# microsoft/gated-graph-neural-network-samples

Measured on AMD Instinct MI355X. Metric: node-state updates/sec on QM9-shaped graphs, h=100, 4 edge types, higher is better.
Workload: dtype f32

## Files before the change

gated-graph-neural-network-samples_amd/_lib.py:

```python
from __future__ import annotations

import ctypes
import os
from ctypes import POINTER, c_char_p, c_float, c_int, c_int32, c_int64, c_size_t, c_uint64, c_void_p

_HERE = os.path.dirname(os.path.abspath(__file__))
LIB_PATH = os.path.join(_HERE, "libggnn_hip%s.so" % ("_" + os.environ["GGNN_LIB_VARIANT"] if os.environ.get("GGNN_LIB_VARIANT") else ""))
ABI_VERSION = 3

SYMBOLS = {
    "ggnn_abi_version": (c_int, []),
    "ggnn_matrix_path_is_split": (c_int, []),
    "ggnn_gru_forward_format": (c_int, []),
    "ggnn_gru_form_set": (c_int, [c_int]),
    "ggnn_absmax_f32": (c_int, [POINTER(c_void_p), POINTER(c_int64), c_int, c_void_p, c_void_p]),
    "ggnn_last_error": (c_char_p, []),
    "ggnn_csr_workspace_bytes": (c_size_t, [c_int64, c_int]),
    "ggnn_build_target_csr": (c_int, [c_void_p, POINTER(c_int64), c_int, c_int, c_int64, c_void_p, c_void_p,
                                      c_void_p, c_void_p, c_void_p, c_size_t, c_void_p]),
    "ggnn_build_source_csr": (c_int, [c_void_p, POINTER(c_int64), c_int, c_int, c_int64, c_void_p, c_void_p,
                                      c_void_p, c_void_p, c_void_p, c_size_t, c_void_p]),
    "ggnn_msg_transform_f32": (c_int, [c_void_p, c_int, c_void_p, c_void_p, c_int, c_int, c_int, c_void_p]),
    "ggnn_msg_transform_compact_supported": (c_int, [c_int]),
    "ggnn_compact_workspace_bytes": (c_size_t, [c_int, c_int]),
    "ggnn_build_compact_sources": (c_int, [c_void_p, c_int, c_int, c_void_p, c_void_p, c_void_p, c_void_p, c_size_t, c_void_p]),
    "ggnn_remap_gather_rows": (c_int, [c_void_p, c_void_p, c_void_p, c_int64, c_void_p]),
    "ggnn_msg_transform_compact_workspace_bytes": (c_size_t, [c_int, c_int]),
    "ggnn_msg_transform_compact_f32": (c_int, [c_void_p, c_void_p, c_void_p, POINTER(c_int64), c_void_p, c_void_p, c_size_t,
                                               c_int, c_int, c_int, c_int, c_void_p]),
    "ggnn_gather_segment_sum_f32": (c_int, [c_void_p, c_void_p, c_void_p, c_void_p, c_void_p, c_int, c_void_p,
                                            c_int, c_int, c_int, c_void_p]),
    "ggnn_build_slot_heads": (c_int, [c_void_p, c_void_p, c_void_p, c_int, c_void_p]),
    "ggnn_gather_segment_sum_heads_f32": (c_int, [c_void_p, c_void_p, c_void_p, c_void_p, c_void_p, c_void_p, c_int, c_void_p,
                                                  c_int, c_int, c_int, c_int, c_void_p]),
    "ggnn_attn_bwd_target_f32": (c_int, [c_void_p] * 11 + [c_int, c_int, c_int, c_int, c_void_p]),
    "ggnn_weighted_segment_sum_f32": (c_int, [c_void_p] * 6 + [c_int, c_int, c_int, c_void_p]),
    "ggnn_range_sum_f32": (c_int, [c_void_p, POINTER(c_int64), c_int, c_void_p, c_void_p]),
    "ggnn_unsorted_segment_sum_f32": (c_int, [c_void_p, c_void_p, c_void_p, c_int64, c_int, c_int, c_void_p]),
    "ggnn_gated_readout_f32": (c_int, [c_void_p, c_void_p, c_void_p, c_void_p, c_void_p, c_void_p, c_void_p, c_void_p, c_int,
                                       c_int, c_int, c_void_p]),
    "ggnn_readout_workspace_bytes": (c_size_t, [c_int, c_int, c_int]),
    "ggnn_readout_loss_fwd_f32": (c_int, [c_void_p] * 15 + [c_void_p, c_size_t, c_int, c_int, c_int, c_void_p]),
    "ggnn_readout_loss_bwd_f32": (c_int, [c_void_p] * 14 + [c_int] + [c_void_p] * 4 + [c_void_p, c_size_t, c_int, c_int, c_int, c_void_p]),
    "ggnn_gru_workspace_bytes": (c_size_t, [c_int, c_int]),
    "ggnn_gru_f32": (c_int, [POINTER(c_void_p), c_int, c_void_p, c_void_p, c_void_p, c_void_p, c_void_p, c_void_p,
                             c_void_p, c_size_t, c_void_p, c_void_p, c_void_p, c_int, c_int, c_int, c_void_p]),
    "ggnn_gather_segment_sum_attn_f32": (c_int, [c_void_p, c_void_p, c_void_p, c_void_p, c_void_p, c_void_p, c_void_p, c_int,
                                                 c_void_p, c_int, c_int, c_int, c_void_p]),
    "ggnn_rnn_f32": (c_int, [POINTER(c_void_p), c_int, c_void_p, c_void_p, c_void_p, c_void_p, c_int, c_int, c_int, c_void_p]),
    "ggnn_cudnn_gru_workspace_bytes": (c_size_t, [c_int, c_int]),
    "ggnn_cudnn_gru_f32": (c_int, [POINTER(c_void_p), c_int, c_void_p, c_void_p, c_void_p, c_void_p, c_void_p, c_void_p,
                                   c_void_p, c_void_p, c_void_p, c_size_t, c_int, c_int, c_void_p]),
    "ggnn_gru_is_fused": (c_int, [c_int]),
    "ggnn_gru_packed_bytes": (c_size_t, [c_int, c_int]),
    "ggnn_gru_pack_weights_f32": (c_int, [c_void_p, c_void_p, c_int, c_int, c_int, c_void_p, c_void_p]),
    "ggnn_gru_packed_f32": (c_int, [POINTER(c_void_p), c_int, c_void_p, c_void_p, c_void_p, c_void_p, c_void_p, c_void_p,
                                    c_void_p, c_void_p, c_int, c_int, c_int, c_int, c_void_p, c_void_p]),
    "ggnn_edge_weights_pack_f32": (c_int, [c_void_p, c_int, c_int, c_int, c_void_p, c_void_p]),
    "ggnn_gru_packed_gather_f32": (c_int, [POINTER(c_void_p), c_int, c_void_p, c_void_p, c_void_p, c_void_p, c_void_p, c_void_p,
                                           c_void_p, c_void_p, c_void_p, c_int, c_int, c_int, c_int, c_int, c_int, c_void_p, c_void_p]),
    "ggnn_gru_packed_gather_train_f32": (c_int, [POINTER(c_void_p), c_int, c_void_p, c_void_p, c_void_p, c_void_p, c_void_p, c_void_p,
                                                 c_void_p, c_void_p, c_void_p, c_int, c_int, c_void_p, c_void_p, c_void_p, c_void_p,
                                                 c_int, c_int, c_int, c_int, c_void_p, c_void_p]),
    "ggnn_gru_gates_f32": (c_int, [POINTER(c_void_p), c_int, c_void_p, c_void_p, c_void_p, c_void_p, c_void_p, c_void_p,
                                   c_int, c_int, c_void_p]),
    "ggnn_gru_candidate_f32": (c_int, [POINTER(c_void_p), c_int, c_void_p, c_void_p, c_void_p, c_void_p, c_void_p,
                                       c_void_p, c_void_p, c_int, c_int, c_int, c_void_p]),
    "ggnn_sparse_propagate_workspace_bytes": (c_size_t, [c_int, c_int, c_int, c_int64]),
    "ggnn_sparse_propagate_f32": (c_int, [c_void_p, c_int, c_int, c_int, c_void_p, c_void_p, c_void_p, POINTER(c_int64),
                                          c_void_p, c_int, c_int, POINTER(c_int32), POINTER(c_int32), POINTER(c_int32),
                                          POINTER(c_void_p), POINTER(c_void_p), POINTER(c_void_p), POINTER(c_void_p),
                                          POINTER(c_void_p), POINTER(c_void_p), POINTER(c_void_p), POINTER(c_void_p), POINTER(c_int32),
                                          POINTER(c_int32), c_int, c_int, POINTER(c_void_p), c_void_p, c_size_t, c_void_p]),
    "ggnn_gru_bwd_stage1_f32": (c_int, [c_void_p, c_void_p, c_void_p, c_void_p, c_void_p, c_int, c_void_p, c_void_p, c_void_p,
                                        c_void_p, c_int, c_int, c_int, c_int, c_void_p]),
    "ggnn_gru_bwd_stage2_f32": (c_int, [c_void_p, c_int, c_void_p, c_void_p, c_void_p, c_void_p, c_int, c_int, c_void_p]),
    "ggnn_dense_aggregate_f32": (c_int, [c_void_p, c_void_p, c_void_p, c_void_p, c_int, c_int, c_int, c_int, c_void_p]),
    "ggnn_gemm_f32": (c_int, [POINTER(c_void_p), c_int, c_int, c_int, c_void_p, c_int, c_void_p, c_int, c_int, c_int,
                              c_void_p]),
    "ggnn_xty_workspace_bytes": (c_size_t, [c_int, c_int, c_int, c_int]),
    "ggnn_xty_f32": (c_int, [POINTER(c_void_p), c_int, c_int, POINTER(c_int32), c_void_p, c_void_p, c_int, c_void_p, c_int, c_int,
                             c_int, POINTER(c_int32), c_int, c_void_p, c_size_t, c_void_p]),
    "ggnn_dense_propagate_supported": (c_int, [c_int, c_int, c_int]),
    "ggnn_dense_propagate_is_split": (c_int, [c_int, c_int, c_int]),
    "ggnn_dense_edge_packed_bytes": (c_size_t, [c_int, c_int]),
    "ggnn_dense_edge_pack_f32": (c_int, [c_void_p, c_int, c_int, c_void_p, c_void_p]),
    "ggnn_dense_gru_packed_bytes": (c_size_t, [c_int]),
    "ggnn_dense_gru_pack_f32": (c_int, [c_void_p, c_void_p, c_int, c_void_p, c_void_p]),
    "ggnn_dense_propagate_f32": (c_int, [c_void_p, c_void_p, c_void_p, c_void_p, c_void_p, c_void_p, c_void_p, c_void_p, c_int, c_int,
                                         c_int, c_int, c_int, c_int, c_void_p]),
    "ggnn_dense_train_supported": (c_int, [c_int, c_int, c_int]),
    "ggnn_dense_train_saved_bytes": (c_size_t, [c_int, c_int, c_int, c_int]),
    "ggnn_dense_propagate_save_f32": (c_int, [c_void_p, c_void_p, c_void_p, c_void_p, c_void_p, c_void_p, c_void_p, c_void_p, c_int, c_int,
                                              c_int, c_int, c_int, c_int, c_void_p, c_size_t, c_void_p]),
    "ggnn_dense_bwd_packed_bytes": (c_size_t, [c_int, c_int]),
    "ggnn_dense_bwd_pack_f32": (c_int, [c_void_p, c_void_p, c_void_p, c_int, c_int, c_void_p, c_void_p]),
    "ggnn_dense_propagate_bwd_f32": (c_int, [c_void_p, c_void_p, c_void_p, c_void_p, c_int, c_int, c_int, c_int, c_int, c_void_p, c_void_p,
                                             c_void_p, c_void_p, c_void_p, c_void_p]),
    "ggnn_dense_edge_grad_workspace_bytes": (c_size_t, [c_int, c_int, c_int]),
    "ggnn_dense_edge_grad_f32": (c_int, [c_void_p, c_void_p, c_void_p, c_void_p, c_int, c_int, c_int, c_int, c_void_p, c_void_p, c_int,
                                         c_void_p, c_size_t, c_void_p]),
    "ggnn_dense_train_workspace_bytes": (c_size_t, [c_int, c_int, c_int, c_int, c_int]),
    "ggnn_dense_train_forward_f32": (c_int, [c_void_p, c_void_p, c_void_p, c_void_p, c_void_p, c_void_p, c_void_p, c_int, c_int, c_int,
                                             c_int, c_int, c_int, c_void_p, c_size_t, POINTER(c_int64), c_void_p]),
    "ggnn_dense_train_backward_f32": (c_int, [c_void_p, c_void_p, c_void_p, c_void_p, c_int, c_int, c_int, c_int, c_int, c_void_p,
                                              c_void_p, c_void_p, c_void_p, c_void_p, c_void_p, c_void_p, c_size_t, c_void_p, c_void_p]),
    "ggnn_assemble_batch_backward": (c_int, [POINTER(c_void_p), POINTER(c_void_p), c_int, c_int, POINTER(c_int64), POINTER(c_int64), c_void_p,
                                             c_void_p, c_int, c_int, c_int, c_int, c_int, POINTER(c_int64), POINTER(c_int64),
                                             POINTER(c_void_p), c_void_p]),
    "ggnn_assemble_batch": (c_int, [POINTER(c_void_p), c_int, c_int, POINTER(c_int64), POINTER(c_int64), c_void_p, c_int, c_int, c_int,
                                    c_int, c_int, POINTER(c_int64), POINTER(c_int64), POINTER(c_void_p), c_void_p]),
    "ggnn_xty_acc_f32": (c_int, [POINTER(c_void_p), c_int, c_int, POINTER(c_int32), c_void_p, c_void_p, c_int, c_void_p, c_void_p,
                                 c_int, c_int, c_int, c_int, POINTER(c_int32), c_int, c_void_p, c_size_t, c_void_p]),
    "ggnn_colsum_workspace_bytes": (c_size_t, [c_int]),
    "ggnn_colsum_f32": (c_int, [c_void_p, c_int, c_int, c_int, c_void_p, c_void_p, c_size_t, c_void_p]),
    "ggnn_gru_bwd_dx_cand_f32": (c_int, [c_void_p] * 7 + [c_int, c_int, c_int, c_void_p]),
    "ggnn_gru_bwd_dx_gates_f32": (c_int, [c_void_p] * 5 + [c_int, c_int, c_void_p, c_int, c_int, c_int, c_void_p]),
    "ggnn_gather_segment_sum_acc_f32": (c_int, [c_void_p, c_void_p, c_void_p, c_void_p, c_int, c_int, c_void_p]),
    "ggnn_bwd_dx_f32": (c_int, [c_void_p, c_int, c_int, c_void_p, c_int, c_void_p, c_int, c_int, c_void_p, c_void_p, c_int, c_int,
                                c_void_p, c_int, c_int, c_int, c_int, c_void_p]),
    "ggnn_act_bwd_f32": (c_int, [c_void_p, c_void_p, c_int, c_void_p, c_int, c_int, c_void_p]),
    "ggnn_cudnn_gru_train_f32": (c_int, [POINTER(c_void_p), c_int] + [c_void_p] * 9 + [c_void_p, c_size_t, c_int, c_int, c_void_p]),
    "ggnn_cudnn_gru_bwd_stage_f32": (c_int, [c_void_p] * 10 + [c_int, c_int, c_void_p]),
    "ggnn_gru_bwd_is_fused": (c_int, [c_int]),
    "ggnn_gru_bwd_packed_bytes": (c_size_t, [c_int, c_int]),
    "ggnn_gru_bwd_fused_f32": (c_int, [c_void_p] * 12 + [POINTER(c_void_p), c_void_p, c_int, c_int, c_int, c_int, c_int, c_int, c_void_p]),
    "ggnn_gru_bwd_fused_gather_f32": (c_int, [c_void_p] * 12 + [POINTER(c_void_p), c_void_p, c_int, c_int, c_int, c_int, c_int, c_int, c_void_p]),
    "ggnn_optim_block_floats": (c_int, []),
    "ggnn_clip_adam_f32": (c_int, [c_void_p] * 9 + [c_int, c_float, c_float, c_float, c_float, c_float, c_void_p]),
    "ggnn_probe_mfma_workspace_bytes": (c_size_t, []),
    "ggnn_probe_mfma_rate": (c_int, [c_int, c_int, c_void_p, c_size_t, POINTER(ctypes.c_double), POINTER(ctypes.c_double), c_void_p]),
    "ggnn_gemm_tn_workspace_bytes": (c_size_t, [c_int, c_int, c_int]),
    "ggnn_gemm_tn_f32": (c_int, [c_void_p, c_int, c_void_p, c_int, c_void_p, c_int, c_int, c_int, c_void_p, c_size_t, c_void_p]),
    "ggnn_pack_batch_tables": (c_int, [c_void_p, c_int, c_int, c_void_p, c_int, c_void_p, c_void_p, c_int, c_void_p, c_int, c_void_p,
                                       c_void_p, c_void_p, c_void_p]),
    "ggnn_sparse_train_prepare_f32": (c_int, [c_int, c_int, c_int, POINTER(c_int32), POINTER(c_void_p), c_float, POINTER(c_uint64),
                                              POINTER(c_void_p), POINTER(c_void_p), POINTER(c_int32), POINTER(c_void_p), POINTER(c_void_p),
                                              POINTER(c_void_p), POINTER(c_void_p), c_void_p]),
    "ggnn_sparse_train_workspace_bytes": (c_size_t, [c_int, c_int, c_int, c_int64, c_int]),
    "ggnn_sparse_train_forward_f32": (c_int, [c_void_p, c_int, c_int, c_int, c_void_p, c_void_p, c_void_p, POINTER(c_int64), c_void_p,
                                              c_int, c_int, POINTER(c_int32), POINTER(c_int32), POINTER(c_int32), POINTER(c_void_p),
                                              POINTER(c_void_p), POINTER(c_void_p), POINTER(c_void_p), POINTER(c_int32), c_int, c_void_p,
                                              c_size_t, POINTER(c_int64), c_void_p]),
    "ggnn_sparse_train_backward_f32": (c_int, [c_void_p, c_int, c_int, c_int, c_void_p, POINTER(c_int64), c_void_p, c_int, c_int,
                                               POINTER(c_int32), POINTER(c_int32), POINTER(c_int32), c_void_p, c_void_p, c_void_p,
                                               c_void_p, c_void_p, c_void_p, c_void_p, POINTER(c_void_p), POINTER(c_void_p), c_int,
                                               POINTER(c_void_p), POINTER(c_void_p), POINTER(c_void_p), POINTER(c_void_p),
                                               POINTER(c_void_p), c_void_p, POINTER(c_void_p), c_void_p, c_size_t, c_void_p, c_void_p]),
    "ggnn_dropout_f32": (c_int, [c_void_p, c_void_p, c_void_p, c_int64, c_uint64, c_float, c_int64, c_int, c_void_p]),
    "ggnn_gcn_fused_supported": (c_int, [c_int]),
    "ggnn_gcn_image_bytes": (c_size_t, [c_int]),
    "ggnn_gcn_pack_weights_f32": (c_int, [c_void_p, c_int, c_int, c_void_p, c_void_p]),
    "ggnn_gcn_layer_f32": (c_int, [c_void_p, c_void_p, c_void_p, c_void_p, c_int64, c_void_p, c_void_p, c_int, c_void_p, c_int64,
                                   c_uint64, c_float, c_void_p, c_void_p, c_int, c_int, c_void_p]),
    "ggnn_gcn_epilogue_f32": (c_int, [c_void_p, c_void_p, c_int, c_void_p, c_int64, c_uint64, c_float, c_void_p, c_int, c_int, c_void_p]),
    "ggnn_gcn_workspace_bytes": (c_size_t, [c_int, c_int, c_int]),
    "ggnn_gcn_propagate_f32": (c_int, [c_void_p, c_int, c_int, c_int, c_void_p, c_void_p, c_void_p, c_int64, POINTER(c_void_p),
                                       POINTER(c_void_p), c_void_p, c_void_p, c_size_t, c_void_p]),
    "ggnn_gcn_assemble_batch": (c_int, [POINTER(c_void_p), c_int, c_int, c_int, c_void_p, c_int, c_void_p, c_int, c_int, c_int, c_int,
                                        c_int, c_int, POINTER(c_void_p), c_void_p]),
    "ggnn_dense_assemble_batch": (c_int, [POINTER(c_void_p), c_int, c_int, c_int, c_int, c_void_p, c_int, c_void_p, c_int, c_int, c_int,
                                          c_int, c_int, c_int, c_int, POINTER(c_int64), POINTER(c_int64), c_int, POINTER(c_void_p),
                                          c_void_p]),
}

_lib = None


class GGNNError(RuntimeError):
    def __init__(self, code: int, msg: str):
        super().__init__("libggnn_hip error %d: %s" % (code, msg))
        self.code = code


def load() -> ctypes.CDLL:
    global _lib
    if _lib is not None:
        return _lib
    if not os.path.exists(LIB_PATH):
        raise ImportError(
            "libggnn_hip.so not found at %s -- run `python __graft_entry__.py build` (hipcc, gfx950). "
            "There is no CPU fallback for the GGNN hot path." % LIB_PATH)
    lib = ctypes.CDLL(LIB_PATH)
    for name, (restype, argtypes) in SYMBOLS.items():
        fn = getattr(lib, name)
        fn.restype = restype
        fn.argtypes = argtypes
    ver = lib.ggnn_abi_version()
    if ver != ABI_VERSION:
        raise ImportError("libggnn_hip.so ABI version %d != expected %d; rebuild" % (ver, ABI_VERSION))
    _lib = lib
    return lib


def check(rc: int) -> None:
    if rc != 0:
        msg = load().ggnn_last_error()
        raise GGNNError(rc, msg.decode("utf-8", "replace") if msg else "")
```

gated-graph-neural-network-samples_amd/csrc/ggnn_bwd_gemm.hip:

```cpp
#include "ggnn_gemm.hpp"
#include "ggnn_split.hpp"

namespace ggnn {

constexpr int kXtyMaxBatch = 64;
constexpr int kXtyWaves = 16;
constexpr int kXtyMaxI = 4;
#ifndef GGNN_XTY_TIMELINE
#define GGNN_XTY_TIMELINE 0
#endif

__device__ const float kXtyOnesChunk[4] = {1.0f, 0.0f, 0.0f, 0.0f};
__device__ const float kXtyZeroChunk[4] = {0.0f, 0.0f, 0.0f, 0.0f};

struct XtyArgs {
    const float* X[4]; int ldx[4]; int nseg; int Dseg;
    const int* x_rows;
    const float* Y; int ldy;
    float* part;
    int K, N, nbatch;
    int Kout;
    int row_off[kXtyMaxBatch + 1];
    int wg_off[kXtyMaxBatch + 1];
    int kb_tiles, n_tiles;
    int pitch_x, pitch_y;
    unsigned long long* tdbg;
};

static inline int xty_pitch(int width) {
    int p = (width + 15) / 16 * 16;
    while (p % 64 != 16 && p % 64 != 48) p += 16;
    return p;
}

__host__ __device__ inline void xty_group(int n, int g, int& off, int& cnt) {
    const int base = n >> 2, rem = n & 3;
    cnt = base + (g < rem ? 1 : 0);
    off = g * base + (g < rem ? g : rem);
}

template <bool GATHER, int ROWS, int MTM, int NTM>
__global__ __launch_bounds__(kXtyWaves * 64) void xty_kernel(XtyArgs a) {
    extern __shared__ __attribute__((aligned(16))) float slab[];
    constexpr int nw = kXtyWaves;
    const int tid = threadIdx.x, lane = tid & 63;
    const int wave = __builtin_amdgcn_readfirstlane(tid >> 6);
    const int li = lane & 15, kq = lane >> 4;
    int batch = 0;
    while (batch + 1 < a.nbatch && (int)blockIdx.y >= a.wg_off[batch + 1]) ++batch;
    const int split = (int)blockIdx.y - a.wg_off[batch], splits = a.wg_off[batch + 1] - a.wg_off[batch];
    const int rb = a.row_off[batch], re = a.row_off[batch + 1];
    int rows_per = (re - rb + splits - 1) / splits;
    rows_per = (rows_per + ROWS - 1) / ROWS * ROWS;
    const int r_beg = rb + split * rows_per;
    const int r_end = min(re, r_beg + rows_per);
    const int kcol0 = blockIdx.x * a.kb_tiles * 16;
    const int px = a.pitch_x, py = a.pitch_y;
    float* sx = slab;
    float* sy = slab + 2 * ROWS * px;
    float* out = a.part + (size_t)blockIdx.y * a.Kout * a.N;

    int kt0, my_mt, nt0, my_nt;
    xty_group(a.kb_tiles, wave >> 2, kt0, my_mt);
    xty_group(a.n_tiles, ((wave >> 2) + (wave & 3)) & 3, nt0, my_nt);

    int stamp_i = 2;
#if GGNN_XTY_TIMELINE
#define GGNN_XT(K) if (a.tdbg && blockIdx.x == 0 && blockIdx.y == 0 && lane == 0 && (wave == 0 || wave == nw - 1) && (K) < 64) \
        a.tdbg[(wave ? 64 : 0) + (K)] = __builtin_amdgcn_s_memtime();
#else
#define GGNN_XT(K)
#endif
    GGNN_XT(0)

    constexpr int MAXI = kXtyMaxI;
    const int cprx = px / 4, cpry = py / 4;
    const int nix = ROWS * cprx / 64, niy = ROWS * cpry / 64;
    unsigned mx[MAXI], my[MAXI];
#pragma unroll
    for (int j = 0; j < MAXI; ++j) {
        const int ix = j * nw + wave;
        mx[j] = 0x80000000u; my[j] = 0x80000000u;
        if (ix < nix) {
            const int c = ix * 64 + lane, row = c / cprx, q = c - row * cprx;
            int col = kcol0 + 4 * q;
            const bool ones = a.Kout > a.K && col == a.K && 4 * q < a.kb_tiles * 16;
            if (!(4 * q < a.kb_tiles * 16 && col < a.K)) col = 0;
            const int seg = col / a.Dseg, within = col - seg * a.Dseg;
            mx[j] = (unsigned)within | ((unsigned)seg << 16) | ((unsigned)row << 18) | (ones ? 0x40000000u : 0u);
        }
        if (ix < niy) {
            const int c = ix * 64 + lane, row = c / cpry, q = c - row * cpry;
            my[j] = (unsigned)(4 * q < a.N ? 4 * q : 0) | ((unsigned)row << 18);
        }
    }
    auto xrow = [&](int r0, unsigned m) -> int {
        int r = r0 + (int)((m >> 18) & 127u); r = r < r_end ? r : r_end - 1;
        return r;
    };
    int rid[GATHER ? MAXI : 1];
    auto fetch_rows = [&](int r0) {
        if constexpr (GATHER) {
#pragma unroll
            for (int j = 0; j < MAXI; ++j) rid[j] = (mx[j] >> 31) ? 0 : a.x_rows[xrow(r0 < r_end ? r0 : r_beg, mx[j])];
        }
    };
    auto sgpr_ptr = [](const float* p) {
        const unsigned long long v = reinterpret_cast<unsigned long long>(p);
        const unsigned lo = __builtin_amdgcn_readfirstlane((unsigned)v), hi = __builtin_amdgcn_readfirstlane((unsigned)(v >> 32));
        return reinterpret_cast<const float*>(((unsigned long long)hi << 32) | lo);
    };
    const float* X0 = sgpr_ptr(a.X[0]); const float* X1 = sgpr_ptr(a.X[1]);
    const float* X2 = sgpr_ptr(a.X[2]); const float* X3 = sgpr_ptr(a.X[3]);
    const int L0 = __builtin_amdgcn_readfirstlane(a.ldx[0]), L1 = __builtin_amdgcn_readfirstlane(a.ldx[1]);
    const int L2 = __builtin_amdgcn_readfirstlane(a.ldx[2]), L3 = __builtin_amdgcn_readfirstlane(a.ldx[3]);
    const float* Yb = sgpr_ptr(a.Y);
    const int ldy = __builtin_amdgcn_readfirstlane(a.ldy);
    auto issue = [&](int buf, int r0) {
#pragma unroll
        for (int j = 0; j < MAXI; ++j) {
            if (!(mx[j] >> 31)) {
                const unsigned m = mx[j];
                const int seg = (int)((m >> 16) & 3u);
                const float* xb = seg == 0 ? X0 : (seg == 1 ? X1 : (seg == 2 ? X2 : X3));
                const int xl = seg == 0 ? L0 : (seg == 1 ? L1 : (seg == 2 ? L2 : L3));
                const int xr = GATHER ? rid[GATHER ? j : 0] : xrow(r0, m);
                const float* src = xb + (size_t)xr * xl + (m & 0xFFFFu);
                if (m & 0x40000000u) src = kXtyOnesChunk;
                if (r0 + (int)((m >> 18) & 127u) >= r_end) src = kXtyZeroChunk;
                float* dst = sx + buf * ROWS * px + (size_t)(j * nw + wave) * 256;
                __builtin_amdgcn_global_load_lds((glb_void*)src, (lds_void*)dst, 16, 0, 0);
            }
        }
#pragma unroll
        for (int j = 0; j < MAXI; ++j) {
            if (!(my[j] >> 31)) {
                const unsigned m = my[j];
                int r = r0 + (int)((m >> 18) & 127u); r = r < r_end ? r : r_end - 1;
                const float* src = Yb + (size_t)r * ldy + (m & 0xFFFFu);
                float* dst = sy + buf * ROWS * py + (size_t)(j * nw + wave) * 256;
                __builtin_amdgcn_global_load_lds((glb_void*)src, (lds_void*)dst, 16, 0, 0);
            }
        }
    };

    auto run = [&](auto mt_c, auto nt_c) {
        constexpr int MT = decltype(mt_c)::value, NT = decltype(nt_c)::value;
        constexpr bool ON = MT > 0 && NT > 0;
        f32x4 acc[ON ? MT : 1][ON ? NT : 1];
#pragma unroll
        for (int mt = 0; mt < (ON ? MT : 1); ++mt)
#pragma unroll
            for (int nt = 0; nt < (ON ? NT : 1); ++nt) acc[mt][nt] = f32x4{0.f, 0.f, 0.f, 0.f};
        const int cls = wave >> 2;
        if (r_beg < r_end) {
            int buf = 0;
            fetch_rows(r_beg);
            issue(0, r_beg);
            fetch_rows(r_beg + ROWS);
            __syncthreads();
            GGNN_XT(1)
            for (int r0 = r_beg; r0 < r_end; r0 += ROWS) {
                const bool has_next = r0 + ROWS < r_end;
                if (has_next && !ON) { issue(buf ^ 1, r0 + ROWS); fetch_rows(r0 + 2 * ROWS); }
                if (stamp_i < 22) { GGNN_XT(20 + stamp_i) }
                if constexpr (ON) {
                    const float* bx = sx + buf * ROWS * px + kt0 * 16 + li;
                    const float* by = sy + buf * ROWS * py + nt0 * 16 + li;
                    float xa[2][MT], yb[2][NT];
#pragma unroll
                    for (int mt = 0; mt < MT; ++mt) xa[0][mt] = bx[kq * px + mt * 16];
#pragma unroll
                    for (int nt = 0; nt < NT; ++nt) yb[0][nt] = by[kq * py + nt * 16];
#pragma unroll
                    for (int s = 0; s < ROWS / 4; ++s) {
                        if (s + 1 < ROWS / 4) {
#pragma unroll
                            for (int mt = 0; mt < MT; ++mt) xa[(s + 1) & 1][mt] = bx[(4 * (s + 1) + kq) * px + mt * 16];
#pragma unroll
                            for (int nt = 0; nt < NT; ++nt) yb[(s + 1) & 1][nt] = by[(4 * (s + 1) + kq) * py + nt * 16];
                        }
                        if (s % (ROWS / 32) == 0 && s / (ROWS / 32) < 4) {
                            if (has_next && cls == s / (ROWS / 32)) { issue(buf ^ 1, r0 + ROWS); fetch_rows(r0 + 2 * ROWS); }
                        }
                        __builtin_amdgcn_sched_barrier(0);
#pragma unroll
                        for (int mt = 0; mt < MT; ++mt)
#pragma unroll
                            for (int nt = 0; nt < NT; ++nt)
                                acc[mt][nt] = __builtin_amdgcn_mfma_f32_16x16x4f32(xa[s & 1][mt], yb[s & 1][nt], acc[mt][nt], 0, 0, 0);
                        __builtin_amdgcn_sched_barrier(0);
                    }
                }
                if (stamp_i < 22) { GGNN_XT(40 + stamp_i) }
                __syncthreads();
                buf ^= 1;
                if (stamp_i < 22) { GGNN_XT(stamp_i) }
                ++stamp_i;
            }
        }
        GGNN_XT(62)
        if constexpr (ON) {
#pragma unroll
            for (int mt = 0; mt < MT; ++mt) {
                const int k0 = kcol0 + (kt0 + mt) * 16;
#pragma unroll
                for (int nt = 0; nt < NT; ++nt) {
                    const int n = 16 * (nt0 + nt) + li;
                    if (n < a.N) {
#pragma unroll
                        for (int e = 0; e < 4; ++e) {
                            const int k = k0 + 4 * kq + e;
                            if (k < a.Kout) out[(size_t)k * a.N + n] = acc[mt][nt][e];
                        }
                    }
                }
            }
        }
        GGNN_XT(63)
    };
    using I0 = std::integral_constant<int, 0>;
    using IM = std::integral_constant<int, MTM>; using IM1 = std::integral_constant<int, MTM - 1>;
    using IN = std::integral_constant<int, NTM>; using IN1 = std::integral_constant<int, NTM - 1>;
    if (my_mt == MTM && my_nt == NTM) run(IM{}, IN{});
    else if (my_mt == MTM - 1 && my_nt == NTM) run(IM1{}, IN{});
    else if (my_mt == MTM && my_nt == NTM - 1) run(IM{}, IN1{});
    else if (my_mt == MTM - 1 && my_nt == NTM - 1) run(IM1{}, IN1{});
    else run(I0{}, I0{});
#undef GGNN_XT
}


#ifndef GGNN_XTY_INTER_MAX
#define GGNN_XTY_INTER_MAX 24
#endif
constexpr int kXtySplitWaves = 8;
constexpr int kXtySplitMaxI = 8;

template <bool GATHER, int ROWS, int MTM, int NTM>
__global__ __launch_bounds__(kXtySplitWaves * 64) void xty_split_kernel(XtyArgs a) {
    extern __shared__ __attribute__((aligned(16))) float slab[];
    constexpr int nw = kXtySplitWaves;
    const int tid = threadIdx.x, lane = tid & 63;
    const int wave = __builtin_amdgcn_readfirstlane(tid >> 6);
    const int li = lane & 15, kq = lane >> 4;
    int batch = 0;
    while (batch + 1 < a.nbatch && (int)blockIdx.y >= a.wg_off[batch + 1]) ++batch;
    const int split = (int)blockIdx.y - a.wg_off[batch], splits = a.wg_off[batch + 1] - a.wg_off[batch];
    const int rb = a.row_off[batch], re = a.row_off[batch + 1];
    int rows_per = (re - rb + splits - 1) / splits;
    rows_per = (rows_per + ROWS - 1) / ROWS * ROWS;
    const int r_beg = rb + split * rows_per;
    const int r_end = min(re, r_beg + rows_per);
    const int kcol0 = blockIdx.x * a.kb_tiles * 16;
    const int px = a.pitch_x, py = a.pitch_y;
    float* sx = slab;
    float* sy = slab + 2 * ROWS * px;
    float* out = a.part + (size_t)blockIdx.y * a.Kout * a.N;

    int kt0, my_mt, nta0, cnta, ntb0, cntb;
    xty_group(a.kb_tiles, wave >> 1, kt0, my_mt);
    const int ga = ((wave >> 1) + 2 * (wave & 1)) & 3;
    xty_group(a.n_tiles, ga, nta0, cnta);
    xty_group(a.n_tiles, (ga + 1) & 3, ntb0, cntb);
    const int my_nt = cnta + cntb;

    constexpr int MAXI = kXtySplitMaxI;
    const int cprx = px / 4, cpry = py / 4;
    const int nix = ROWS * cprx / 64, niy = ROWS * cpry / 64;
    unsigned mx[MAXI], my[MAXI];
#pragma unroll
    for (int j = 0; j < MAXI; ++j) {
        const int ix = j * nw + wave;
        mx[j] = 0x80000000u; my[j] = 0x80000000u;
        if (ix < nix) {
            const int c = ix * 64 + lane, row = c / cprx, q = c - row * cprx;
            int col = kcol0 + 4 * q;
            const bool ones = a.Kout > a.K && col == a.K && 4 * q < a.kb_tiles * 16;
            if (!(4 * q < a.kb_tiles * 16 && col < a.K)) col = 0;
            const int seg = col / a.Dseg, within = col - seg * a.Dseg;
            mx[j] = (unsigned)within | ((unsigned)seg << 16) | ((unsigned)row << 18) | (ones ? 0x40000000u : 0u);
        }
        if (ix < niy) {
            const int c = ix * 64 + lane, row = c / cpry, q = c - row * cpry;
            my[j] = (unsigned)(4 * q < a.N ? 4 * q : 0) | ((unsigned)row << 18);
        }
    }
    auto xrow = [&](int r0, unsigned m) __attribute__((always_inline)) -> int {
        int r = r0 + (int)((m >> 18) & 127u); r = r < r_end ? r : r_end - 1;
        return r;
    };
    int rid[GATHER ? MAXI : 1];
    auto fetch_rows = [&](int r0) __attribute__((always_inline)) {
        if constexpr (GATHER) {
#pragma unroll
            for (int j = 0; j < MAXI; ++j) rid[j] = (mx[j] >> 31) ? 0 : a.x_rows[xrow(r0 < r_end ? r0 : r_beg, mx[j])];
        }
    };
    auto sgpr_ptr = [](const float* p) {
        const unsigned long long v = reinterpret_cast<unsigned long long>(p);
        const unsigned lo = __builtin_amdgcn_readfirstlane((unsigned)v), hi = __builtin_amdgcn_readfirstlane((unsigned)(v >> 32));
        return reinterpret_cast<const float*>(((unsigned long long)hi << 32) | lo);
    };
    const float* X0 = sgpr_ptr(a.X[0]); const float* X1 = sgpr_ptr(a.X[1]);
    const float* X2 = sgpr_ptr(a.X[2]); const float* X3 = sgpr_ptr(a.X[3]);
    const int L0 = __builtin_amdgcn_readfirstlane(a.ldx[0]), L1 = __builtin_amdgcn_readfirstlane(a.ldx[1]);
    const int L2 = __builtin_amdgcn_readfirstlane(a.ldx[2]), L3 = __builtin_amdgcn_readfirstlane(a.ldx[3]);
    const float* Yb = sgpr_ptr(a.Y);
    const int ldy = __builtin_amdgcn_readfirstlane(a.ldy);
    auto dma1 = [&](const float* src, float* dst) __attribute__((always_inline)) {
        const unsigned l = __builtin_amdgcn_readfirstlane((unsigned)(unsigned long)(lds_void*)dst);
        asm volatile("s_mov_b32 m0, %0\n\ts_nop 0\n\tglobal_load_lds_dwordx4 %1, off" :: "s"(l), "v"(src) : "memory");
    };
    auto issue = [&](int buf, int r0) __attribute__((always_inline)) {
#pragma unroll
        for (int j = 0; j < MAXI; ++j) {
            if (!(mx[j] >> 31)) {
                const unsigned m = mx[j];
                const int seg = (int)((m >> 16) & 3u);
                const float* xb = seg == 0 ? X0 : (seg == 1 ? X1 : (seg == 2 ? X2 : X3));
                const int xl = seg == 0 ? L0 : (seg == 1 ? L1 : (seg == 2 ? L2 : L3));
                const int xr = GATHER ? rid[GATHER ? j : 0] : xrow(r0, m);
                const float* src = xb + (size_t)xr * xl + (m & 0xFFFFu);
                if (m & 0x40000000u) src = kXtyOnesChunk;
                if (r0 + (int)((m >> 18) & 127u) >= r_end) src = kXtyZeroChunk;
                dma1(src, sx + buf * ROWS * px + (size_t)(j * nw + wave) * 256);
            }
        }
#pragma unroll
        for (int j = 0; j < MAXI; ++j) {
            if (!(my[j] >> 31)) {
                const unsigned m = my[j];
                int r = r0 + (int)((m >> 18) & 127u); r = r < r_end ? r : r_end - 1;
                dma1(Yb + (size_t)r * ldy + (m & 0xFFFFu), sy + buf * ROWS * py + (size_t)(j * nw + wave) * 256);
            }
        }
    };

    auto run = [&](auto mt_c, auto nt_c) __attribute__((always_inline)) {
        constexpr int MT = decltype(mt_c)::value, NT = decltype(nt_c)::value;
        constexpr bool ON = MT > 0 && NT > 0;
        f32x4 acc[ON ? MT : 1][ON ? NT : 1];
#pragma unroll
        for (int mt = 0; mt < (ON ? MT : 1); ++mt)
#pragma unroll
            for (int nt = 0; nt < (ON ? NT : 1); ++nt) acc[mt][nt] = f32x4{0.f, 0.f, 0.f, 0.f};
        auto ycol = [&](int t) __attribute__((always_inline)) { return (t < cnta ? nta0 + t : ntb0 + (t - cnta)) * 16; };
        if (r_beg < r_end) {
            int buf = 0;
            fetch_rows(r_beg);
            issue(0, r_beg);
            fetch_rows(r_beg + ROWS);
            dma_wait();
            __syncthreads();
            for (int r0 = r_beg; r0 < r_end; r0 += ROWS) {
                const bool has_next = r0 + ROWS < r_end;
                if (has_next) { issue(buf ^ 1, r0 + ROWS); fetch_rows(r0 + 2 * ROWS); }
                if constexpr (ON) {
                    const float* bx = sx + buf * ROWS * px + kt0 * 16 + li;
                    const float* by = sy + buf * ROWS * py + li;
                    auto tile_planes = [&](const float* col, int pitch, int s, u32x4& hi, u32x4& mid, u32x4& lo) __attribute__((always_inline)) {
                        float v[8];
#pragma unroll
                        for (int j = 0; j < 8; ++j) v[j] = col[(size_t)(32 * s + 4 * j + kq) * pitch];
                        unsigned h[4], m[4], l[4];
#pragma unroll
                        for (int q = 0; q < 4; ++q) split_pair(v[2 * q], v[2 * q + 1], h[q], m[q], l[q]);
                        hi = u32x4{h[0], h[1], h[2], h[3]}; mid = u32x4{m[0], m[1], m[2], m[3]}; lo = u32x4{l[0], l[1], l[2], l[3]};
                    };
#pragma unroll
                    for (int s = 0; s < ROWS / 32; ++s) {
                        u32x4 xh[MT], xm[MT], xl[MT];
#pragma unroll
                        for (int mt = 0; mt < MT; ++mt) tile_planes(bx + mt * 16, px, s, xh[mt], xm[mt], xl[mt]);
                        u32x4 yh, ym, yl, zh, zm, zl;
                        tile_planes(by + ycol(0), py, s, yh, ym, yl);
#pragma unroll
                        for (int nt = 0; nt < NT; ++nt) {
                            __builtin_amdgcn_sched_barrier(0);
                            if (nt + 1 < NT) tile_planes(by + ycol(nt + 1), py, s, zh, zm, zl);
#define GGNN_XS(XP, YP) _Pragma("unroll") for (int mt = 0; mt < MT; ++mt) acc[mt][nt] = mfma_bf16(XP[mt], YP, acc[mt][nt]);
                            GGNN_XS(xl, yh) GGNN_XS(xm, ym) GGNN_XS(xm, yh) GGNN_XS(xh, yl) GGNN_XS(xh, ym) GGNN_XS(xh, yh)
#undef GGNN_XS
                            yh = zh; ym = zm; yl = zl;
                        }
                        __builtin_amdgcn_sched_barrier(0);
                    }
                }
                dma_wait();
                __syncthreads();
                buf ^= 1;
            }
        }
        if constexpr (ON) {
#pragma unroll
            for (int mt = 0; mt < MT; ++mt) {
                const int k0 = kcol0 + (kt0 + mt) * 16;
#pragma unroll
                for (int nt = 0; nt < NT; ++nt) {
                    const int n = ycol(nt) + li;
                    if (n < a.N) {
#pragma unroll
                        for (int e = 0; e < 4; ++e) {
                            const int k = k0 + 4 * kq + e;
                            if (k < a.Kout) out[(size_t)k * a.N + n] = acc[mt][nt][e];
                        }
                    }
                }
            }
        }
    };
    using I0 = std::integral_constant<int, 0>;
    using IM = std::integral_constant<int, MTM>; using IM1 = std::integral_constant<int, MTM - 1>;
    using IN = std::integral_constant<int, 2 * NTM>; using IN1 = std::integral_constant<int, 2 * NTM - 1>;
    using IN2 = std::integral_constant<int, 2 * NTM - 2>;
    if (my_mt == MTM && my_nt == 2 * NTM) run(IM{}, IN{});
    else if (my_mt == MTM && my_nt == 2 * NTM - 1) run(IM{}, IN1{});
    else if (my_mt == MTM && my_nt == 2 * NTM - 2) run(IM{}, IN2{});
    else if (my_mt == MTM - 1 && my_nt == 2 * NTM) run(IM1{}, IN{});
    else if (my_mt == MTM - 1 && my_nt == 2 * NTM - 1) run(IM1{}, IN1{});
    else if (my_mt == MTM - 1 && my_nt == 2 * NTM - 2) run(IM1{}, IN2{});
    else run(I0{}, I0{});
}

template <int MTM, int NTM>
__global__ __launch_bounds__(kXtySplitWaves * 64) void xty_planes_kernel(XtyArgs a) {
    extern __shared__ __attribute__((aligned(16))) float slab[];
    constexpr int nw = kXtySplitWaves, NTH = nw * 64, ROWS = 32;
    const int tid = threadIdx.x, lane = tid & 63;
    const int wave = __builtin_amdgcn_readfirstlane(tid >> 6);
    const int li = lane & 15, kq = lane >> 4;
    int batch = 0;
    while (batch + 1 < a.nbatch && (int)blockIdx.y >= a.wg_off[batch + 1]) ++batch;
    const int split = (int)blockIdx.y - a.wg_off[batch], splits = a.wg_off[batch + 1] - a.wg_off[batch];
    const int rb = a.row_off[batch], re = a.row_off[batch + 1];
    int rows_per = (re - rb + splits - 1) / splits;
    rows_per = (rows_per + ROWS - 1) / ROWS * ROWS;
    const int r_beg = rb + split * rows_per;
    const int r_end = min(re, r_beg + rows_per);
    const int kcol0 = blockIdx.x * a.kb_tiles * 16;
    const int XC = a.kb_tiles * 16, YC = a.n_tiles * 16, CT = XC + YC;
    const unsigned plane_b = 4u * (unsigned)CT * 16u;
    const unsigned buf_b = 3u * plane_b;
    float* out = a.part + (size_t)blockIdx.y * a.Kout * a.N;

    int kt0, my_mt, nta0, cnta, ntb0, cntb;
    xty_group(a.kb_tiles, wave >> 1, kt0, my_mt);
    const int ga = ((wave >> 1) + 2 * (wave & 1)) & 3;
    xty_group(a.n_tiles, ga, nta0, cnta);
    xty_group(a.n_tiles, (ga + 1) & 3, ntb0, cntb);
    const int my_nt = cnta + cntb;

    const char* const zero_p = reinterpret_cast<const char*>(kXtyZeroChunk);
    const int QT = CT >> 2;
    const bool uon = tid < 4 * QT;
    const int ug = uon ? tid / QT : 0;
    const int uc = uon ? 4 * (tid - ug * QT) : 0;
    const int ureg = uc < XC ? 0 : XC, utile = (uc - ureg) >> 4;
    const unsigned udbase = ((unsigned)ug * (unsigned)CT + (unsigned)ureg + 16u * (unsigned)utile) * 16u;
    const unsigned urot = (unsigned)(((uc - ureg) & 15) + utile);
    const char* urow = zero_p; unsigned ustride = 0u;
    if (uon) {
        const size_t row0 = (size_t)(r_beg + 8 * ug);
        if (uc < XC) {
            const int col = kcol0 + uc;
            if (col < a.K) {
                const int seg = col / a.Dseg;
                ustride = (unsigned)a.ldx[seg] * 4u;
                urow = reinterpret_cast<const char*>(a.X[seg] + (col - seg * a.Dseg)) + row0 * ustride;
            } else if (col == a.K && a.Kout > a.K) urow = reinterpret_cast<const char*>(kXtyOnesChunk);
        } else if (uc - XC < a.N) {
            ustride = (unsigned)a.ldy * 4u;
            urow = reinterpret_cast<const char*>(a.Y + (uc - XC)) + row0 * ustride;
        }
    }
    const bool wave_on = wave * 64 < 4 * QT;
    f32x4 stage[8];
    auto fetch = [&](int r0, auto full_c) __attribute__((always_inline)) {
        constexpr bool FULL = decltype(full_c)::value;
        if (wave_on) {
            const char* q = urow;
#pragma unroll
            for (int j = 0; j < 8; ++j) {
                const char* src = q;
                if constexpr (!FULL) { if (r0 + 8 * ug + j >= r_end) src = zero_p; }
                stage[j] = *(const __attribute__((address_space(1))) f32x4*)src;
                q += ustride;
            }
            urow += (size_t)32 * ustride;
        }
    };
    auto fetch_step = [&](int r0) __attribute__((always_inline)) {
        if (r0 + ROWS <= r_end) fetch(r0, std::true_type{}); else fetch(r0, std::false_type{});
    };
    auto put_col = [&](int buf, auto k_c) __attribute__((always_inline)) {
        constexpr int k = decltype(k_c)::value;
        if (wave_on) {
            char* base = reinterpret_cast<char*>(slab) + (size_t)buf * buf_b;
            unsigned h[4], m[4], l[4];
#pragma unroll
            for (int q = 0; q < 4; ++q) split_pair(stage[2 * q][k], stage[2 * q + 1][k], h[q], m[q], l[q]);
            if (uon) {
                const unsigned d = udbase + ((urot + (unsigned)k) & 15u) * 16u;
                *reinterpret_cast<u32x4*>(base + d) = u32x4{h[0], h[1], h[2], h[3]};
                *reinterpret_cast<u32x4*>(base + plane_b + d) = u32x4{m[0], m[1], m[2], m[3]};
                *reinterpret_cast<u32x4*>(base + 2u * plane_b + d) = u32x4{l[0], l[1], l[2], l[3]};
            }
        }
    };
    auto put = [&](int buf) __attribute__((always_inline)) {
        put_col(buf, std::integral_constant<int, 0>{}); put_col(buf, std::integral_constant<int, 1>{});
        put_col(buf, std::integral_constant<int, 2>{}); put_col(buf, std::integral_constant<int, 3>{});
    };
    auto advance_col = [&](int buf, int r0, bool has_next, auto k_c) __attribute__((always_inline)) {
        if (has_next) {
            put_col(buf ^ 1, k_c);
            if (decltype(k_c)::value == 3 && r0 + 2 * ROWS < r_end) fetch_step(r0 + 2 * ROWS);
        }
    };

    auto run = [&](auto mt_c, auto nt_c) __attribute__((always_inline)) {
        constexpr int MT = decltype(mt_c)::value, NT = decltype(nt_c)::value;
        constexpr bool ON = MT > 0 && NT > 0;
        f32x4 acc[ON ? MT : 1][ON ? NT : 1];
#pragma unroll
        for (int mt = 0; mt < (ON ? MT : 1); ++mt)
#pragma unroll
            for (int nt = 0; nt < (ON ? NT : 1); ++nt) acc[mt][nt] = f32x4{0.f, 0.f, 0.f, 0.f};
        auto ytile = [&](int t) __attribute__((always_inline)) { return t < cnta ? nta0 + t : ntb0 + (t - cnta); };
        auto mma_step = [&](int buf, int r0, bool has_next, auto inter_c) __attribute__((always_inline)) {
            constexpr bool INTER = decltype(inter_c)::value;
            if constexpr (ON) {
                const char* pb = reinterpret_cast<const char*>(slab) + (size_t)buf * buf_b + (unsigned)kq * (unsigned)CT * 16u;
                auto planes = [&](int reg, int T, u32x4& hi, u32x4& mid, u32x4& lo) __attribute__((always_inline)) {
                    const char* q = pb + (unsigned)(reg + 16 * T + ((li + T) & 15)) * 16u;
                    hi = *reinterpret_cast<const u32x4*>(q); mid = *reinterpret_cast<const u32x4*>(q + plane_b);
                    lo = *reinterpret_cast<const u32x4*>(q + 2u * plane_b);
                };
                u32x4 xh[MT], xm[MT], xl[MT];
#pragma unroll
                for (int mt = 0; mt < MT; ++mt) planes(0, kt0 + mt, xh[mt], xm[mt], xl[mt]);
                u32x4 yh, ym, yl, zh, zm, zl;
                planes(XC, ytile(0), yh, ym, yl);
#pragma unroll
                for (int nt = 0; nt < NT; ++nt) {
                    if (nt + 1 < NT) planes(XC, ytile(nt + 1), zh, zm, zl);
#define GGNN_XS(XP, YP) _Pragma("unroll") for (int mt = 0; mt < MT; ++mt) acc[mt][nt] = mfma_bf16(XP[mt], YP, acc[mt][nt]);
                    GGNN_XS(xl, yh) GGNN_XS(xm, ym) GGNN_XS(xm, yh) GGNN_XS(xh, yl) GGNN_XS(xh, ym) GGNN_XS(xh, yh)
#undef GGNN_XS
                    yh = zh; ym = zm; yl = zl;
                    if constexpr (INTER) {
                        constexpr int PU = NT >= 8 ? 2 : 1;
                        if (nt % PU == 0 && nt / PU < 4) {
                            if (nt / PU == 0) advance_col(buf, r0, has_next, std::integral_constant<int, 0>{});
                            if (nt / PU == 1) advance_col(buf, r0, has_next, std::integral_constant<int, 1>{});
                            if (nt / PU == 2) advance_col(buf, r0, has_next, std::integral_constant<int, 2>{});
                            if (nt / PU == 3) advance_col(buf, r0, has_next, std::integral_constant<int, 3>{});
                        }
                    }
                }
                if constexpr (INTER && NT < 4) {
                    if (NT <= 1) advance_col(buf, r0, has_next, std::integral_constant<int, 1>{});
                    if (NT <= 2) advance_col(buf, r0, has_next, std::integral_constant<int, 2>{});
                    if (NT <= 3) advance_col(buf, r0, has_next, std::integral_constant<int, 3>{});
                }
            }
        };
        if (r_beg < r_end) {
            int buf = 0;
            fetch_step(r_beg);
            put(0);
            if (r_beg + ROWS < r_end) fetch_step(r_beg + ROWS);
            __syncthreads();
            constexpr bool INTER = ON && MT * NT <= GGNN_XTY_INTER_MAX;
            for (int r0 = r_beg; r0 < r_end; r0 += ROWS) {
                const bool has_next = r0 + ROWS < r_end;
                if constexpr (!INTER) { if (has_next) { put(buf ^ 1); if (r0 + 2 * ROWS < r_end) fetch_step(r0 + 2 * ROWS); } }
                mma_step(buf, r0, has_next, std::integral_constant<bool, INTER>{});
                __syncthreads();
                buf ^= 1;
            }
        }
        if constexpr (ON) {
#pragma unroll
            for (int mt = 0; mt < MT; ++mt) {
                const int k0 = kcol0 + (kt0 + mt) * 16;
#pragma unroll
                for (int nt = 0; nt < NT; ++nt) {
                    const int n = ytile(nt) * 16 + li;
                    if (n < a.N) {
#pragma unroll
                        for (int e = 0; e < 4; ++e) {
                            const int k = k0 + 4 * kq + e;
                            if (k < a.Kout) out[(size_t)k * a.N + n] = acc[mt][nt][e];
                        }
                    }
                }
            }
        }
    };
    using I0 = std::integral_constant<int, 0>;
    using IM = std::integral_constant<int, MTM>; using IM1 = std::integral_constant<int, MTM - 1>;
    using IN = std::integral_constant<int, 2 * NTM>; using IN1 = std::integral_constant<int, 2 * NTM - 1>;
    using IN2 = std::integral_constant<int, 2 * NTM - 2>;
    if (my_mt == MTM && my_nt == 2 * NTM) run(IM{}, IN{});
    else if (my_mt == MTM && my_nt == 2 * NTM - 1) run(IM{}, IN1{});
    else if (my_mt == MTM && my_nt == 2 * NTM - 2) run(IM{}, IN2{});
    else if (my_mt == MTM - 1 && my_nt == 2 * NTM) run(IM1{}, IN{});
    else if (my_mt == MTM - 1 && my_nt == 2 * NTM - 1) run(IM1{}, IN1{});
    else if (my_mt == MTM - 1 && my_nt == 2 * NTM - 2) run(IM1{}, IN2{});
    else run(I0{}, I0{});
}

struct XtyReduceArgs { int wg_off[kXtyMaxBatch + 1]; };
__global__ __launch_bounds__(256) void xty_reduce_kernel(const float* __restrict__ part, float* __restrict__ C, float* __restrict__ Cb,
                                                         int KN, int KwN, int nbatch, int accumulate, XtyReduceArgs ra) {
    __shared__ float red[8][32];
    const int c = threadIdx.x & 31, q = threadIdx.x >> 5;
    const long long i = (long long)blockIdx.x * 32 + c;
    const bool on = i < (long long)KN * nbatch;
    float s = 0.f;
    int b = 0, j = 0;
    if (on) {
        b = (int)(i / KN); j = (int)(i - (long long)b * KN);
        const int S = ra.wg_off[b + 1] - ra.wg_off[b];
        const float* src = part + (size_t)ra.wg_off[b] * KN + j;
        int p = q;
        for (; p + 24 < S; p += 32) {
            const float v0 = src[(size_t)p * KN], v1 = src[(size_t)(p + 8) * KN], v2 = src[(size_t)(p + 16) * KN], v3 = src[(size_t)(p + 24) * KN];
            s += v0; s += v1; s += v2; s += v3;
        }
        for (; p < S; p += 8) s += src[(size_t)p * KN];
    }
    red[q][c] = s;
    __syncthreads();
    if (q == 0 && on) {
        const float v = ((red[0][c] + red[1][c]) + (red[2][c] + red[3][c])) + ((red[4][c] + red[5][c]) + (red[6][c] + red[7][c]));
        float* dst = (Cb && j >= KwN) ? Cb + (size_t)b * (KN - KwN) + (j - KwN) : C + (size_t)b * (Cb ? KwN : KN) + j;
        *dst = accumulate ? *dst + v : v;
    }
}

struct XtyPlan { int rows, kb_tiles, n_tiles, kblocks, px, py, wg_rows; size_t lds; int wg_off[kXtyMaxBatch + 1]; };

static XtyPlan xty_plan(const int* row_off, int nbatch, int Kout, int N) {
    XtyPlan p{};
    const int ktiles = (Kout + 15) / 16;
    p.kblocks = (ktiles + 15) / 16;
    p.kb_tiles = (ktiles + p.kblocks - 1) / p.kblocks;
    p.n_tiles = (N + 15) / 16;
    p.px = xty_pitch(p.kb_tiles * 16); p.py = xty_pitch(p.n_tiles * 16);
    const int mtm = (p.kb_tiles + 3) / 4, ntm = (p.n_tiles + 3) / 4;
    p.rows = (size_t)2 * 64 * (p.px + p.py) * sizeof(float) <= (size_t)160 * 1024 && mtm + ntm <= 6 ? 64 : 32;
    static const int rows_env = [] { const char* e = getenv("GGNN_XTY_ROWS"); return e ? atoi(e) : 0; }();
    if (rows_env == 32) p.rows = 32;
    p.lds = (size_t)2 * p.rows * (p.px + p.py) * sizeof(float);
    long long total = 0;
    for (int b = 0; b < nbatch; ++b) total += row_off[b + 1] - row_off[b];
    int target = num_cus() / p.kblocks;
    if (target < 1) target = 1;
    p.wg_off[0] = 0;
    for (int b = 0; b < nbatch; ++b) {
        const long long m = row_off[b + 1] - row_off[b];
        long long w = total > 0 ? (long long)target * m / total : 0;
        const long long cap = (m + 4 * p.rows - 1) / (4 * p.rows);
        if (w > cap) w = cap;
        if (w < 1 && m > 0) w = 1;
        p.wg_off[b + 1] = p.wg_off[b] + (int)w;
    }
    p.wg_rows = p.wg_off[nbatch];
    return p;
}

template <bool GATHER, int ROWS, int MTM, int NTM>
static int launch_xty(const XtyArgs& a, const XtyPlan& p, float* C, float* Cb, int accumulate, hipStream_t st) {
    static std::atomic<unsigned long long> lds_ok{0};
    if (p.wg_rows > 0) {
        if (p.lds > 64 * 1024) GGNN_CHECK_HIP((allow_dynamic_lds(&xty_kernel<GATHER, ROWS, MTM, NTM>, p.lds, lds_ok)));
        hipLaunchKernelGGL((xty_kernel<GATHER, ROWS, MTM, NTM>), dim3(p.kblocks, p.wg_rows), dim3(kXtyWaves * 64), p.lds, st, a);
        GGNN_CHECK_HIP(hipGetLastError());
    }
    XtyReduceArgs ra;
    for (int b = 0; b <= kXtyMaxBatch; ++b) ra.wg_off[b] = a.wg_off[b <= a.nbatch ? b : a.nbatch];
    const long long total = (long long)a.Kout * a.N * a.nbatch;
    hipLaunchKernelGGL(xty_reduce_kernel, dim3((unsigned)((total + 31) / 32)), dim3(256), 0, st, (const float*)a.part, C, Cb, a.Kout * a.N,
                       a.K * a.N, a.nbatch, accumulate, ra);
    GGNN_CHECK_HIP(hipGetLastError());
    return GGNN_OK;
}

template <int MTM, int NTM>
static int launch_xty_planes(const XtyArgs& a, const XtyPlan& p, float* C, float* Cb, int accumulate, hipStream_t st) {
    static std::atomic<unsigned long long> lds_ok{0};
    const size_t lds = (size_t)2 * 192 * (size_t)(16 * (p.kb_tiles + p.n_tiles));
    if (p.wg_rows > 0) {
        if (lds > 64 * 1024) GGNN_CHECK_HIP((allow_dynamic_lds(&xty_planes_kernel<MTM, NTM>, lds, lds_ok)));
        hipLaunchKernelGGL((xty_planes_kernel<MTM, NTM>), dim3(p.kblocks, p.wg_rows), dim3(kXtySplitWaves * 64), lds, st, a);
        GGNN_CHECK_HIP(hipGetLastError());
    }
    XtyReduceArgs ra;
    for (int b = 0; b <= kXtyMaxBatch; ++b) ra.wg_off[b] = a.wg_off[b <= a.nbatch ? b : a.nbatch];
    const long long total = (long long)a.Kout * a.N * a.nbatch;
    hipLaunchKernelGGL(xty_reduce_kernel, dim3((unsigned)((total + 31) / 32)), dim3(256), 0, st, (const float*)a.part, C, Cb, a.Kout * a.N,
                       a.K * a.N, a.nbatch, accumulate, ra);
    GGNN_CHECK_HIP(hipGetLastError());
    return GGNN_OK;
}

template <bool GATHER, int ROWS, int MTM, int NTM>
static int launch_xty_split(const XtyArgs& a, const XtyPlan& p, float* C, float* Cb, int accumulate, hipStream_t st) {
    static std::atomic<unsigned long long> lds_ok{0};
    if (p.wg_rows > 0) {
        if (p.lds > 64 * 1024) GGNN_CHECK_HIP((allow_dynamic_lds(&xty_split_kernel<GATHER, ROWS, MTM, NTM>, p.lds, lds_ok)));
        hipLaunchKernelGGL((xty_split_kernel<GATHER, ROWS, MTM, NTM>), dim3(p.kblocks, p.wg_rows), dim3(kXtySplitWaves * 64), p.lds, st, a);
        GGNN_CHECK_HIP(hipGetLastError());
    }
    XtyReduceArgs ra;
    for (int b = 0; b <= kXtyMaxBatch; ++b) ra.wg_off[b] = a.wg_off[b <= a.nbatch ? b : a.nbatch];
    const long long total = (long long)a.Kout * a.N * a.nbatch;
    hipLaunchKernelGGL(xty_reduce_kernel, dim3((unsigned)((total + 31) / 32)), dim3(256), 0, st, (const float*)a.part, C, Cb, a.Kout * a.N,
                       a.K * a.N, a.nbatch, accumulate, ra);
    GGNN_CHECK_HIP(hipGetLastError());
    return GGNN_OK;
}

constexpr int kColsumBlocks = 256;

__global__ __launch_bounds__(256) void colsum_partial_kernel(const float* __restrict__ Y, int ldy, int M, int N, float* __restrict__ part) {
    extern __shared__ float red[];
    const int N4 = N >> 2;
    const int lanes_per_row = N4;
    const int rows_par = 256 / lanes_per_row > 0 ? 256 / lanes_per_row : 1;
    const int rl = threadIdx.x / lanes_per_row, c4 = threadIdx.x % lanes_per_row;
    f32x4 s = {0.f, 0.f, 0.f, 0.f};
    if (rl < rows_par) {
        for (int r = blockIdx.x * rows_par + rl; r < M; r += gridDim.x * rows_par)
            s += *reinterpret_cast<const f32x4*>(Y + (size_t)r * ldy + 4 * c4);
        *reinterpret_cast<f32x4*>(red + rl * N + 4 * c4) = s;
    }
    __syncthreads();
    for (int i = threadIdx.x; i < N; i += 256) {
        float t = 0.f;
        for (int q = 0; q < rows_par; ++q) t += red[q * N + i];
        part[(size_t)blockIdx.x * N + i] = t;
    }
}

__global__ void colsum_final_kernel(const float* __restrict__ part, int nblocks, int N, float* __restrict__ out) {
    const int i = blockIdx.x * blockDim.x + threadIdx.x;
    if (i >= N) return;
    float s[8] = {0.f, 0.f, 0.f, 0.f, 0.f, 0.f, 0.f, 0.f};
    int b = 0;
    for (; b + 8 <= nblocks; b += 8) {
#pragma unroll
        for (int q = 0; q < 8; ++q) s[q] += part[(size_t)(b + q) * N + i];
    }
    for (int q = 0; b < nblocks; ++b, ++q) s[q] += part[(size_t)b * N + i];
    out[i] = ((s[0] + s[1]) + (s[2] + s[3])) + ((s[4] + s[5]) + (s[6] + s[7]));
}

}

using namespace ggnn;

extern "C" size_t ggnn_xty_workspace_bytes(int M_max, int K, int N, int nbatch) {
    if (M_max <= 0 || K <= 0 || N <= 0 || nbatch <= 0) return 256;
    return (size_t)(num_cus() + nbatch) * (K + 1) * N * sizeof(float) + 256;
}

extern "C" int ggnn_xty_f32(const float* const* x_segs, int nseg, int Dseg, const int32_t* ldx, const int32_t* x_rows,
                            const float* Y, int ldy, float* C, int K, int N, int ones_row, const int32_t* row_off, int nbatch,
                            void* ws, size_t ws_bytes, ggnn_stream_t stream) {
    return ggnn_xty_acc_f32(x_segs, nseg, Dseg, ldx, x_rows, Y, ldy, C, nullptr, 0, K, N, ones_row, row_off, nbatch, ws, ws_bytes, stream);
}

extern "C" int ggnn_xty_acc_f32(const float* const* x_segs, int nseg, int Dseg, const int32_t* ldx, const int32_t* x_rows,
                                const float* Y, int ldy, float* C, float* Cb, int accumulate, int K, int N, int ones_row,
                                const int32_t* row_off, int nbatch, void* ws, size_t ws_bytes, ggnn_stream_t stream) {
    const int Kout = ones_row ? K + 1 : K;
    GGNN_CHECK_ARG(!Cb || ones_row, "a bias destination needs the ones row");
    GGNN_CHECK_ARG(nseg >= 1 && nseg <= 4 && Dseg > 0 && Dseg % 4 == 0 && K == nseg * Dseg, "X is nseg <= 4 segments of Dseg columns (K = %d, nseg = %d, Dseg = %d)", K, nseg, Dseg);
    GGNN_CHECK_ARG(N > 0 && N % 4 == 0 && N <= 256, "N = %d must be a multiple of 4, <= 256", N);
    GGNN_CHECK_ARG(nbatch >= 1 && nbatch <= kXtyMaxBatch && row_off && C && ldx, "bad batch description");
    GGNN_CHECK_ARG(ldy >= N && ldy % 4 == 0, "ldy %d", ldy);
    hipStream_t st = (hipStream_t)stream;
    XtyArgs a{};
    int m_max = 0;
    for (int b = 0; b <= nbatch; ++b) {
        a.row_off[b] = row_off[b];
        if (b) { GGNN_CHECK_ARG(row_off[b] >= row_off[b - 1], "row_off not monotone"); m_max = row_off[b] - row_off[b - 1] > m_max ? row_off[b] - row_off[b - 1] : m_max; }
    }
    if (m_max == 0) {
        if (!accumulate) {
            GGNN_CHECK_HIP(hipMemsetAsync(C, 0, (size_t)nbatch * (Cb ? K : Kout) * N * sizeof(float), st));
            if (Cb) GGNN_CHECK_HIP(hipMemsetAsync(Cb, 0, (size_t)nbatch * N * sizeof(float), st));
        }
        return GGNN_OK;
    }
    GGNN_CHECK_ARG(x_segs && Y && ws && aligned16(Y) && aligned16(ws), "null or misaligned pointer");
    for (int s = 0; s < nseg; ++s) {
        GGNN_CHECK_ARG(x_segs[s] && aligned16(x_segs[s]) && ldx[s] >= Dseg && ldx[s] % 4 == 0, "X segment %d null, misaligned or bad stride", s);
        a.X[s] = x_segs[s]; a.ldx[s] = ldx[s];
    }
    if (ws_bytes < ggnn_xty_workspace_bytes(m_max, K, N, nbatch)) return fail(GGNN_E_WORKSPACE, "xty workspace too small");
    const XtyPlan p = xty_plan(row_off, nbatch, Kout, N);
    a.Kout = Kout;
    a.nseg = nseg; a.Dseg = Dseg; a.x_rows = x_rows; a.Y = Y; a.ldy = ldy; a.part = static_cast<float*>(ws);
    a.K = K; a.N = N; a.nbatch = nbatch; a.kb_tiles = p.kb_tiles; a.n_tiles = p.n_tiles;
    a.pitch_x = p.px; a.pitch_y = p.py;
    for (int b = 0; b <= kXtyMaxBatch; ++b) a.wg_off[b] = p.wg_off[b <= nbatch ? b : nbatch];
    { const char* e = getenv("GGNN_XTY_TPTR"); a.tdbg = e ? (unsigned long long*)strtoull(e, nullptr, 10) : nullptr; }
    if ((p.rows * p.px / 256 + kXtyWaves - 1) / kXtyWaves > kXtyMaxI || (p.rows * p.py / 256 + kXtyWaves - 1) / kXtyWaves > kXtyMaxI)
        return fail(GGNN_E_UNSUPPORTED, "xty: slab too wide (K=%d N=%d)", K, N);
    const int mtm = (p.kb_tiles + 3) / 4, ntm = (p.n_tiles + 3) / 4;
    const bool g = x_rows != nullptr;
    static const bool xty_split = [] { const char* e = getenv("GGNN_XTY_SPLIT"); return !e || atoi(e) != 0; }();
    if (split_matrix_path() && xty_split && p.kb_tiles >= 4 && p.n_tiles >= 4 && (p.rows * p.px / 256 + kXtySplitWaves - 1) / kXtySplitWaves <= kXtySplitMaxI &&
        (p.rows * p.py / 256 + kXtySplitWaves - 1) / kXtySplitWaves <= kXtySplitMaxI) {
        static const bool xty_planes = [] { const char* e = getenv("GGNN_XTY_PLANES"); return !e || atoi(e) != 0; }();
        if (xty_planes && !g && (size_t)2 * 192 * 16 * (p.kb_tiles + p.n_tiles) <= (size_t)160 * 1024 &&
            16 * (p.kb_tiles + p.n_tiles) <= kXtySplitWaves * 64) {
#define GGNN_XTYP_CASE(M, Nn) if (mtm == M && ntm == Nn) return launch_xty_planes<M, Nn>(a, p, C, Cb, accumulate, st);
            GGNN_XTYP_CASE(4, 4) GGNN_XTYP_CASE(3, 4) GGNN_XTYP_CASE(4, 2) GGNN_XTYP_CASE(3, 2)
#undef GGNN_XTYP_CASE
        }
#define GGNN_XTYS_CASE(G, R, M, Nn) if (g == G && p.rows == R && mtm == M && ntm == Nn) return launch_xty_split<G, R, M, Nn>(a, p, C, Cb, accumulate, st);
        GGNN_XTYS_CASE(false, 32, 4, 4) GGNN_XTYS_CASE(false, 32, 3, 4) GGNN_XTYS_CASE(false, 64, 4, 2) GGNN_XTYS_CASE(false, 64, 3, 2)
#undef GGNN_XTYS_CASE
    }
#define GGNN_XTY_CASE(G, R, M, Nn) if (g == G && p.rows == R && mtm == M && ntm == Nn) return launch_xty<G, R, M, Nn>(a, p, C, Cb, accumulate, st);
#define GGNN_XTY_ROW32(M) GGNN_XTY_CASE(false, 32, M, 1) GGNN_XTY_CASE(false, 32, M, 2) GGNN_XTY_CASE(false, 32, M, 3) GGNN_XTY_CASE(false, 32, M, 4)
    GGNN_XTY_ROW32(1) GGNN_XTY_ROW32(2) GGNN_XTY_ROW32(3) GGNN_XTY_ROW32(4)
    GGNN_XTY_CASE(false, 64, 1, 1) GGNN_XTY_CASE(false, 64, 1, 2) GGNN_XTY_CASE(false, 64, 1, 3) GGNN_XTY_CASE(false, 64, 1, 4)
    GGNN_XTY_CASE(false, 64, 2, 1) GGNN_XTY_CASE(false, 64, 2, 2) GGNN_XTY_CASE(false, 64, 2, 3) GGNN_XTY_CASE(false, 64, 2, 4)
    GGNN_XTY_CASE(false, 64, 3, 1) GGNN_XTY_CASE(false, 64, 3, 2) GGNN_XTY_CASE(false, 64, 3, 3)
    GGNN_XTY_CASE(false, 64, 4, 1) GGNN_XTY_CASE(false, 64, 4, 2)
    GGNN_XTY_CASE(true, 64, 1, 1) GGNN_XTY_CASE(true, 64, 1, 2) GGNN_XTY_CASE(true, 64, 2, 1) GGNN_XTY_CASE(true, 64, 2, 2)
#undef GGNN_XTY_ROW32
#undef GGNN_XTY_CASE
    return fail(GGNN_E_UNSUPPORTED, "xty: no kernel for %d x %d tile groups (K=%d N=%d)", mtm, ntm, K, N);
}

extern "C" size_t ggnn_colsum_workspace_bytes(int N) { return (size_t)kColsumBlocks * (N > 0 ? N : 1) * sizeof(float) + 256; }

extern "C" int ggnn_colsum_f32(const float* Y, int ldy, int M, int N, float* out, void* ws, size_t ws_bytes, ggnn_stream_t stream) {
    GGNN_CHECK_ARG(M >= 0 && N > 0 && N % 4 == 0 && N <= 1024 && ldy >= N && ldy % 4 == 0, "bad sizes M=%d N=%d ldy=%d", M, N, ldy);
    GGNN_CHECK_ARG(out && ws, "null pointer");
    if (ws_bytes < ggnn_colsum_workspace_bytes(N)) return fail(GGNN_E_WORKSPACE, "colsum workspace too small");
    hipStream_t st = (hipStream_t)stream;
    if (M == 0) { GGNN_CHECK_HIP(hipMemsetAsync(out, 0, N * sizeof(float), st)); return GGNN_OK; }
    GGNN_CHECK_ARG(Y && aligned16(Y), "null or misaligned pointer");
    const int rows_par = 256 / (N / 4) > 0 ? 256 / (N / 4) : 1;
    GGNN_CHECK_ARG(N / 4 <= 256, "N too large");
    int nb = (M + rows_par - 1) / rows_par;
    if (nb > kColsumBlocks) nb = kColsumBlocks;
    float* part = static_cast<float*>(ws);
    hipLaunchKernelGGL(colsum_partial_kernel, dim3(nb), dim3(256), (size_t)rows_par * N * sizeof(float), st, Y, ldy, M, N, part);
    GGNN_CHECK_HIP(hipGetLastError());
    hipLaunchKernelGGL(colsum_final_kernel, dim3((N + 255) / 256), dim3(256), 0, st, (const float*)part, nb, N, out);
    GGNN_CHECK_HIP(hipGetLastError());
    return GGNN_OK;
}
```

gated-graph-neural-network-samples_amd/csrc/ggnn_train.hip:

```cpp
#include "ggnn_split.hpp"
#include "ggnn_philox.hpp"
#include <mutex>

namespace ggnn {
namespace {

constexpr int kMaxLayers = 62;
constexpr int kMaxNx = 3;

inline size_t al256(size_t x) { return (x + 255) / 256 * 256; }

struct TrainLayout {
    size_t Hc, state, r, u, c, inc, counters;
    size_t dpc, rh, dh, dpg, dx, dHc, Z, xty;
    size_t vd, rd, total;
    int steps;
};

TrainLayout train_layout(int V, int D, int T, int64_t R, int steps) {
    TrainLayout L{};
    L.steps = steps;
    L.vd = (size_t)V * D * sizeof(float);
    L.rd = al256((size_t)(R > 0 ? R : 1) * D * sizeof(float));
    size_t p = 0;
    auto take = [&](size_t bytes) { const size_t at = p; p += al256(bytes); return at; };
    L.Hc = take(L.rd);
    L.state = take(L.vd * (steps + 1));
    L.r = take(L.vd * steps); L.u = take(L.vd * steps); L.c = take(L.vd * steps);
    L.inc = take(L.vd * steps);
    L.counters = take((size_t)steps * sizeof(int32_t));
    L.dpc = take(L.vd * steps); L.rh = take(L.vd * steps); L.dh = take(L.vd * steps); L.dpg = take(2 * L.vd * steps);
    L.dx = take(L.vd * steps * kMaxNx);
    L.dHc = take(L.rd * steps); L.Z = take(L.rd);
    L.xty = take(ggnn_xty_workspace_bytes((V > R ? V : (int)R) * (steps > 1 ? steps : 1), 4 * D, 2 * D, T));
    L.total = p + 256;
    (void)T;
    return L;
}

struct EventPool {
    hipEvent_t ev[64];
    int next = 0;
    bool ready = false;
};
std::mutex g_pool_mutex;
EventPool g_pools[16];

int next_event(hipEvent_t* out) {
    int dev = 0;
    GGNN_CHECK_HIP(hipGetDevice(&dev));
    std::lock_guard<std::mutex> lock(g_pool_mutex);
    EventPool& p = g_pools[dev & 15];
    if (!p.ready) {
        for (int i = 0; i < 64; ++i) GGNN_CHECK_HIP(hipEventCreateWithFlags(&p.ev[i], hipEventDisableTiming));
        p.ready = true;
    }
    *out = p.ev[p.next];
    p.next = (p.next + 1) & 63;
    return GGNN_OK;
}

int order_after(hipStream_t waiter, hipStream_t producer) {
    if (waiter == producer) return GGNN_OK;
    hipEvent_t e;
    if (int rc = next_event(&e)) return rc;
    GGNN_CHECK_HIP(hipEventRecord(e, producer));
    GGNN_CHECK_HIP(hipStreamWaitEvent(waiter, e, 0));
    return GGNN_OK;
}

__global__ void add_inplace_kernel(float* __restrict__ dst, const float* __restrict__ src, long long n4) {
    const long long i = (long long)blockIdx.x * blockDim.x + threadIdx.x;
    if (i >= n4) return;
    f32x4 a = reinterpret_cast<f32x4*>(dst)[i];
    const f32x4 b = reinterpret_cast<const f32x4*>(src)[i];
    a += b;
    reinterpret_cast<f32x4*>(dst)[i] = a;
}

int add_inplace(float* dst, const float* src, long long n, hipStream_t st) {
    const long long n4 = n / 4;
    if (n4 == 0) return GGNN_OK;
    hipLaunchKernelGGL(add_inplace_kernel, dim3((unsigned)((n4 + 255) / 256)), dim3(256), 0, st, dst, src, n4);
    GGNN_CHECK_HIP(hipGetLastError());
    return GGNN_OK;
}

constexpr int kPrepMaxLayers = 16;
struct PrepArgs {
    const float* edge_w[kPrepMaxLayers]; const float* Wg[kPrepMaxLayers]; const float* Wc[kPrepMaxLayers];
    float* edge_img[kPrepMaxLayers]; float* edge_img_t[kPrepMaxLayers]; float* gru_img[kPrepMaxLayers]; float* gru_bwd_img[kPrepMaxLayers];
    unsigned long long seed[kPrepMaxLayers];
    int nx[kPrepMaxLayers];
    int gru_fmt[kPrepMaxLayers];
    int T; float keep;
};

template <int D, bool SF>
__global__ __launch_bounds__(256) void train_prepare_kernel(PrepArgs a) {
    using C = StageCfg<D>;
    const int l = blockIdx.z, i = blockIdx.y;
    const int first = blockIdx.x * blockDim.x + threadIdx.x, stride = gridDim.x * blockDim.x;
    const int T = a.T, ng = 3 * (a.nx[l] + 1);
    if (i < 2 * T) {
        const bool tr = i >= T;
        const int t = tr ? i - T : i;
        const float* W = a.edge_w[l] + (size_t)t * D * D;
        const float keep = a.keep;
        const unsigned long long seed = a.seed[l];
        auto value = [&](int k, int n) -> float {
            if (n >= D) return 0.f;
            const int r = tr ? n : k, c = tr ? k : n;
            float v = W[(size_t)r * D + c];
            if (keep < 1.0f) v = dropout_apply(v, keep, seed, (unsigned long long)(t * D + r), c);
            return v;
        };
        float* img = (tr ? a.edge_img_t[l] : a.edge_img[l]) + (size_t)t * ImgCfg<D, SF>::IMG;
        if constexpr (SF) {
            pack_split_image<D>(value, img, first, stride);
        } else {
            for (int j = first; j < C::IMG; j += stride) {
                float v = 0.f;
                if (j < C::MAIN) {
                    const int e = j & 3, n = (j >> 2) % C::BN, k = 4 * ((j >> 2) / C::BN) + e;
                    v = value(k, n);
                } else if (j < C::MAIN + C::REM) {
                    const int jj = j - C::MAIN;
                    v = value(16 * C::NC + jj / C::BN, jj % C::BN);
                }
                img[j] = v;
            }
        }
    } else if (i < 2 * T + ng) {
        const int ci = i - 2 * T;
        if constexpr (SF) {
            if (a.gru_fmt[l] == kSplitF16x2)
                gru_fwd_image_pack_split<D, kSplitF16x2>(a.Wg[l], a.Wc[l], a.nx[l], ci, a.gru_img[l] + (size_t)ci * ImgCfg<D, true, kSplitF16x2>::IMG, first, stride);
            else
                gru_fwd_image_pack_split<D, kSplitBf16x3>(a.Wg[l], a.Wc[l], a.nx[l], ci, a.gru_img[l] + (size_t)ci * ImgCfg<D, true>::IMG, first, stride);
        } else gru_fwd_image_pack<D>(a.Wg[l], a.Wc[l], a.nx[l], ci, a.gru_img[l] + (size_t)ci * ImgCfg<D, false>::IMG, first, stride);
    } else if (i < 2 * T + 2 * ng) {
        const int bi = i - 2 * T - ng;
        float* img = a.gru_bwd_img[l] + (size_t)bi * ImgCfg<D, SF>::IMG;
        if constexpr (SF) gru_bwd_image_pack_split<D>(a.Wg[l], a.Wc[l], a.nx[l], bi, img, first, stride);
        else gru_bwd_image_pack<D>(a.Wg[l], a.Wc[l], a.nx[l], bi, img, first, stride);
    }
}

bool merge_products() {
    static const bool v = [] { const char* e = getenv("GGNN_TRAIN_MERGE_PRODUCTS"); return !e || atoi(e) != 0; }();
    return v;
}

struct LayerPlan { int first_step, steps, nres; int res[kMaxNx]; };

int plan_layers(int num_layers, const int32_t* layer_timesteps, const int32_t* res_ptr, const int32_t* res_idx, LayerPlan* plan,
                int* total_steps) {
    GGNN_CHECK_ARG(num_layers > 0 && num_layers <= kMaxLayers && layer_timesteps && res_ptr, "bad layer description");
    int steps = 0;
    for (int l = 0; l < num_layers; ++l) {
        LayerPlan& P = plan[l];
        P.first_step = steps; P.steps = layer_timesteps[l];
        GGNN_CHECK_ARG(P.steps >= 1, "layer %d has %d timesteps: the native training step needs at least one per layer", l, P.steps);
        P.nres = res_ptr[l + 1] - res_ptr[l];
        GGNN_CHECK_ARG(P.nres >= 0 && P.nres + 1 <= kMaxNx, "layer %d has %d residual inputs (the fused kernels take %d)", l, P.nres, kMaxNx - 1);
        for (int i = 0; i < P.nres; ++i) {
            P.res[i] = res_idx[res_ptr[l] + i];
            GGNN_CHECK_ARG(P.res[i] >= 0 && P.res[i] <= l, "layer %d: residual index %d refers to a later layer", l, P.res[i]);
        }
        steps += P.steps;
    }
    *total_steps = steps;
    return GGNN_OK;
}

}

int stream_order_after(hipStream_t waiter, hipStream_t producer) { return order_after(waiter, producer); }

}

using namespace ggnn;

extern "C" int ggnn_sparse_train_prepare_f32(int num_layers, int T, int D, const int32_t* nx, const float* const* edge_w, float keep_prob,
                                             const uint64_t* seeds, const float* const* Wg, const float* const* Wc,
                                             const int32_t* gru_fmt, float* const* edge_packed, float* const* edge_packed_t,
                                             float* const* gru_packed, float* const* gru_bwd_packed, ggnn_stream_t stream) {
    GGNN_CHECK_ARG(num_layers > 0 && num_layers <= kPrepMaxLayers, "num_layers %d outside 1..%d", num_layers, kPrepMaxLayers);
    GGNN_CHECK_ARG(T > 0 && T <= 64 && nx && edge_w && Wg && Wc && edge_packed && edge_packed_t && gru_packed && gru_bwd_packed, "bad arguments");
    GGNN_CHECK_ARG(keep_prob > 0.0f && keep_prob <= 1.0f && (keep_prob >= 1.0f || seeds), "keep_prob %g outside (0, 1] or seeds missing", (double)keep_prob);
    if (ggnn_gru_is_fused(D) != 1 || !ggnn_gru_bwd_is_fused(D) || !ggnn_msg_transform_compact_supported(D))
        return fail(GGNN_E_UNSUPPORTED, "no whole-block stage images for hidden size %d", D);
    PrepArgs a{};
    a.T = T; a.keep = keep_prob;
    int max_images = 0;
    for (int l = 0; l < num_layers; ++l) {
        GGNN_CHECK_ARG(nx[l] >= 1 && nx[l] <= kMaxNx, "layer %d: nx %d outside 1..%d", l, nx[l], kMaxNx);
        GGNN_CHECK_ARG(edge_w[l] && Wg[l] && Wc[l] && edge_packed[l] && edge_packed_t[l] && gru_packed[l] && gru_bwd_packed[l], "layer %d: null pointer", l);
        a.edge_w[l] = edge_w[l]; a.Wg[l] = Wg[l]; a.Wc[l] = Wc[l];
        a.edge_img[l] = edge_packed[l]; a.edge_img_t[l] = edge_packed_t[l]; a.gru_img[l] = gru_packed[l]; a.gru_bwd_img[l] = gru_bwd_packed[l];
        a.seed[l] = seeds ? seeds[l] : 0ULL; a.nx[l] = nx[l];
        a.gru_fmt[l] = gru_launch_fmt(gru_fmt ? gru_fmt[l] : kSplitBf16x3);
        const int images = 2 * T + 6 * (nx[l] + 1);
        if (images > max_images) max_images = images;
    }
    const dim3 grid(8, max_images, num_layers);
    hipStream_t st = (hipStream_t)stream;
    const bool sf = split_matrix_path();
#define GGNN_PREP(DD) if (sf) hipLaunchKernelGGL((train_prepare_kernel<DD, true>), grid, dim3(256), 0, st, a); \
                      else hipLaunchKernelGGL((train_prepare_kernel<DD, false>), grid, dim3(256), 0, st, a);
    switch (D) {
        case 100: GGNN_PREP(100) break;
        case 64: GGNN_PREP(64) break;
        default: GGNN_PREP(32) break;
    }
#undef GGNN_PREP
    GGNN_CHECK_HIP(hipGetLastError());
    return GGNN_OK;
}

extern "C" size_t ggnn_sparse_train_workspace_bytes(int V, int D, int T, int64_t compact_rows, int total_steps) {
    if (V < 0 || D <= 0 || T <= 0 || total_steps <= 0) return 0;
    return train_layout(V, D, T, compact_rows, total_steps).total;
}

extern "C" int ggnn_sparse_train_forward_f32(
        const float* h0, int V, int D, int T, const int32_t* row_ptr, const int32_t* gather_row_c, const int32_t* pair_node,
        const int64_t* type_row_off, const float* nin, int use_avg, int num_layers, const int32_t* layer_timesteps,
        const int32_t* res_ptr, const int32_t* res_idx, const float* const* edge_packed, const float* const* bg,
        const float* const* bc, const float* const* gru_packed, const int32_t* gru_fmt, int act, void* ws, size_t ws_bytes,
        int64_t* final_state_offset, ggnn_stream_t stream) {
    GGNN_CHECK_ARG(V > 0 && D > 0 && D % 4 == 0 && T > 0, "bad sizes V=%d D=%d T=%d", V, D, T);
    GGNN_CHECK_ARG(h0 && row_ptr && gather_row_c && pair_node && type_row_off && ws && final_state_offset, "null pointer");
    GGNN_CHECK_ARG(edge_packed && bg && bc && gru_packed, "weights missing");
    GGNN_CHECK_ARG((reinterpret_cast<size_t>(ws) & 255) == 0, "workspace must be 256-byte aligned");
    if (ggnn_gru_is_fused(D) != 1 || !ggnn_msg_transform_compact_supported(D))
        return fail(GGNN_E_UNSUPPORTED, "native training step: hidden size %d has no gather-fused GRU / compacted transform", D);
    LayerPlan plan[kMaxLayers];
    int steps = 0;
    if (int rc = plan_layers(num_layers, layer_timesteps, res_ptr, res_idx, plan, &steps)) return rc;
    const int64_t R = type_row_off[T];
    GGNN_CHECK_ARG(R > 0, "no messages in the batch");
    const TrainLayout L = train_layout(V, D, T, R, steps);
    if (ws_bytes < L.total) return fail(GGNN_E_WORKSPACE, "training workspace too small: %zu < %zu", ws_bytes, L.total);
    char* base = static_cast<char*>(ws);
    float* Hc = reinterpret_cast<float*>(base + L.Hc);
    int32_t* counters = reinterpret_cast<int32_t*>(base + L.counters);
    hipStream_t st = (hipStream_t)stream;
    GGNN_CHECK_HIP(hipMemsetAsync(counters, 0, (size_t)steps * sizeof(int32_t), st));
    auto buf = [&](size_t off, int step) { return reinterpret_cast<float*>(base + off + (size_t)step * L.vd); };
    const float* states[kMaxLayers + 1];
    states[0] = h0;
    GGNN_CHECK_HIP(hipMemcpyAsync(buf(L.state, 0), h0, L.vd, hipMemcpyDeviceToDevice, st));
    const size_t edge_img_bytes = ggnn_msg_transform_compact_workspace_bytes(D, T);
    for (int l = 0; l < num_layers; ++l) {
        const LayerPlan& P = plan[l];
        const float* xs[kMaxNx];
        for (int i = 0; i < P.nres; ++i) xs[i] = states[P.res[i]];
        const int nx = P.nres + 1;
        const float* cur = states[l];
        GGNN_CHECK_ARG(edge_packed[l] && bg[l] && bc[l] && gru_packed[l], "layer %d: weights missing", l);
        for (int s = 0; s < P.steps; ++s) {
            const int k = P.first_step + s;
            if (int rc = ggnn_msg_transform_compact_f32(cur, nullptr, pair_node, type_row_off, Hc, const_cast<float*>(edge_packed[l]),
                                                        edge_img_bytes, V, D, T, GGNN_GRU_FMT_BF16X3, stream)) return rc;
            float* out = buf(L.state, k + 1);
            if (int rc = ggnn_gru_packed_gather_train_f32(xs, nx, cur, gru_packed[l], bg[l], bc[l], out, Hc, row_ptr, gather_row_c,
                                                          use_avg ? nin : nullptr, T, use_avg ? 1 : 0, buf(L.r, k), buf(L.u, k),
                                                          buf(L.c, k), buf(L.inc, k), V, D, act,
                                                          gru_fmt ? gru_fmt[l] : GGNN_GRU_FMT_BF16X3, counters + k, stream)) return rc;
            cur = out;
        }
        states[l + 1] = cur;
    }
    *final_state_offset = (int64_t)(reinterpret_cast<const char*>(states[num_layers]) - base);
    return GGNN_OK;
}

extern "C" int ggnn_sparse_train_backward_f32(
        const float* h0, int V, int D, int T, const int32_t* pair_node, const int64_t* type_row_off, const float* nin, int use_avg,
        int num_layers, const int32_t* layer_timesteps, const int32_t* res_ptr, const int32_t* res_idx,
        const int32_t* rows_rp, const int32_t* rows_gather, const int32_t* rows_heads,
        const int32_t* node_rp, const int32_t* node_order, const int32_t* node_heads, const int32_t* identity_rows,
        const float* const* edge_packed_t, const float* const* gru_bwd_packed, int act,
        float* const* g_edge, float* const* g_Wg, float* const* g_bg, float* const* g_Wc, float* const* g_bc,
        float* d_final, float* const* d_state_ws, void* ws, size_t ws_bytes, ggnn_stream_t stream, ggnn_stream_t side_stream) {
    GGNN_CHECK_ARG(V > 0 && D > 0 && D % 4 == 0 && T > 0 && T <= 64, "bad sizes V=%d D=%d T=%d", V, D, T);
    GGNN_CHECK_ARG(h0 && pair_node && type_row_off && rows_rp && rows_gather && node_rp && node_order && identity_rows && d_final && ws,
                   "null pointer");
    GGNN_CHECK_ARG(edge_packed_t && gru_bwd_packed && g_edge && g_Wg && g_bg && g_Wc && g_bc && d_state_ws, "weights / gradient buffers missing");
    GGNN_CHECK_ARG(!use_avg || nin, "nin is required for mean aggregation");
    GGNN_CHECK_ARG((reinterpret_cast<size_t>(ws) & 255) == 0, "workspace must be 256-byte aligned");
    if (!ggnn_gru_bwd_is_fused(D)) return fail(GGNN_E_UNSUPPORTED, "native training step: no fused GRU backward for hidden size %d", D);
    LayerPlan plan[kMaxLayers];
    int steps = 0;
    if (int rc = plan_layers(num_layers, layer_timesteps, res_ptr, res_idx, plan, &steps)) return rc;
    const int64_t R64 = type_row_off[T];
    GGNN_CHECK_ARG(R64 > 0 && R64 < (1LL << 31), "bad compact row count");
    const int R = (int)R64;
    const TrainLayout L = train_layout(V, D, T, R, steps);
    if (ws_bytes < L.total) return fail(GGNN_E_WORKSPACE, "training workspace too small: %zu < %zu", ws_bytes, L.total);
    char* base = static_cast<char*>(ws);
    hipStream_t st = (hipStream_t)stream, side = side_stream ? (hipStream_t)side_stream : (hipStream_t)stream;
    auto buf = [&](size_t off, int step) { return reinterpret_cast<float*>(base + off + (size_t)step * L.vd); };
    float* Z = reinterpret_cast<float*>(base + L.Z);
    void* xty_ws = base + L.xty;
    const size_t xty_ws_bytes = L.total - 256 - L.xty;
    const size_t edge_img_bytes = ggnn_msg_transform_compact_workspace_bytes(D, T);
    const long long nvd = (long long)V * D;
    int32_t row_off_v[2] = {0, V};
    int32_t row_off_t[65];
    for (int t = 0; t <= T; ++t) row_off_t[t] = (int32_t)type_row_off[t];

    const float* states[kMaxLayers + 1];
    states[0] = buf(L.state, 0);
    for (int l = 0; l < num_layers; ++l) states[l + 1] = buf(L.state, plan[l].first_step + plan[l].steps);
    (void)h0;
    float* dstate[kMaxLayers + 1];
    bool has[kMaxLayers + 1];
    for (int l = 0; l < num_layers; ++l) { dstate[l] = d_state_ws[l]; has[l] = false; GGNN_CHECK_ARG(dstate[l], "d_state_ws[%d] is null", l); }
    dstate[num_layers] = d_final; has[num_layers] = true;

    if (int rc = order_after(side, st)) return rc;

    static const bool fuse_env = [] { const char* e = getenv("GGNN_TRAIN_FUSE_NODE_SUM"); return !e || atoi(e) != 0; }();
    const bool fuse_node_sum = fuse_env && node_heads != nullptr && T <= 4;
    bool z_pending = false;

    for (int l = num_layers - 1; l >= 0; --l) {
        const LayerPlan& P = plan[l];
        const int nx = P.nres + 1;
        GGNN_CHECK_ARG(has[l + 1], "no gradient reaches the output of layer %d", l);
        GGNN_CHECK_ARG(edge_packed_t[l] && gru_bwd_packed[l] && g_edge[l] && g_Wg[l] && g_bg[l] && g_Wc[l] && g_bc[l], "layer %d: pointers missing", l);
        const float* g = dstate[l + 1];
        for (int s = P.steps - 1; s >= 0; --s) {
            const int k = P.first_step + s;
            const float* h_in = buf(L.state, k);
            float* dh_dst = buf(L.dh, k);
            bool dh_direct = false;
            if (s == 0 && !has[l]) { dh_dst = dstate[l]; dh_direct = true; }
            float* dxp[kMaxNx];
            bool dx_direct[kMaxNx];
            for (int i = 0; i < P.nres; ++i) {
                const int src = P.res[i];
                dx_direct[i] = !has[src] && !(s == 0 && src == l && dh_direct);
                for (int j = 0; j < i; ++j) if (P.res[j] == src) dx_direct[i] = false;
                dxp[i] = dx_direct[i] ? dstate[src] : reinterpret_cast<float*>(base + L.dx + ((size_t)k * kMaxNx + i) * L.vd);
            }
            float* dinc = reinterpret_cast<float*>(base + L.dx + ((size_t)k * kMaxNx + (nx - 1)) * L.vd);
            dxp[nx - 1] = dinc;
            float* dpc = buf(L.dpc, k); float* rh = buf(L.rh, k);
            float* dpg = reinterpret_cast<float*>(base + L.dpg + (size_t)k * 2 * L.vd);
            if (z_pending) {
                if (int rc = ggnn_gru_bwd_fused_gather_f32(g, Z, node_heads, h_in, buf(L.r, k), buf(L.u, k), buf(L.c, k),
                                                           const_cast<float*>(gru_bwd_packed[l]), dpc, dpg, rh, dh_dst, dxp, nin, T,
                                                           use_avg ? 1 : 0, nx, V, D, act, stream)) return rc;
                z_pending = false;
            } else {
                if (int rc = ggnn_gru_bwd_fused_f32(g, h_in, buf(L.r, k), buf(L.u, k), buf(L.c, k), nullptr, nullptr,
                                                    const_cast<float*>(gru_bwd_packed[l]), dpc, dpg, rh, dh_dst, dxp, nin, T, use_avg ? 1 : 0,
                                                    nx, V, D, act, stream)) return rc;
            }
            for (int i = 0; i < P.nres; ++i) if (dx_direct[i]) has[P.res[i]] = true;
            if (dh_direct) has[l] = true;

            const bool merged = P.nres == 0 && P.steps > 1 && merge_products();
            if (merged) {
                if (s == 0) {
                    if (int rc = order_after(side, st)) return rc;
                    const int k0 = P.first_step;
                    int32_t row_off_m[2] = {0, V * P.steps};
                    const float* X[2] = {buf(L.inc, k0), buf(L.rh, k0)}; int32_t ldx[2] = {D, D};
                    if (int rc = ggnn_xty_acc_f32(X, 2, D, ldx, nullptr, buf(L.dpc, k0), D, g_Wc[l], g_bc[l], 1, 2 * D, D, 1, row_off_m, 1,
                                                  xty_ws, xty_ws_bytes, side)) return rc;
                    X[1] = buf(L.state, k0);
                    if (int rc = ggnn_xty_acc_f32(X, 2, D, ldx, nullptr, reinterpret_cast<float*>(base + L.dpg + (size_t)k0 * 2 * L.vd), 2 * D,
                                                  g_Wg[l], g_bg[l], 1, 2 * D, 2 * D, 1, row_off_m, 1, xty_ws, xty_ws_bytes, side)) return rc;
                }
            } else {
                if (int rc = order_after(side, st)) return rc;
                const float* X[4]; int32_t ldx[4];
                for (int i = 0; i < P.nres; ++i) { X[i] = states[P.res[i]]; ldx[i] = D; }
                X[nx - 1] = buf(L.inc, k); ldx[nx - 1] = D;
                X[nx] = rh; ldx[nx] = D;
                if (int rc = ggnn_xty_acc_f32(X, nx + 1, D, ldx, nullptr, dpc, D, g_Wc[l], g_bc[l], 1, (nx + 1) * D, D, 1, row_off_v, 1,
                                              xty_ws, xty_ws_bytes, side)) return rc;
                X[nx] = h_in;
                if (int rc = ggnn_xty_acc_f32(X, nx + 1, D, ldx, nullptr, dpg, 2 * D, g_Wg[l], g_bg[l], 1, (nx + 1) * D, 2 * D, 1, row_off_v, 1,
                                              xty_ws, xty_ws_bytes, side)) return rc;
            }

            float* dHc = reinterpret_cast<float*>(base + L.dHc + (size_t)k * L.rd);
            if (rows_heads) {
                if (int rc = ggnn_gather_segment_sum_heads_f32(dinc, rows_rp, rows_gather, rows_heads, nullptr, nullptr, 0, dHc, R, D, 1, 0, stream)) return rc;
            } else {
                if (int rc = ggnn_gather_segment_sum_f32(dinc, rows_rp, rows_gather, nullptr, nullptr, 0, dHc, R, D, 1, stream)) return rc;
            }
            const bool first_step = l == 0 && s == 0;
            if (!first_step) {
                if (int rc = ggnn_msg_transform_compact_f32(dHc, nullptr, identity_rows, type_row_off, Z, const_cast<float*>(edge_packed_t[l]),
                                                            edge_img_bytes, R, D, T, GGNN_GRU_FMT_BF16X3, stream)) return rc;
                if (fuse_node_sum) {
                    z_pending = true;
                } else if (node_heads) {
                    if (int rc = ggnn_gather_segment_sum_heads_f32(Z, node_rp, node_order, node_heads, nullptr, nullptr, 0, dh_dst, V, D, 1, 1, stream)) return rc;
                } else {
                    if (int rc = ggnn_gather_segment_sum_acc_f32(Z, node_rp, node_order, dh_dst, V, D, stream)) return rc;
                }
            }
            if (int rc = order_after(side, st)) return rc;
            {
                const float* X[1] = {h_in}; int32_t ldx[1] = {D};
                if (int rc = ggnn_xty_acc_f32(X, 1, D, ldx, pair_node, dHc, D, g_edge[l], nullptr, 1, D, D, 0, row_off_t, T, xty_ws, xty_ws_bytes,
                                              side)) return rc;
            }
            for (int i = 0; i < P.nres; ++i) {
                if (!dx_direct[i] && P.res[i] != 0) { if (int rc = add_inplace(dstate[P.res[i]], dxp[i], nvd, st)) return rc; }
            }
            if (s == 0 && !dh_direct && l != 0) { if (int rc = add_inplace(dstate[l], dh_dst, nvd, st)) return rc; }
            g = dh_dst;
        }
    }
    GGNN_CHECK_ARG(!z_pending, "internal: a deferred node sum of the transform backward was never added (fuse_node_sum invariant)");
    return order_after(st, side);
}
```

gated-graph-neural-network-samples_amd/ops.py:

```python
from __future__ import annotations

import ctypes
import os
from dataclasses import dataclass
from typing import Any, Dict, List, Optional, Sequence

import torch

from . import _lib
from ._lib import check

ACT_IDS = {"tanh": 0, "relu": 1}
GRU_FUSED_MAX_INPUTS = 3
GRU_MAX_INPUTS = 7
GRU_FMT_F16X2, GRU_FMT_EXACT = 2, 3


def kernel_width(D: int) -> int:
    D = int(D)
    if D <= 0:
        raise ValueError("hidden_size must be positive")
    if D % 32 == 0 or D % 100 == 0:
        return D
    for w in (32, 64, 100, 128, 192, 256):
# ... 46 lines not shown
    if t.dtype != dtype:
        raise TypeError("%s must be %s, got %s" % (name, dtype, t.dtype))
    if not t.is_contiguous():
        raise ValueError("%s must be contiguous" % name)
    return t


def _ptr(t: Optional[torch.Tensor]):
    return None if t is None else t.data_ptr()


@dataclass
class MessageIndex:
    adj: torch.Tensor
    type_off: List[int]
    row_ptr: torch.Tensor
    gather_row: torch.Tensor
    msg_perm: torch.Tensor
    num_nodes: int
    num_edge_types: int

    @property
    def num_messages(self) -> int:
        return int(self.type_off[-1])


def _build_index(adjacency_lists: Sequence[torch.Tensor], num_nodes: int, validate: bool, by_source: bool) -> MessageIndex:
    lib = _lib.load()
    T = len(adjacency_lists)
    if T == 0:
        raise ValueError("need at least one edge type")
    lists = [_req(a.reshape(-1, 2), torch.int32, "adjacency_lists[%d]" % i) for i, a in enumerate(adjacency_lists)]
    dev = lists[0].device
    type_off = [0]
    for a in lists:
        type_off.append(type_off[-1] + a.shape[0])
    M = type_off[-1]
    adj = torch.cat(lists, dim=0).contiguous() if M else torch.zeros((0, 2), dtype=torch.int32, device=dev)
    nseg = num_nodes * T if by_source else num_nodes
    row_ptr = torch.empty(nseg + 1, dtype=torch.int32, device=dev)
    gather_row = torch.empty(M, dtype=torch.int32, device=dev)
    msg_perm = torch.empty(M, dtype=torch.int32, device=dev)
    err = torch.zeros(1, dtype=torch.int32, device=dev)
    ws_bytes = lib.ggnn_csr_workspace_bytes(M, num_nodes)
    ws = torch.empty(ws_bytes, dtype=torch.uint8, device=dev)
    off = (ctypes.c_int64 * (T + 1))(*type_off)
    fn = lib.ggnn_build_source_csr if by_source else lib.ggnn_build_target_csr
    check(fn(_ptr(adj), off, T, num_nodes, M, _ptr(row_ptr), _ptr(gather_row), _ptr(msg_perm), _ptr(err), _ptr(ws),
             ws_bytes, _stream()))
    if validate and M and int(err.item()) != 0:
        raise IndexError("adjacency list holds a node id outside [0, %d)" % num_nodes)
    return MessageIndex(adj, type_off, row_ptr, gather_row, msg_perm, nseg, T)


def build_message_index(adjacency_lists: Sequence[torch.Tensor], num_nodes: int,
                        validate: bool = True) -> MessageIndex:
    return _build_index(adjacency_lists, num_nodes, validate, by_source=False)


def build_source_index(adjacency_lists: Sequence[torch.Tensor], num_nodes: int) -> MessageIndex:
    return _build_index(adjacency_lists, num_nodes, False, by_source=True)


USE_SLOT_HEADS = os.environ.get("GGNN_SLOT_HEADS", "1") != "0"


def slot_heads(owner, row_ptr: torch.Tensor, gather_row: torch.Tensor, num_segments: int) -> Optional[torch.Tensor]:
    if not USE_SLOT_HEADS or num_segments == 0:
        return None
    cached = getattr(owner, "_slot_heads", None)
    if cached is not None and cached[0] is gather_row:
        return cached[1]
    lib = _lib.load()
    heads = torch.empty((num_segments, 4), dtype=torch.int32, device=row_ptr.device)
    check(lib.ggnn_build_slot_heads(_ptr(row_ptr), _ptr(gather_row), _ptr(heads), num_segments, _stream()))
    owner._slot_heads = (gather_row, heads)
    return heads


def _segment_sum(name, Hrows, row_ptr, gather_row, heads, nin, bias, use_avg, out, V, D, T, accumulate=False):
    lib = _lib.load()
    if heads is not None:
        _launch(name, lambda: lib.ggnn_gather_segment_sum_heads_f32(
            _ptr(Hrows), _ptr(row_ptr), _ptr(gather_row), _ptr(heads), _ptr(nin), _ptr(bias), 1 if use_avg else 0, _ptr(out), V, D, T,
            1 if accumulate else 0, _stream()))
    elif accumulate:
        _launch(name, lambda: lib.ggnn_gather_segment_sum_acc_f32(_ptr(Hrows), _ptr(row_ptr), _ptr(gather_row), _ptr(out), V, D, _stream()))
    else:
        _launch(name, lambda: lib.ggnn_gather_segment_sum_f32(_ptr(Hrows), _ptr(row_ptr), _ptr(gather_row), _ptr(nin), _ptr(bias),
                                                              1 if use_avg else 0, _ptr(out), V, D, T, _stream()))
    return out


def msg_transform(h: torch.Tensor, edge_weights: torch.Tensor, out: Optional[torch.Tensor] = None) -> torch.Tensor:
    lib = _lib.load()
    _req(h, torch.float32, "h"); _req(edge_weights, torch.float32, "edge_weights")
    V, D = h.shape
    T = edge_weights.shape[0]
    if edge_weights.shape != (T, D, D):
        raise ValueError("edge_weights must be [T,D,D]")
    if out is None:
        out = torch.empty((V, T * D), dtype=torch.float32, device=h.device)
    else:
        _req(out, torch.float32, "out")
        if out.shape != (V, T * D):
            raise ValueError("out must be [V, T*D]")
    _launch("msg_transform", lambda: lib.ggnn_msg_transform_f32(_ptr(h), D, _ptr(edge_weights), _ptr(out), V, D, T, _stream()))
    return out


def gather_segment_sum(H: torch.Tensor, index: MessageIndex, num_incoming_edges_per_type: Optional[torch.Tensor],
                       edge_biases: Optional[torch.Tensor], use_avg: bool,
                       out: Optional[torch.Tensor] = None) -> torch.Tensor:
    lib = _lib.load()
    _req(H, torch.float32, "H")
    V, T = index.num_nodes, index.num_edge_types
    if H.shape[0] != V or H.shape[1] % T:
        raise ValueError("H must be [V, T*D]")
    D = H.shape[1] // T
    nin = num_incoming_edges_per_type
    if nin is not None:
        _req(nin, torch.float32, "num_incoming_edges_per_type")
        if nin.shape != (V, T):
            raise ValueError("num_incoming_edges_per_type must be [V,T]")
    if edge_biases is not None:
        _req(edge_biases, torch.float32, "edge_biases")
        if edge_biases.shape != (T, D):
            raise ValueError("edge_biases must be [T,D]")
    if out is None:
        out = torch.empty((V, D), dtype=torch.float32, device=H.device)
    else:
        _req(out, torch.float32, "out")
    return _segment_sum("gather_segment_sum", H, index.row_ptr, index.gather_row, slot_heads(index, index.row_ptr, index.gather_row, V),
                        nin, edge_biases, use_avg, out, V, D, T)


def gru_workspace(V: int, D: int, device) -> torch.Tensor:
    lib = _lib.load()
    return torch.empty(lib.ggnn_gru_workspace_bytes(V, D) // 4, dtype=torch.float32, device=device)


def gru(x_segs: Sequence[torch.Tensor], h: torch.Tensor, Wg: torch.Tensor, bg: torch.Tensor, Wc: torch.Tensor,
        bc: torch.Tensor, activation: str = "tanh", out: Optional[torch.Tensor] = None,
        ws: Optional[torch.Tensor] = None, save: Optional[dict] = None, two_launch: bool = False,
        fmt: Optional[int] = None) -> torch.Tensor:
    lib = _lib.load()
    if fmt is not None and int(fmt) != GRU_FMT_EXACT and not two_launch and lib.ggnn_gru_is_fused(h.shape[1]) \
            and len(x_segs) <= GRU_FUSED_MAX_INPUTS:
        _req(Wg, torch.float32, "Wg"); _req(Wc, torch.float32, "Wc")
        packed = _gru_images().gru(Wg, Wc, len(x_segs), h.shape[1], int(fmt))
        return gru_packed(x_segs, h, packed, bg, bc, activation, out=out, fmt=int(fmt), save=save)
    _req(h, torch.float32, "h")
    V, D = h.shape
    nx = len(x_segs)
    for i, x in enumerate(x_segs):
        _req(x, torch.float32, "x_segs[%d]" % i)
        if x.shape != (V, D):
            raise ValueError("x_segs[%d] must be [V,D]" % i)
    for n, w, shp in (("Wg", Wg, ((nx + 1) * D, 2 * D)), ("bg", bg, (2 * D,)), ("Wc", Wc, ((nx + 1) * D, D)), ("bc", bc, (D,))):
        _req(w, torch.float32, n)
        if tuple(w.shape) != shp:
            raise ValueError("%s must have shape %s, got %s" % (n, shp, tuple(w.shape)))
    act = ACT_IDS.get(activation.lower())
    if act is None:
        raise Exception("Unknown activation function type '%s'." % activation)
    if out is None:
        out = torch.empty_like(h)
    if ws is None:
        ws = gru_workspace(V, D, h.device)
    sr = su = sc = None
    if save is not None:
        sr = save["r"] = torch.empty_like(h)
        su = save["u"] = torch.empty_like(h)
        sc = save["c"] = torch.empty_like(h)
    segs = (ctypes.c_void_p * nx)(*[x.data_ptr() for x in x_segs])
    if not two_launch and (_timing is None or lib.ggnn_gru_is_fused(D)):
        _launch("gru_fused[nx=%d]" % nx, lambda: lib.ggnn_gru_f32(
            segs, nx, _ptr(h), _ptr(Wg), _ptr(bg), _ptr(Wc), _ptr(bc), _ptr(out), _ptr(ws), ws.numel() * 4,
            _ptr(sr), _ptr(su), _ptr(sc), V, D, act, _stream()))
    else:
        if ws.numel() < 2 * V * D:
            raise ValueError("GRU workspace too small")
        rh = ws[:V * D]
        u = su if su is not None else ws[V * D:2 * V * D]
        _launch("gru_gates[nx=%d]" % nx, lambda: lib.ggnn_gru_gates_f32(segs, nx, _ptr(h), _ptr(Wg), _ptr(bg), _ptr(rh),
                                                                         _ptr(u), _ptr(sr), V, D, _stream()))
        _launch("gru_candidate[nx=%d]" % nx, lambda: lib.ggnn_gru_candidate_f32(
            segs, nx, _ptr(rh), _ptr(h), _ptr(u), _ptr(Wc), _ptr(bc), _ptr(out), _ptr(sc), V, D, act, _stream()))
    return out


def gemm(a_segs: Sequence[torch.Tensor], B: torch.Tensor, out: Optional[torch.Tensor] = None) -> torch.Tensor:
    lib = _lib.load()
    M, D = a_segs[0].shape
    lda = a_segs[0].stride(0) if M > 1 else D
    for i, a in enumerate(a_segs):
        if not a.is_cuda or a.dtype != torch.float32:
            raise TypeError("a_segs[%d] must be a float32 CUDA/HIP tensor" % i)
        if a.shape != (M, D) or a.stride(1) != 1 or (M > 1 and a.stride(0) != lda):
            raise ValueError("all segments must be [M,D] row-major with one common row stride")
    _req(B, torch.float32, "B")
    K, N = B.shape
    if K != len(a_segs) * D:
        raise ValueError("B must be [nseg*D, N]")
    if out is None:
        out = torch.empty((M, N), dtype=torch.float32, device=B.device)
    segs = (ctypes.c_void_p * len(a_segs))(*[a.data_ptr() for a in a_segs])
    _launch("gemm[K=%d,N=%d]" % (K, N), lambda: lib.ggnn_gemm_f32(segs, len(a_segs), D, lda, _ptr(B), N, _ptr(out), N, M, N, _stream()))
    return out


def gemm_tn(x: torch.Tensor, dy: torch.Tensor) -> torch.Tensor:
    lib = _lib.load()
    for name, t in (("x", x), ("dy", dy)):
        if not t.is_cuda or t.dtype != torch.float32 or t.dim() != 2 or (t.shape[0] > 0 and t.stride(1) != 1):
            raise TypeError("%s must be a 2-D float32 CUDA/HIP tensor with unit column stride" % name)
    M, K = x.shape
    N = dy.shape[1]
    if dy.shape[0] != M:
        raise ValueError("x and dy must have the same number of rows")
    if M == 0:
        return torch.zeros((K, N), dtype=torch.float32, device=x.device)
    if M > 1 and (dy.stride(0) % 4 != 0 or dy.data_ptr() % 16 != 0):
        n_pad = (N + 3) // 4 * 4
        buf = torch.zeros((M, n_pad), dtype=torch.float32, device=dy.device)
        buf[:, :N] = dy
        return gemm_tn(x, buf)[:, :N].contiguous() if n_pad != N else gemm_tn(x, buf)
    if N > 512 or N % 4 != 0:
        n4 = N // 4 * 4
        parts = [gemm_tn(x, dy[:, c:min(c + 512, n4)]) for c in range(0, n4, 512)]
        if n4 < N:
            tail = torch.zeros((M, 4), dtype=torch.float32, device=dy.device)
            tail[:, :N - n4] = dy[:, n4:]
            parts.append(gemm_tn(x, tail)[:, :N - n4])
        return torch.cat(parts, dim=1)
    lda = x.stride(0) if M > 1 else K
    ldb = dy.stride(0) if M > 1 else N
    out = torch.empty((K, N), dtype=torch.float32, device=x.device)
    ws_bytes = lib.ggnn_gemm_tn_workspace_bytes(M, K, N)
    ws = torch.empty(ws_bytes, dtype=torch.uint8, device=x.device)
    _launch("gemm_tn[K=%d,N=%d]" % (K, N), lambda: lib.ggnn_gemm_tn_f32(_ptr(x), lda, _ptr(dy), ldb, _ptr(out), M, K, N,
                                                                       _ptr(ws), ws_bytes, _stream()))
    return out


def xty(x_segs: Sequence[torch.Tensor], dy: torch.Tensor, x_rows: Optional[torch.Tensor] = None,
        row_off: Optional[Sequence[int]] = None, ones_row: bool = False, add_to: Optional[torch.Tensor] = None,
        add_bias_to: Optional[torch.Tensor] = None) -> Optional[torch.Tensor]:
    lib = _lib.load()
    nseg = len(x_segs)
    Dseg = x_segs[0].shape[1]
    if nseg > 4:
        if row_off is not None or x_rows is not None:
            raise ValueError("batched / row-gathered products take at most 4 segments")
        N = dy.shape[1]
        groups = [list(x_segs[i:i + 4]) for i in range(0, nseg, 4)]
        if add_to is not None:
            dst = add_to.view(nseg * Dseg, N)
            k0 = 0
            for gi, grp in enumerate(groups):
                last = gi == len(groups) - 1
                xty(grp, dy, ones_row=ones_row and last, add_to=dst[k0:k0 + len(grp) * Dseg], add_bias_to=add_bias_to if last else None)
                k0 += len(grp) * Dseg
            return None
        parts = [xty(grp, dy, ones_row=ones_row and gi == len(groups) - 1) for gi, grp in enumerate(groups)]
        return torch.cat(parts, dim=0)
    for i, x in enumerate(x_segs):
        if not x.is_cuda or x.dtype != torch.float32 or x.dim() != 2 or x.shape[1] != Dseg or (x.shape[0] > 1 and x.stride(1) != 1):
            raise TypeError("x_segs[%d] must be a [M, %d] float32 CUDA/HIP tensor with unit column stride" % (i, Dseg))
    if not dy.is_cuda or dy.dtype != torch.float32 or dy.dim() != 2 or (dy.shape[0] > 1 and dy.stride(1) != 1):
        raise TypeError("dy must be a 2-D float32 CUDA/HIP tensor with unit column stride")
    M, N = dy.shape
    K = nseg * Dseg
    batched = row_off is not None
    offs = [0, M] if row_off is None else [int(o) for o in row_off]
    B = len(offs) - 1
    Kout = K + 1 if ones_row else K
    if add_to is not None:
        if ones_row != (add_bias_to is not None):
            raise ValueError("add_to with ones_row needs add_bias_to (and vice versa)")
        for t, n in ((add_to, B * K * N), (add_bias_to, B * N)):
            if t is not None and (not t.is_cuda or t.dtype != torch.float32 or not t.is_contiguous() or t.numel() != n):
                raise TypeError("accumulation buffers must be contiguous float32 CUDA/HIP tensors of %d elements" % n)
        out = None
    else:
        out = torch.empty((B, Kout, N), dtype=torch.float32, device=dy.device)
    m_max = max([offs[b + 1] - offs[b] for b in range(B)] + [0])
    ws_bytes = lib.ggnn_xty_workspace_bytes(m_max, K, N, B)
    ws = torch.empty(ws_bytes, dtype=torch.uint8, device=dy.device)
    segs = (ctypes.c_void_p * nseg)(*[x.data_ptr() for x in x_segs])
    ldx = (ctypes.c_int32 * nseg)(*[(x.stride(0) if x.shape[0] > 1 else Dseg) for x in x_segs])
    ro = (ctypes.c_int32 * (B + 1))(*offs)
    ldy = dy.stride(0) if M > 1 else N
    if x_rows is not None:
        _req(x_rows, torch.int32, "x_rows")
    if out is None:
        _launch("xty[K=%d,N=%d%s]" % (K, N, ",x%d" % B if batched else ""), lambda: lib.ggnn_xty_acc_f32(
            segs, nseg, Dseg, ldx, _ptr(x_rows), _ptr(dy), ldy, _ptr(add_to), _ptr(add_bias_to), 1, K, N, 1 if ones_row else 0, ro, B,
            _ptr(ws), ws_bytes, _stream()))
        return None
    _launch("xty[K=%d,N=%d%s]" % (K, N, ",x%d" % B if batched else ""), lambda: lib.ggnn_xty_f32(
        segs, nseg, Dseg, ldx, _ptr(x_rows), _ptr(dy), ldy, _ptr(out), K, N, 1 if ones_row else 0, ro, B, _ptr(ws), ws_bytes, _stream()))
    return out if batched else out[0]


def colsum(dy: torch.Tensor) -> torch.Tensor:
    lib = _lib.load()
    M, N = dy.shape
    if N > 1024:
        return torch.cat([colsum(dy[:, c:min(c + 1024, N)]) for c in range(0, N, 1024)])
    out = torch.empty(N, dtype=torch.float32, device=dy.device)
    ws_bytes = lib.ggnn_colsum_workspace_bytes(N)
    ws = torch.empty(ws_bytes, dtype=torch.uint8, device=dy.device)
    _launch("colsum[N=%d]" % N, lambda: lib.ggnn_colsum_f32(_ptr(dy), dy.stride(0) if M > 1 else N, M, N, _ptr(out), _ptr(ws), ws_bytes, _stream()))
    return out


def segment_sum_rows_acc(rows: torch.Tensor, index, out: torch.Tensor) -> torch.Tensor:
    lib = _lib.load()
    _req(rows, torch.float32, "rows"); _req(out, torch.float32, "out")
    return _segment_sum("gather_segment_sum_acc", rows, index.row_ptr, index.gather_row,
                        slot_heads(index, index.row_ptr, index.gather_row, index.num_nodes), None, None, False, out, index.num_nodes,
                        rows.shape[1], 1, accumulate=True)


def gru_bwd_is_fused(D: int) -> bool:
    return bool(_lib.load().ggnn_gru_bwd_is_fused(D))


def gru_bwd_fused(g, h, r, u, c, packed, nin, use_avg: bool, nx: int, activation: str, gather=None):
    lib = _lib.load()
    V, D = h.shape
    T = nin.shape[1] if nin is not None else 1
    dev = h.device
    dpc = torch.empty_like(h); rh = torch.empty_like(h); dh = torch.empty_like(h)
    dpg = torch.empty((V, 2 * D), dtype=torch.float32, device=dev)
    dx = [torch.empty_like(h) for _ in range(nx)]
    dxp = (ctypes.c_void_p * nx)(*[t.data_ptr() for t in dx])
    if gather is not None:
        rows, heads = gather
        _req(rows, torch.float32, "rows"); _req(heads, torch.int32, "heads")
        _launch("gru_bwd_fused_gather[nx=%d]" % nx, lambda: lib.ggnn_gru_bwd_fused_gather_f32(
            _ptr(g), _ptr(rows), _ptr(heads), _ptr(h), _ptr(r), _ptr(u), _ptr(c), _ptr(packed), _ptr(dpc), _ptr(dpg), _ptr(rh), _ptr(dh),
            dxp, _ptr(nin), T, 1 if use_avg else 0, nx, V, D, ACT_IDS[activation.lower()], _stream()))
        return dpc, dpg, rh, dh, dx
    _launch("gru_bwd_fused[nx=%d]" % nx, lambda: lib.ggnn_gru_bwd_fused_f32(
        _ptr(g), _ptr(h), _ptr(r), _ptr(u), _ptr(c), None, None, _ptr(packed), _ptr(dpc), _ptr(dpg), _ptr(rh), _ptr(dh), dxp,
        _ptr(nin), T, 1 if use_avg else 0, nx, V, D, ACT_IDS[activation.lower()], _stream()))
    return dpc, dpg, rh, dh, dx


def weighted_segment_sum(rows: torch.Tensor, index: "SegmentIndex", weight_id: torch.Tensor, weights: torch.Tensor,
                         out: Optional[torch.Tensor] = None, accumulate: bool = False) -> torch.Tensor:
    lib = _lib.load()
    _req(rows, torch.float32, "rows"); _req(weights, torch.float32, "weights"); _req(weight_id, torch.int32, "weight_id")
    D = rows.shape[1]
    nseg = index.num_nodes
    if out is None:
        out = torch.empty((nseg, D), dtype=torch.float32, device=rows.device)
    _launch("weighted_segment_sum", lambda: lib.ggnn_weighted_segment_sum_f32(
        _ptr(rows), _ptr(index.row_ptr), _ptr(index.gather_row), _ptr(weight_id), _ptr(weights), _ptr(out), 1 if accumulate else 0,
        nseg, D, _stream()))
    return out


def attn_backward_target(H: torch.Tensor, h: torch.Tensor, d_att: torch.Tensor, index: MessageIndex, type_factors: torch.Tensor,
                         dh: torch.Tensor):
    lib = _lib.load()
    V, D = h.shape
    T, M = index.num_edge_types, index.num_messages
    dev = h.device
    ca = torch.empty(max(M, 1), dtype=torch.float32, device=dev); cs = torch.empty_like(ca); df = torch.empty_like(ca)
    _launch("attn_bwd_target", lambda: lib.ggnn_attn_bwd_target_f32(
        _ptr(H), _ptr(h), _ptr(d_att), _ptr(index.row_ptr), _ptr(index.gather_row), _ptr(index.msg_perm), _ptr(type_factors), _ptr(ca),
        _ptr(cs), _ptr(df), _ptr(dh), 1, V, D, T, _stream()))
    return ca, cs, df


def range_sum(values: torch.Tensor, offsets: Sequence[int]) -> torch.Tensor:
    lib = _lib.load()
    B = len(offsets) - 1
    out = torch.empty(B, dtype=torch.float32, device=values.device)
    off = (ctypes.c_int64 * (B + 1))(*[int(o) for o in offsets])
    check(lib.ggnn_range_sum_f32(_ptr(values), off, B, _ptr(out), _stream()))
    return out


def bwd_dx(dY: torch.Tensor, nseg_y: int, WT: torch.Tensor, xcols: int, split_inc: bool, dx: Optional[torch.Tensor],
           dinc: Optional[torch.Tensor], nin: Optional[torch.Tensor], use_avg: bool, dh: Optional[torch.Tensor], acc_dx: bool,
           acc_dh: bool, D: int) -> None:
    lib = _lib.load()
    V = dY.shape[0]
    K = WT.shape[1]
    T = nin.shape[1] if nin is not None else 1
    _launch("bwd_dx[K=%d]" % K, lambda: lib.ggnn_bwd_dx_f32(
        _ptr(dY), dY.stride(0) if V > 1 else dY.shape[1], nseg_y, _ptr(WT), K, _ptr(dx), xcols, 1 if split_inc else 0, _ptr(dinc),
        _ptr(nin), T, 1 if use_avg else 0, _ptr(dh), 1 if acc_dx else 0, 1 if acc_dh else 0, V, D, _stream()))


def act_bwd(g: torch.Tensor, out: torch.Tensor, activation: str) -> torch.Tensor:
    lib = _lib.load()
    V, D = out.shape
    dP = torch.empty_like(out)
    _launch("act_bwd", lambda: lib.ggnn_act_bwd_f32(_ptr(g), _ptr(out), ACT_IDS[activation.lower()], _ptr(dP), V, D, _stream()))
    return dP


def cudnn_gru_train(x_segs: Sequence[torch.Tensor], h: torch.Tensor, Wg, bg, Wcx, bcx, Wch, bch):
    lib = _lib.load()
    V, D = h.shape
    nx = len(x_segs)
    out = torch.empty_like(h); c = torch.empty_like(h)
    ws_bytes = lib.ggnn_cudnn_gru_workspace_bytes(V, D)
    ws = torch.empty(max(ws_bytes // 4, 1), dtype=torch.float32, device=h.device)
    segs = (ctypes.c_void_p * nx)(*[_req(x, torch.float32, "x").data_ptr() for x in x_segs])
    _launch("cudnn_gru[nx=%d]" % nx, lambda: lib.ggnn_cudnn_gru_train_f32(segs, nx, _ptr(h), _ptr(Wg), _ptr(bg), _ptr(Wcx), _ptr(bcx),
                                                                          _ptr(Wch), _ptr(bch), _ptr(out), _ptr(c), _ptr(ws), ws_bytes,
                                                                          V, D, _stream()))
    n = V * D
    return out, ws[2 * n:3 * n].view(V, D), ws[n:2 * n].view(V, D), c, ws[3 * n:4 * n].view(V, D)


def cudnn_gru_bwd_stage(g, h, r, u, c, hc):
    lib = _lib.load()
    V, D = h.shape
    dpc = torch.empty_like(h); dh = torch.empty_like(h); dhc = torch.empty_like(h)
    dpg = torch.empty((V, 2 * D), dtype=torch.float32, device=h.device)
    _launch("cudnn_gru_bwd_stage", lambda: lib.ggnn_cudnn_gru_bwd_stage_f32(_ptr(g), _ptr(h), _ptr(r), _ptr(u), _ptr(c), _ptr(hc),
                                                                             _ptr(dpc), _ptr(dpg), _ptr(dh), _ptr(dhc), V, D, _stream()))
    return dpc, dpg, dh, dhc


def dropout(x: torch.Tensor, keep_prob: float, seed: int, row_key: Optional[torch.Tensor] = None, row_key_base: int = 0,
            out: Optional[torch.Tensor] = None) -> torch.Tensor:
    lib = _lib.load()
    _req(x, torch.float32, "x")
    if x.dim() < 1:
        raise ValueError("x must have at least one dimension")
    cols = x.shape[-1]
    rows = x.numel() // cols if cols else 0
    if row_key is not None:
        _req(row_key, torch.int64, "row_key")
        if row_key.numel() != rows:
            raise ValueError("row_key must have one entry per row")
    if out is None:
        out = torch.empty_like(x)
    _launch("dropout", lambda: lib.ggnn_dropout_f32(_ptr(x), _ptr(out), _ptr(row_key), int(row_key_base),
                                                    int(seed) & 0xFFFFFFFFFFFFFFFF, float(keep_prob), rows, cols, _stream()))
    return out


def unsorted_segment_sum(data: torch.Tensor, segment_ids: torch.Tensor, num_segments: int) -> torch.Tensor:
    lib = _lib.load()
    _req(data, torch.float32, "data"); _req(segment_ids, torch.int32, "segment_ids")
    M = data.shape[0]
    D = 1 if data.dim() == 1 else data.shape[1]
    out = torch.empty((num_segments,) if data.dim() == 1 else (num_segments, D), dtype=torch.float32, device=data.device)
    check(lib.ggnn_unsorted_segment_sum_f32(_ptr(data), _ptr(segment_ids), _ptr(out), M, D, num_segments, _stream()))
    return out


def segment_sum_rows_by_index(rows: torch.Tensor, index: MessageIndex, out: Optional[torch.Tensor] = None) -> torch.Tensor:
    lib = _lib.load()
    _req(rows, torch.float32, "rows")
    D = rows.shape[1]
    nseg = index.num_nodes
    if out is None:
        out = torch.empty((nseg, D), dtype=torch.float32, device=rows.device)
    return _segment_sum("gather_segment_sum_bwd", rows, index.row_ptr, index.gather_row,
                        slot_heads(index, index.row_ptr, index.gather_row, nseg), None, None, False, out, nseg, D, 1)


def dense_aggregate(adjacency: torch.Tensor, Hm: torch.Tensor, edge_biases: Optional[torch.Tensor],
                    out: Optional[torch.Tensor] = None) -> torch.Tensor:
    lib = _lib.load()
    _req(adjacency, torch.float32, "adjacency"); _req(Hm, torch.float32, "Hm")
    b, E, v, v2 = adjacency.shape
    if v != v2 or Hm.shape[0] != b * v or Hm.shape[1] % E:
        raise ValueError("shape mismatch between adjacency [b,e,v,v] and Hm [b*v, e*D]")
    D = Hm.shape[1] // E
    if edge_biases is not None:
        _req(edge_biases, torch.float32, "edge_biases")
        if edge_biases.shape != (E, D):
            raise ValueError("edge_biases must be [e,D]")
    if out is None:
        out = torch.empty((b * v, D), dtype=torch.float32, device=Hm.device)
    _launch("dense_aggregate", lambda: lib.ggnn_dense_aggregate_f32(_ptr(adjacency), _ptr(Hm), _ptr(edge_biases), _ptr(out),
                                                                   b, v, E, D, _stream()))
    return out


def dense_propagate_supported(v: int, E: int, D: int) -> bool:
    return bool(_lib.load().ggnn_dense_propagate_supported(int(v), int(E), int(D)))


def dense_propagate(h0: torch.Tensor, adjacency: torch.Tensor, edge_packed: torch.Tensor, gru_packed: torch.Tensor,
                    edge_biases: Optional[torch.Tensor], bg: torch.Tensor, bc: torch.Tensor, steps: int,
                    fmt: int = GRU_FMT_EXACT) -> torch.Tensor:
    lib = _lib.load()
    _req(h0, torch.float32, "h0"); _req(adjacency, torch.float32, "adjacency")
    b, v, D = h0.shape
    E = adjacency.shape[1]
    if adjacency.shape != (b, E, v, v):
        raise ValueError("adjacency must be [b,e,v,v]")
    for t, n, name in ((bg, 2 * D, "bg"), (bc, D, "bc")):
        _req(t, torch.float32, name)
        if t.numel() != n:
            raise ValueError("%s must have %d elements" % (name, n))
    if edge_biases is not None:
        _req(edge_biases, torch.float32, "edge_biases")
        if edge_biases.numel() != E * D:
            raise ValueError("edge_biases must be [e,D]")
    out = torch.empty_like(h0)
    _launch("dense_propagate[steps=%d]" % steps, lambda: lib.ggnn_dense_propagate_f32(
        _ptr(h0), _ptr(adjacency), _ptr(edge_packed), _ptr(gru_packed), _ptr(edge_biases), _ptr(bg), _ptr(bc), _ptr(out), b, v, E, D,
        int(steps), int(fmt), _stream()))
    return out


def dense_train_supported(v: int, E: int, D: int) -> bool:
    return bool(_lib.load().ggnn_dense_train_supported(int(v), int(E), int(D)))


def dense_propagate_save(h0: torch.Tensor, adjacency: torch.Tensor, edge_packed: torch.Tensor, gru_packed: torch.Tensor,
                         edge_biases: Optional[torch.Tensor], bg: torch.Tensor, bc: torch.Tensor, steps: int,
                         fmt: int = GRU_FMT_EXACT):
    lib = _lib.load()
    _req(h0, torch.float32, "h0"); _req(adjacency, torch.float32, "adjacency")
    if h0.dim() != 3 or adjacency.dim() != 4:
        raise ValueError("h0 must be [b,v,D] and adjacency [b,e,v,v]")
    b, v, D = h0.shape
    E = adjacency.shape[1]
    if adjacency.shape != (b, E, v, v):
        raise ValueError("adjacency must be [b,e,v,v]")
    for t, n, name in ((bg, 2 * D, "bg"), (bc, D, "bc")):
        _req(t, torch.float32, name)
        if t.numel() != n:
            raise ValueError("%s must have %d elements" % (name, n))
    if edge_biases is not None:
        _req(edge_biases, torch.float32, "edge_biases")
        if edge_biases.numel() != E * D:
            raise ValueError("edge_biases must be [e,D]")
    steps = int(steps)
    if steps < 1:
        raise ValueError("steps must be >= 1")
    out = torch.empty_like(h0)
    saved = torch.empty((6, steps, b * v, D), dtype=torch.float32, device=h0.device)
    _launch("dense_propagate_save[steps=%d]" % steps, lambda: lib.ggnn_dense_propagate_save_f32(
        _ptr(h0), _ptr(adjacency), _ptr(edge_packed), _ptr(gru_packed), _ptr(edge_biases), _ptr(bg), _ptr(bc), _ptr(out), b, v, E, D,
        steps, int(fmt), _ptr(saved), saved.numel() * 4, _stream()))
    return out, saved


def dense_bwd_pack(W: torch.Tensor, Wg: torch.Tensor, Wc: torch.Tensor) -> torch.Tensor:
    lib = _lib.load()
    _req(W, torch.float32, "edge_weights"); _req(Wg, torch.float32, "Wg"); _req(Wc, torch.float32, "Wc")
    if W.dim() != 3 or W.shape[1] != W.shape[2]:
        raise ValueError("edge_weights must be [e,D,D]")
    E, D = W.shape[0], W.shape[1]
    if tuple(Wg.shape) != (2 * D, 2 * D) or tuple(Wc.shape) != (2 * D, D):
        raise ValueError("Wg must be [2D,2D] and Wc [2D,D]")
    nbytes = lib.ggnn_dense_bwd_packed_bytes(D, E)
    if not nbytes:
        raise ValueError("no graph-resident dense backward for hidden size %d" % D)
    packed = torch.empty(nbytes // 4, dtype=torch.float32, device=W.device)
    check(lib.ggnn_dense_bwd_pack_f32(_ptr(W), _ptr(Wg), _ptr(Wc), E, D, _ptr(packed), _stream()))
    return packed


def dense_propagate_bwd(d_out: torch.Tensor, adjacency: torch.Tensor, bwd_packed: torch.Tensor, saved: torch.Tensor,
                        need_d_h0: bool = True):
    lib = _lib.load()
    _req(d_out, torch.float32, "d_out"); _req(adjacency, torch.float32, "adjacency"); _req(saved, torch.float32, "saved")
    if d_out.dim() != 3 or adjacency.dim() != 4:
        raise ValueError("d_out must be [b,v,D] and adjacency [b,e,v,v]")
    b, v, D = d_out.shape
    E = adjacency.shape[1]
    if adjacency.shape != (b, E, v, v):
        raise ValueError("adjacency must be [b,e,v,v]")
    if saved.dim() != 4 or saved.shape[0] != 6 or saved.shape[2:] != (b * v, D):
        raise ValueError("saved must be dense_propagate_save's [6, steps, b*v, D]")
    steps = saved.shape[1]
    dev = d_out.device
    d_h0 = torch.empty_like(d_out) if need_d_h0 else None
    dpc = torch.empty((steps, b * v, D), dtype=torch.float32, device=dev)
    dpg = torch.empty((steps, b * v, 2 * D), dtype=torch.float32, device=dev)
    dx = torch.empty((steps, b * v, D), dtype=torch.float32, device=dev)
    dM = torch.empty((steps, b * v, E * D), dtype=torch.float32, device=dev)
    _launch("dense_propagate_bwd[steps=%d]" % steps, lambda: lib.ggnn_dense_propagate_bwd_f32(
        _ptr(d_out), _ptr(adjacency), _ptr(bwd_packed), _ptr(saved), b, v, E, D, steps, _ptr(d_h0), _ptr(dpc), _ptr(dpg), _ptr(dx),
        _ptr(dM), _stream()))
    return d_h0, dpc, dpg, dx, dM


def dense_edge_grad_supported(E: int, D: int) -> bool:
    return int(D) in (32, 64, 100) and int(E) in (2, 4, 6, 8)


def dense_edge_grad(h: torch.Tensor, dM: torch.Tensor, nin: Optional[torch.Tensor] = None, dx: Optional[torch.Tensor] = None,
                    dW: Optional[torch.Tensor] = None, db: Optional[torch.Tensor] = None, accumulate: bool = False,
                    ws: Optional[torch.Tensor] = None):
    lib = _lib.load()
    tensors = [("h", h), ("dM", dM)] + ([("nin", nin), ("dx", dx)] if nin is not None else []) + \
              [(n, t) for n, t in (("dW", dW), ("db", db if nin is not None else None)) if t is not None]
    for name, t in tensors:
        if not isinstance(t, torch.Tensor) or not t.is_cuda or t.dtype != torch.float32 or not t.is_contiguous():
# ... 876 lines not shown
```

include/ggnn_hip.h:

```cpp
#ifndef GGNN_HIP_H
#define GGNN_HIP_H

#include <stddef.h>
#include <stdint.h>

#ifdef __cplusplus
extern "C" {
#endif

#define GGNN_ABI_VERSION 3

#define GGNN_OK 0
#define GGNN_E_INVALID (-1)
#define GGNN_E_UNSUPPORTED (-2)
#define GGNN_E_WORKSPACE (-3)
#define GGNN_E_HIP (-4)
#define GGNN_E_INDEX (-5)

#define GGNN_ACT_TANH 0
#define GGNN_ACT_RELU 1

typedef void* ggnn_stream_t;

int ggnn_abi_version(void);
const char* ggnn_last_error(void);
int ggnn_matrix_path_is_split(void);
#define GGNN_GRU_FMT_F16X2 2
#define GGNN_GRU_FMT_BF16X3 3
#define GGNN_F16X2_MAX_WEIGHT 255.875f
#define GGNN_F16X2_MAX_ACTIVATION 65504.0f
int ggnn_gru_forward_format(void);
int ggnn_gru_form_set(int form);
int ggnn_absmax_f32(const float* const* ptrs, const int64_t* numel, int n, float* out, ggnn_stream_t stream);

size_t ggnn_csr_workspace_bytes(int64_t M, int V);
int ggnn_build_target_csr(const int32_t* adj, const int64_t* type_off, int T, int V, int64_t M,
                          int32_t* row_ptr, int32_t* gather_row, int32_t* msg_perm, int32_t* err_flag,
                          void* ws, size_t ws_bytes, ggnn_stream_t stream);

int ggnn_build_source_csr(const int32_t* adj, const int64_t* type_off, int T, int V, int64_t M,
                          int32_t* row_ptr, int32_t* gather_row, int32_t* msg_perm, int32_t* err_flag,
                          void* ws, size_t ws_bytes, ggnn_stream_t stream);

int ggnn_msg_transform_f32(const float* h, int ldh, const float* W, float* H, int V, int D, int T,
                           ggnn_stream_t stream);

int ggnn_msg_transform_compact_supported(int D);
size_t ggnn_compact_workspace_bytes(int V, int T);
int ggnn_build_compact_sources(const int32_t* src_row_ptr, int V, int T, int32_t* pair_node, int32_t* pair_id,
                               int32_t* type_row_off, void* ws, size_t ws_bytes, ggnn_stream_t stream);
int ggnn_remap_gather_rows(const int32_t* gather_row, const int32_t* pair_id, int32_t* gather_row_compact, int64_t M,
                           ggnn_stream_t stream);
size_t ggnn_msg_transform_compact_workspace_bytes(int D, int T);
int ggnn_msg_transform_compact_f32(const float* h, const float* W, const int32_t* pair_node, const int64_t* type_row_off,
                                   float* Hc, void* ws, size_t ws_bytes, int V, int D, int T, int fmt, ggnn_stream_t stream);

int ggnn_gather_segment_sum_f32(const float* Hrows, const int32_t* row_ptr, const int32_t* gather_row,
                                const float* nin, const float* bias, int use_avg, float* out,
                                int V, int D, int T, ggnn_stream_t stream);

int ggnn_gather_segment_sum_attn_f32(const float* Hrows, const float* h, const int32_t* row_ptr, const int32_t* gather_row,
                                     const float* type_factors, const float* nin, const float* bias, int use_avg,
                                     float* out, int V, int D, int T, ggnn_stream_t stream);

int ggnn_build_slot_heads(const int32_t* row_ptr, const int32_t* gather_row, int32_t* heads, int V, ggnn_stream_t stream);
int ggnn_gather_segment_sum_heads_f32(const float* Hrows, const int32_t* row_ptr, const int32_t* gather_row, const int32_t* heads,
                                      const float* nin, const float* bias, int use_avg, float* out, int V, int D, int T,
                                      int accumulate, ggnn_stream_t stream);

int ggnn_attn_bwd_target_f32(const float* Hrows, const float* h, const float* d_att, const int32_t* row_ptr,
                             const int32_t* gather_row, const int32_t* msg_perm, const float* type_factors, float* coef_a,
                             float* coef_s, float* dfac, float* dh, int accumulate, int V, int D, int T, ggnn_stream_t stream);
int ggnn_weighted_segment_sum_f32(const float* rows, const int32_t* row_ptr, const int32_t* gather_row, const int32_t* weight_id,
                                  const float* weights, float* out, int accumulate, int num_segments, int D, ggnn_stream_t stream);
int ggnn_range_sum_f32(const float* values, const int64_t* range_off, int num_ranges, float* out, ggnn_stream_t stream);

int ggnn_unsorted_segment_sum_f32(const float* data, const int32_t* ids, float* out, int64_t M, int D,
                                  int num_segments, ggnn_stream_t stream);

int ggnn_gated_readout_f32(const float* hT, const float* h0, const int32_t* graph_nodes_list, const float* gate_W,
                           const float* gate_b, const float* transform_W, const float* transform_b, float* out, int V,
                           int D, int num_graphs, ggnn_stream_t stream);

size_t ggnn_readout_workspace_bytes(int V, int D, int num_graphs);
int ggnn_readout_loss_fwd_f32(const float* hT, const float* h0, const int32_t* graph_nodes_list, const int32_t* graph_ptr,
                              const float* node_mask, const float* gate_W, const float* gate_b, const float* transform_W,
                              const float* transform_b, const float* target, const float* mask, float* out,
                              float* node_gate, float* node_val, float* stats, void* ws, size_t ws_bytes, int V, int D,
                              int num_graphs, ggnn_stream_t stream);
int ggnn_readout_loss_bwd_f32(const float* hT, const float* h0, const int32_t* graph_nodes_list, const float* node_mask,
                              const float* gate_W, const float* transform_W, const float* node_gate, const float* node_val,
                              const float* out, const float* target, const float* mask, const float* d_out,
                              const float* d_stats, float* d_hT, int accumulate, float* d_gate_W, float* d_gate_b,
                              float* d_transform_W, float* d_transform_b, void* ws, size_t ws_bytes, int V, int D,
                              int num_graphs, ggnn_stream_t stream);

size_t ggnn_gru_workspace_bytes(int V, int D);
int ggnn_gru_f32(const float* const* x_segs, int nx, const float* h, const float* Wg, const float* bg,
                 const float* Wc, const float* bc, float* h_out, void* ws, size_t ws_bytes,
                 float* save_r, float* save_u, float* save_c, int V, int D, int act,
                 ggnn_stream_t stream);

int ggnn_rnn_f32(const float* const* x_segs, int nx, const float* h, const float* W, const float* b, float* h_out,
                 int V, int D, int act, ggnn_stream_t stream);
size_t ggnn_cudnn_gru_workspace_bytes(int V, int D);
int ggnn_cudnn_gru_f32(const float* const* x_segs, int nx, const float* h, const float* Wg, const float* bg,
                       const float* Wcx, const float* bcx, const float* Wch, const float* bch, float* h_out,
                       void* ws, size_t ws_bytes, int V, int D, ggnn_stream_t stream);

int ggnn_gru_is_fused(int D);

size_t ggnn_gru_packed_bytes(int D, int nx);
int ggnn_gru_pack_weights_f32(const float* Wg, const float* Wc, int nx, int D, int gru_fmt, float* packed, ggnn_stream_t stream);
int ggnn_gru_packed_f32(const float* const* x_segs, int nx, const float* h, const float* packed, const float* bg,
                        const float* bc, float* h_out, float* save_r, float* save_u, float* save_c, int V, int D, int act,
                        int gru_fmt, int32_t* tile_counter, ggnn_stream_t stream);
int ggnn_edge_weights_pack_f32(const float* W, int T, int D, int fmt, float* packed, ggnn_stream_t stream);

int ggnn_gru_packed_gather_f32(const float* const* x_segs, int nx, const float* h, const float* packed, const float* bg,
                               const float* bc, float* h_out, const float* Hrows, const int32_t* row_ptr,
                               const int32_t* gather_row, const float* nin, int T, int use_avg, int V, int D, int act,
                               int gru_fmt, int32_t* tile_counter, ggnn_stream_t stream);
int ggnn_gru_packed_gather_train_f32(const float* const* x_segs, int nx, const float* h, const float* packed, const float* bg,
                                     const float* bc, float* h_out, const float* Hrows, const int32_t* row_ptr,
                                     const int32_t* gather_row, const float* nin, int T, int use_avg, float* save_r, float* save_u,
                                     float* save_c, float* save_incoming, int V, int D, int act, int gru_fmt,
                                     int32_t* tile_counter, ggnn_stream_t stream);

int ggnn_gru_gates_f32(const float* const* x_segs, int nx, const float* h, const float* Wg, const float* bg,
                       float* rh, float* u, float* save_r, int V, int D, ggnn_stream_t stream);
int ggnn_gru_candidate_f32(const float* const* x_segs, int nx, const float* rh, const float* h, const float* u,
                           const float* Wc, const float* bc, float* h_out, float* save_c, int V, int D, int act,
                           ggnn_stream_t stream);

size_t ggnn_sparse_propagate_workspace_bytes(int V, int D, int T, int64_t compact_rows);
int ggnn_sparse_propagate_f32(const float* h0, int V, int D, int T,
                              const int32_t* row_ptr, const int32_t* gather_row, const int32_t* pair_node,
                              const int64_t* type_row_off, const float* nin, int use_avg,
                              int num_layers, const int32_t* layer_timesteps, const int32_t* res_ptr, const int32_t* res_idx,
                              const float* const* edge_w, const float* const* edge_packed, const float* const* edge_bias,
                              const float* const* Wg, const float* const* bg, const float* const* Wc, const float* const* bc,
                              const float* const* gru_packed, const int32_t* gru_fmt, const int32_t* edge_fmt, int act,
                              int fuse_gather, float* const* layer_out, void* ws, size_t ws_bytes, ggnn_stream_t stream);

int ggnn_gru_bwd_stage1_f32(const float* g, const float* h, const float* r, const float* u, const float* c, int act,
                            float* dpc, float* dpg, float* dh, float* a_c, int lda, int col0, int V, int D,
                            ggnn_stream_t stream);
int ggnn_gru_bwd_stage2_f32(const float* drh, int ld_drh, const float* h, const float* r, float* dh, float* dpg,
                            int V, int D, ggnn_stream_t stream);

int ggnn_dense_propagate_supported(int v, int E, int D);
int ggnn_dense_propagate_is_split(int v, int E, int D);
size_t ggnn_dense_edge_packed_bytes(int D, int T);
int ggnn_dense_edge_pack_f32(const float* W, int T, int D, float* packed, ggnn_stream_t stream);
size_t ggnn_dense_gru_packed_bytes(int D);
int ggnn_dense_gru_pack_f32(const float* Wg, const float* Wc, int D, float* packed, ggnn_stream_t stream);
int ggnn_dense_propagate_f32(const float* h0, const float* A, const float* edge_packed, const float* gru_packed, const float* edge_bias,
                             const float* bg, const float* bc, float* out, int b, int v, int E, int D, int steps, int fmt,
                             ggnn_stream_t stream);
int ggnn_dense_train_supported(int v, int E, int D);
size_t ggnn_dense_train_saved_bytes(int b, int v, int D, int steps);
int ggnn_dense_propagate_save_f32(const float* h0, const float* A, const float* edge_packed, const float* gru_packed,
                                  const float* edge_bias, const float* bg, const float* bc, float* out, int b, int v, int E, int D,
                                  int steps, int fmt, float* saved, size_t saved_bytes, ggnn_stream_t stream);
size_t ggnn_dense_bwd_packed_bytes(int D, int E);
int ggnn_dense_bwd_pack_f32(const float* W, const float* Wg, const float* Wc, int E, int D, float* packed, ggnn_stream_t stream);
int ggnn_dense_propagate_bwd_f32(const float* d_out, const float* A, const float* bwd_packed, const float* saved, int b, int v, int E,
                                 int D, int steps, float* d_h0, float* dpc, float* dpg, float* dx, float* dM, ggnn_stream_t stream);
size_t ggnn_dense_edge_grad_workspace_bytes(int N, int E, int D);
int ggnn_dense_edge_grad_f32(const float* h, const float* dM, const float* nin, const float* dx, int N, int rows_per_step, int E, int D,
                             float* dW, float* db, int accumulate, void* ws, size_t ws_bytes, ggnn_stream_t stream);
size_t ggnn_dense_train_workspace_bytes(int b, int v, int E, int D, int steps);
int ggnn_dense_train_forward_f32(const float* h0, const float* A, const float* edge_packed, const float* gru_packed,
                                 const float* edge_bias, const float* bg, const float* bc, int b, int v, int E, int D, int steps, int fmt,
                                 void* ws, size_t ws_bytes, int64_t* final_off, ggnn_stream_t stream);
int ggnn_dense_train_backward_f32(const float* d_final, const float* A, const float* nin, const float* bwd_packed, int b, int v, int E,
                                  int D, int steps, float* g_W, float* g_b, float* g_Wg, float* g_bg, float* g_Wc, float* g_bc,
                                  void* ws, size_t ws_bytes, ggnn_stream_t stream, ggnn_stream_t side_stream);
int ggnn_dense_aggregate_f32(const float* A, const float* Hm, const float* bias, float* acts, int b, int v,
                             int e, int D, ggnn_stream_t stream);

int ggnn_gemm_f32(const float* const* a_segs, int nseg, int D, int lda, const float* B, int ldb, float* C, int ldc,
                  int M, int N, ggnn_stream_t stream);

size_t ggnn_gemm_tn_workspace_bytes(int M, int K, int N);
int ggnn_gemm_tn_f32(const float* A, int lda, const float* B, int ldb, float* C, int M, int K, int N, void* ws,
                     size_t ws_bytes, ggnn_stream_t stream);

size_t ggnn_xty_workspace_bytes(int M_max, int K, int N, int nbatch);
int ggnn_xty_f32(const float* const* x_segs, int nseg, int Dseg, const int32_t* ldx, const int32_t* x_rows, const float* Y,
                 int ldy, float* C, int K, int N, int ones_row, const int32_t* row_off, int nbatch, void* ws, size_t ws_bytes,
                 ggnn_stream_t stream);
int ggnn_xty_acc_f32(const float* const* x_segs, int nseg, int Dseg, const int32_t* ldx, const int32_t* x_rows, const float* Y,
                     int ldy, float* C, float* Cb, int accumulate, int K, int N, int ones_row, const int32_t* row_off, int nbatch,
                     void* ws, size_t ws_bytes, ggnn_stream_t stream);
size_t ggnn_colsum_workspace_bytes(int N);
int ggnn_colsum_f32(const float* Y, int ldy, int M, int N, float* out, void* ws, size_t ws_bytes, ggnn_stream_t stream);
int ggnn_gru_bwd_dx_cand_f32(const float* dpc, const float* WcT, const float* h, const float* r, float* dx, float* dh,
                             float* dpg, int nx, int V, int D, ggnn_stream_t stream);
int ggnn_gru_bwd_dx_gates_f32(const float* dpg, const float* WgT, float* dx, float* dinc, const float* nin, int T,
                              int use_avg, float* dh, int nx, int V, int D, ggnn_stream_t stream);
int ggnn_gather_segment_sum_acc_f32(const float* Hrows, const int32_t* row_ptr, const int32_t* gather_row, float* out,
                                    int V, int D, ggnn_stream_t stream);

int ggnn_bwd_dx_f32(const float* dY, int ldy, int nseg_y, const float* WT, int K, float* dx, int xcols, int split_inc, float* dinc,
                    const float* nin, int T, int use_avg, float* dh, int acc_dx, int acc_dh, int V, int D, ggnn_stream_t stream);
int ggnn_act_bwd_f32(const float* g, const float* out, int act, float* dP, int V, int D, ggnn_stream_t stream);
int ggnn_cudnn_gru_train_f32(const float* const* x_segs, int nx, const float* h, const float* Wg, const float* bg,
                             const float* Wcx, const float* bcx, const float* Wch, const float* bch, float* h_out,
                             float* save_c, void* ws, size_t ws_bytes, int V, int D, ggnn_stream_t stream);
int ggnn_cudnn_gru_bwd_stage_f32(const float* g, const float* h, const float* r, const float* u, const float* c, const float* hc,
                                 float* dpc, float* dpg, float* dh, float* dhc, int V, int D, ggnn_stream_t stream);

int ggnn_gru_bwd_is_fused(int D);
size_t ggnn_gru_bwd_packed_bytes(int D, int nx);
int ggnn_gru_bwd_fused_f32(const float* g, const float* h, const float* r, const float* u, const float* c, const float* Wg,
                           const float* Wc, float* packed, float* dpc, float* dpg, float* rh, float* dh, float* const* dx,
                           const float* nin, int T, int use_avg, int nx, int V, int D, int act, ggnn_stream_t stream);
int ggnn_gru_bwd_fused_gather_f32(const float* g, const float* gz, const int32_t* gz_heads, const float* h, const float* r,
                                  const float* u, const float* c, float* packed, float* dpc, float* dpg, float* rh, float* dh,
                                  float* const* dx, const float* nin, int T, int use_avg, int nx, int V, int D, int act,
                                  ggnn_stream_t stream);

int ggnn_optim_block_floats(void);
int ggnn_clip_adam_f32(float* const* param_ptrs, const int32_t* var_numel, const float* grads, float* m, float* v, float* partial,
                       const int32_t* block_var, const int32_t* var_first, const int32_t* var_active, int nblocks, float clip_norm,
                       float lr_t, float beta1, float beta2, float epsilon, ggnn_stream_t stream);

int ggnn_assemble_batch_backward(const void* const* ds_tables, const void* const* bwd_tables, int A, int T, const int64_t* ds_type_off,
                                 const int64_t* ds_type_row_off, const int32_t* batch_tab, const int32_t* graph_nodes_list, int G, int V,
                                 int M, int R, int D, const int64_t* type_off, const int64_t* type_row_off, void* const* out,
                                 ggnn_stream_t stream);
int ggnn_assemble_batch(const void* const* ds_tables, int A, int T, const int64_t* ds_type_off, const int64_t* ds_type_row_off,
                        const int32_t* batch_tab, int G, int V, int M, int R, int D, const int64_t* type_off,
                        const int64_t* type_row_off, void* const* out, ggnn_stream_t stream);
int ggnn_pack_batch_tables(const int32_t* counts_t, int Gd, int rows, const int64_t* gids, int G, const float* targets,
                           const float* label_mask, int num_targets, const int64_t* task_ids, int K, int32_t* batch_tab,
                           float* target_values, float* target_mask, ggnn_stream_t stream);
int ggnn_gcn_assemble_batch(const void* const* ds_tables, int Gd, int A, int num_targets, const int64_t* task_ids, int K,
                            const int32_t* epoch_tab, int Ge, int s, int G, int V, int nnz, int D, void* const* out,
                            ggnn_stream_t stream);
int ggnn_dense_assemble_batch(const void* const* ds_tables, int Gd, int A, int T, int num_targets, const int64_t* task_ids, int K,
                              const int32_t* epoch_tab, int Ge, int s, int G, int v, int D, int M, int R, const int64_t* type_off,
                              const int64_t* type_row_off, int sparse, void* const* out, ggnn_stream_t stream);

int ggnn_sparse_train_prepare_f32(int num_layers, int T, int D, const int32_t* nx, const float* const* edge_w, float keep_prob,
                                  const uint64_t* seeds, const float* const* Wg, const float* const* Wc, const int32_t* gru_fmt,
                                  float* const* edge_packed, float* const* edge_packed_t, float* const* gru_packed,
                                  float* const* gru_bwd_packed, ggnn_stream_t stream);
size_t ggnn_sparse_train_workspace_bytes(int V, int D, int T, int64_t compact_rows, int total_steps);
int ggnn_sparse_train_forward_f32(const float* h0, int V, int D, int T, const int32_t* row_ptr, const int32_t* gather_row_c,
                                  const int32_t* pair_node, const int64_t* type_row_off, const float* nin, int use_avg, int num_layers,
                                  const int32_t* layer_timesteps, const int32_t* res_ptr, const int32_t* res_idx,
                                  const float* const* edge_packed, const float* const* bg, const float* const* bc,
                                  const float* const* gru_packed, const int32_t* gru_fmt, int act, void* ws, size_t ws_bytes,
                                  int64_t* final_state_offset, ggnn_stream_t stream);
int ggnn_sparse_train_backward_f32(const float* h0, int V, int D, int T, const int32_t* pair_node, const int64_t* type_row_off,
                                   const float* nin, int use_avg, int num_layers, const int32_t* layer_timesteps,
                                   const int32_t* res_ptr, const int32_t* res_idx, const int32_t* rows_rp, const int32_t* rows_gather,
                                   const int32_t* rows_heads, const int32_t* node_rp, const int32_t* node_order,
                                   const int32_t* node_heads, const int32_t* identity_rows, const float* const* edge_packed_t,
                                   const float* const* gru_bwd_packed, int act, float* const* g_edge, float* const* g_Wg,
                                   float* const* g_bg, float* const* g_Wc, float* const* g_bc, float* d_final, float* const* d_state_ws,
                                   void* ws, size_t ws_bytes, ggnn_stream_t stream, ggnn_stream_t side_stream);

int ggnn_dropout_f32(const float* x, float* out, const int64_t* row_key, int64_t row_key_base, uint64_t seed, float keep_prob,
                     int64_t rows, int cols, ggnn_stream_t stream);

int ggnn_gcn_fused_supported(int D);
size_t ggnn_gcn_image_bytes(int D);
int ggnn_gcn_pack_weights_f32(const float* W, int D, int transpose, float* img, ggnn_stream_t stream);
int ggnn_gcn_layer_f32(const float* x, const int32_t* row_ptr, const int32_t* col, const float* val, int64_t nnz, const float* img,
                       const float* bias, int relu, const int64_t* row_key, int64_t row_key_base, uint64_t seed, float keep_prob,
                       float* out, float* s_out, int V, int D, ggnn_stream_t stream);
int ggnn_gcn_epilogue_f32(const float* P, const float* bias, int relu, const int64_t* row_key, int64_t row_key_base, uint64_t seed,
                          float keep_prob, float* out, int V, int D, ggnn_stream_t stream);
size_t ggnn_gcn_workspace_bytes(int V, int D, int num_layers);
int ggnn_gcn_propagate_f32(const float* h0, int V, int D, int num_layers, const int32_t* row_ptr, const int32_t* col, const float* val,
                           int64_t nnz, const float* const* W, const float* const* bias, float* out, void* ws, size_t ws_bytes,
                           ggnn_stream_t stream);

size_t ggnn_probe_mfma_workspace_bytes(void);
int ggnn_probe_mfma_rate(int mode, int launches, void* ws, size_t ws_bytes, double* tflops, double* shader_mhz, ggnn_stream_t stream);

#ifdef __cplusplus
}
#endif
#endif
```

Baseline: 1.263 billion.

## Defer split-K weight-gradient reductions and batch them into one chained kernel

Weight-gradient X^T·Y products in the training backward now write their split partials into dedicated per-product slots, each with a header of workgroup offsets, instead of reducing immediately. One deferred kernel later reduces all pending products, chaining products that accumulate into the same destination. This removes many small reduce launches and lets the GEMM kernels run back to back without waiting on reductions. In exchange it needs one slot of workspace per pending product and adds host-side chaining and overlap-detection logic.

```diff
diff --git a/gated-graph-neural-network-samples_amd/_lib.py b/gated-graph-neural-network-samples_amd/_lib.py
--- a/gated-graph-neural-network-samples_amd/_lib.py
+++ b/gated-graph-neural-network-samples_amd/_lib.py
@@ -7,6 +7,13 @@
 _HERE = os.path.dirname(os.path.abspath(__file__))
 LIB_PATH = os.path.join(_HERE, "libggnn_hip%s.so" % ("_" + os.environ["GGNN_LIB_VARIANT"] if os.environ.get("GGNN_LIB_VARIANT") else ""))
 ABI_VERSION = 3
+
+
+
+class XtyDeferred(ctypes.Structure):
+    _fields_ = [("slot", c_void_p), ("C", c_void_p), ("Cb", c_void_p), ("K", c_int32), ("N", c_int32), ("ones_row", c_int32),
+                ("nbatch", c_int32), ("accumulate", c_int32), ("wg_rows", c_int32)]
+
 
 SYMBOLS = {
     "ggnn_abi_version": (c_int, []),
@@ -112,6 +119,11 @@
                                     c_int, c_int, POINTER(c_int64), POINTER(c_int64), POINTER(c_void_p), c_void_p]),
     "ggnn_xty_acc_f32": (c_int, [POINTER(c_void_p), c_int, c_int, POINTER(c_int32), c_void_p, c_void_p, c_int, c_void_p, c_void_p,
                                  c_int, c_int, c_int, c_int, POINTER(c_int32), c_int, c_void_p, c_size_t, c_void_p]),
+    "ggnn_xty_slot_bytes": (c_size_t, [POINTER(c_int32), c_int, c_int, c_int, c_int]),
+    "ggnn_xty_slot_bytes_max": (c_size_t, [c_int64, c_int, c_int, c_int]),
+    "ggnn_xty_defer_f32": (c_int, [POINTER(c_void_p), c_int, c_int, POINTER(c_int32), c_void_p, c_void_p, c_int, c_void_p, c_void_p,
+                                   c_int, c_int, c_int, c_int, POINTER(c_int32), c_int, c_void_p, c_size_t, POINTER(XtyDeferred), c_void_p]),
+    "ggnn_xty_reduce_deferred_f32": (c_int, [POINTER(XtyDeferred), c_int, c_void_p]),
     "ggnn_colsum_workspace_bytes": (c_size_t, [c_int]),
     "ggnn_colsum_f32": (c_int, [c_void_p, c_int, c_int, c_int, c_void_p, c_void_p, c_size_t, c_void_p]),
     "ggnn_gru_bwd_dx_cand_f32": (c_int, [c_void_p] * 7 + [c_int, c_int, c_int, c_void_p]),
diff --git a/gated-graph-neural-network-samples_amd/csrc/ggnn_bwd_gemm.hip b/gated-graph-neural-network-samples_amd/csrc/ggnn_bwd_gemm.hip
--- a/gated-graph-neural-network-samples_amd/csrc/ggnn_bwd_gemm.hip
+++ b/gated-graph-neural-network-samples_amd/csrc/ggnn_bwd_gemm.hip
@@ -25,7 +25,13 @@
     int kb_tiles, n_tiles;
     int pitch_x, pitch_y;
     unsigned long long* tdbg;
+    int* hdr;
 };
+
+__device__ inline void xty_write_header(const XtyArgs& a) {
+    if (a.hdr && blockIdx.x == 0 && blockIdx.y == 0 && threadIdx.x == 0)
+        for (int b = 0; b <= a.nbatch; ++b) a.hdr[b] = a.wg_off[b];
+}
 
 static inline int xty_pitch(int width) {
     int p = (width + 15) / 16 * 16;
@@ -227,6 +233,7 @@
     else if (my_mt == MTM && my_nt == NTM - 1) run(IM{}, IN1{});
     else if (my_mt == MTM - 1 && my_nt == NTM - 1) run(IM1{}, IN1{});
     else run(I0{}, I0{});
+    xty_write_header(a);
 #undef GGNN_XT
 }
 
@@ -421,6 +428,7 @@
     else if (my_mt == MTM - 1 && my_nt == 2 * NTM - 1) run(IM1{}, IN1{});
     else if (my_mt == MTM - 1 && my_nt == 2 * NTM - 2) run(IM1{}, IN2{});
     else run(I0{}, I0{});
+    xty_write_header(a);
 }
 
 template <int MTM, int NTM>
@@ -610,6 +618,7 @@
     else if (my_mt == MTM - 1 && my_nt == 2 * NTM - 1) run(IM1{}, IN1{});
     else if (my_mt == MTM - 1 && my_nt == 2 * NTM - 2) run(IM1{}, IN2{});
     else run(I0{}, I0{});
+    xty_write_header(a);
 }
 
 struct XtyReduceArgs { int wg_off[kXtyMaxBatch + 1]; };
@@ -638,6 +647,59 @@
         const float v = ((red[0][c] + red[1][c]) + (red[2][c] + red[3][c])) + ((red[4][c] + red[5][c]) + (red[6][c] + red[7][c]));
         float* dst = (Cb && j >= KwN) ? Cb + (size_t)b * (KN - KwN) + (j - KwN) : C + (size_t)b * (Cb ? KwN : KN) + j;
         *dst = accumulate ? *dst + v : v;
+    }
+}
+
+constexpr int kXtySlotHeader = 512;
+constexpr int kXtyDeferMax = 64;
+struct XtyDeferredArgs {
+    const float* part[kXtyDeferMax]; float* C[kXtyDeferMax]; float* Cb[kXtyDeferMax];
+    int KN[kXtyDeferMax], KwN[kXtyDeferMax], nbatch[kXtyDeferMax], accumulate[kXtyDeferMax], wg_rows[kXtyDeferMax];
+    int next[kXtyDeferMax];
+    int head[kXtyDeferMax], block_begin[kXtyDeferMax + 1];
+    int nchains;
+};
+
+__global__ __launch_bounds__(256) void xty_reduce_deferred_kernel(XtyDeferredArgs d) {
+    __shared__ f32x4 red[8][32];
+    const int c = threadIdx.x & 31, q = threadIdx.x >> 5;
+    int g = 0;
+    while (g + 1 < d.nchains && (int)blockIdx.x >= d.block_begin[g + 1]) ++g;
+    int s = d.head[g];
+    const int KN = d.KN[s], KwN = d.KwN[s], nbatch = d.nbatch[s];
+    const long long i = ((long long)((int)blockIdx.x - d.block_begin[g]) * 32 + c) * 4;
+    const bool on = i < (long long)KN * nbatch;
+    const int b = on ? (int)(i / KN) : 0, j = on ? (int)(i - (long long)b * KN) : 0;
+    for (; s >= 0; s = d.next[s]) {
+        f32x4 sum = {0.f, 0.f, 0.f, 0.f};
+        if (on && d.wg_rows[s] > 0) {
+            const float* part = d.part[s];
+            const int* wg_off = reinterpret_cast<const int*>(reinterpret_cast<const char*>(part) - kXtySlotHeader);
+            const int w0 = wg_off[b], S = wg_off[b + 1] - w0;
+            const float* src = part + (size_t)w0 * KN + j;
+            auto ld = [&](int p) { return *reinterpret_cast<const f32x4*>(src + (size_t)p * KN); };
+            int p = q;
+            for (; p + 56 < S; p += 64) {
+                const f32x4 v0 = ld(p), v1 = ld(p + 8), v2 = ld(p + 16), v3 = ld(p + 24), v4 = ld(p + 32), v5 = ld(p + 40), v6 = ld(p + 48), v7 = ld(p + 56);
+                sum += v0; sum += v1; sum += v2; sum += v3; sum += v4; sum += v5; sum += v6; sum += v7;
+            }
+            for (; p + 24 < S; p += 32) {
+                const f32x4 v0 = ld(p), v1 = ld(p + 8), v2 = ld(p + 16), v3 = ld(p + 24);
+                sum += v0; sum += v1; sum += v2; sum += v3;
+            }
+            for (; p < S; p += 8) sum += ld(p);
+        }
+        red[q][c] = sum;
+        __syncthreads();
+        if (q == 0 && on) {
+            const f32x4 v = ((red[0][c] + red[1][c]) + (red[2][c] + red[3][c])) + ((red[4][c] + red[5][c]) + (red[6][c] + red[7][c]));
+            float* Cb = d.Cb[s];
+            float* dst = (Cb && j >= KwN) ? Cb + (size_t)b * (KN - KwN) + (j - KwN) : d.C[s] + (size_t)b * (Cb ? KwN : KN) + j;
+            const bool acc = d.accumulate[s] != 0;
+#pragma unroll
+            for (int e = 0; e < 4; ++e) dst[e] = acc ? dst[e] + v[e] : v[e];
+        }
+        __syncthreads();
     }
 }
 
@@ -672,6 +734,21 @@
     return p;
 }
 
+static size_t xty_slot_bytes(const XtyPlan& p, int Kout, int N) {
+    return ((size_t)kXtySlotHeader + (size_t)p.wg_rows * Kout * N * sizeof(float) + 255) / 256 * 256;
+}
+
+static int launch_xty_reduce(const XtyArgs& a, float* C, float* Cb, int accumulate, hipStream_t st) {
+    if (a.hdr) return GGNN_OK;
+    XtyReduceArgs ra;
+    for (int b = 0; b <= kXtyMaxBatch; ++b) ra.wg_off[b] = a.wg_off[b <= a.nbatch ? b : a.nbatch];
+    const long long total = (long long)a.Kout * a.N * a.nbatch;
+    hipLaunchKernelGGL(xty_reduce_kernel, dim3((unsigned)((total + 31) / 32)), dim3(256), 0, st, (const float*)a.part, C, Cb, a.Kout * a.N,
+                       a.K * a.N, a.nbatch, accumulate, ra);
+    GGNN_CHECK_HIP(hipGetLastError());
+    return GGNN_OK;
+}
+
 template <bool GATHER, int ROWS, int MTM, int NTM>
 static int launch_xty(const XtyArgs& a, const XtyPlan& p, float* C, float* Cb, int accumulate, hipStream_t st) {
     static std::atomic<unsigned long long> lds_ok{0};
@@ -680,13 +757,7 @@
         hipLaunchKernelGGL((xty_kernel<GATHER, ROWS, MTM, NTM>), dim3(p.kblocks, p.wg_rows), dim3(kXtyWaves * 64), p.lds, st, a);
         GGNN_CHECK_HIP(hipGetLastError());
     }
-    XtyReduceArgs ra;
-    for (int b = 0; b <= kXtyMaxBatch; ++b) ra.wg_off[b] = a.wg_off[b <= a.nbatch ? b : a.nbatch];
-    const long long total = (long long)a.Kout * a.N * a.nbatch;
-    hipLaunchKernelGGL(xty_reduce_kernel, dim3((unsigned)((total + 31) / 32)), dim3(256), 0, st, (const float*)a.part, C, Cb, a.Kout * a.N,
-                       a.K * a.N, a.nbatch, accumulate, ra);
-    GGNN_CHECK_HIP(hipGetLastError());
-    return GGNN_OK;
+    return launch_xty_reduce(a, C, Cb, accumulate, st);
 }
 
 template <int MTM, int NTM>
@@ -698,13 +769,7 @@
         hipLaunchKernelGGL((xty_planes_kernel<MTM, NTM>), dim3(p.kblocks, p.wg_rows), dim3(kXtySplitWaves * 64), lds, st, a);
         GGNN_CHECK_HIP(hipGetLastError());
     }
-    XtyReduceArgs ra;
-    for (int b = 0; b <= kXtyMaxBatch; ++b) ra.wg_off[b] = a.wg_off[b <= a.nbatch ? b : a.nbatch];
-    const long long total = (long long)a.Kout * a.N * a.nbatch;
-    hipLaunchKernelGGL(xty_reduce_kernel, dim3((unsigned)((total + 31) / 32)), dim3(256), 0, st, (const float*)a.part, C, Cb, a.Kout * a.N,
-                       a.K * a.N, a.nbatch, accumulate, ra);
-    GGNN_CHECK_HIP(hipGetLastError());
-    return GGNN_OK;
+    return launch_xty_reduce(a, C, Cb, accumulate, st);
 }
 
 template <bool GATHER, int ROWS, int MTM, int NTM>
@@ -715,13 +780,7 @@
         hipLaunchKernelGGL((xty_split_kernel<GATHER, ROWS, MTM, NTM>), dim3(p.kblocks, p.wg_rows), dim3(kXtySplitWaves * 64), p.lds, st, a);
         GGNN_CHECK_HIP(hipGetLastError());
     }
-    XtyReduceArgs ra;
-    for (int b = 0; b <= kXtyMaxBatch; ++b) ra.wg_off[b] = a.wg_off[b <= a.nbatch ? b : a.nbatch];
-    const long long total = (long long)a.Kout * a.N * a.nbatch;
-    hipLaunchKernelGGL(xty_reduce_kernel, dim3((unsigned)((total + 31) / 32)), dim3(256), 0, st, (const float*)a.part, C, Cb, a.Kout * a.N,
-                       a.K * a.N, a.nbatch, accumulate, ra);
-    GGNN_CHECK_HIP(hipGetLastError());
-    return GGNN_OK;
+    return launch_xty_reduce(a, C, Cb, accumulate, st);
 }
 
 constexpr int kColsumBlocks = 256;
@@ -774,9 +833,9 @@
     return ggnn_xty_acc_f32(x_segs, nseg, Dseg, ldx, x_rows, Y, ldy, C, nullptr, 0, K, N, ones_row, row_off, nbatch, ws, ws_bytes, stream);
 }
 
-extern "C" int ggnn_xty_acc_f32(const float* const* x_segs, int nseg, int Dseg, const int32_t* ldx, const int32_t* x_rows,
-                                const float* Y, int ldy, float* C, float* Cb, int accumulate, int K, int N, int ones_row,
-                                const int32_t* row_off, int nbatch, void* ws, size_t ws_bytes, ggnn_stream_t stream) {
+static int xty_product(const float* const* x_segs, int nseg, int Dseg, const int32_t* ldx, const int32_t* x_rows,
+                       const float* Y, int ldy, float* C, float* Cb, int accumulate, int K, int N, int ones_row,
+                       const int32_t* row_off, int nbatch, void* ws, size_t ws_bytes, ggnn_xty_deferred_t* deferred, ggnn_stream_t stream) {
     const int Kout = ones_row ? K + 1 : K;
     GGNN_CHECK_ARG(!Cb || ones_row, "a bias destination needs the ones row");
     GGNN_CHECK_ARG(nseg >= 1 && nseg <= 4 && Dseg > 0 && Dseg % 4 == 0 && K == nseg * Dseg, "X is nseg <= 4 segments of Dseg columns (K = %d, nseg = %d, Dseg = %d)", K, nseg, Dseg);
@@ -790,6 +849,11 @@
         a.row_off[b] = row_off[b];
         if (b) { GGNN_CHECK_ARG(row_off[b] >= row_off[b - 1], "row_off not monotone"); m_max = row_off[b] - row_off[b - 1] > m_max ? row_off[b] - row_off[b - 1] : m_max; }
     }
+    if (deferred) {
+        deferred->slot = ws; deferred->C = C; deferred->Cb = Cb; deferred->K = K; deferred->N = N; deferred->ones_row = ones_row ? 1 : 0;
+        deferred->nbatch = nbatch; deferred->accumulate = accumulate ? 1 : 0; deferred->wg_rows = 0;
+        if (m_max == 0) { if (accumulate) deferred->nbatch = 0; return GGNN_OK; }
+    }
     if (m_max == 0) {
         if (!accumulate) {
             GGNN_CHECK_HIP(hipMemsetAsync(C, 0, (size_t)nbatch * (Cb ? K : Kout) * N * sizeof(float), st));
@@ -802,10 +866,18 @@
         GGNN_CHECK_ARG(x_segs[s] && aligned16(x_segs[s]) && ldx[s] >= Dseg && ldx[s] % 4 == 0, "X segment %d null, misaligned or bad stride", s);
         a.X[s] = x_segs[s]; a.ldx[s] = ldx[s];
     }
-    if (ws_bytes < ggnn_xty_workspace_bytes(m_max, K, N, nbatch)) return fail(GGNN_E_WORKSPACE, "xty workspace too small");
     const XtyPlan p = xty_plan(row_off, nbatch, Kout, N);
+    if (deferred) {
+        if (ws_bytes < xty_slot_bytes(p, Kout, N)) return fail(GGNN_E_WORKSPACE, "xty slot too small");
+        a.hdr = static_cast<int*>(ws);
+        a.part = reinterpret_cast<float*>(static_cast<char*>(ws) + kXtySlotHeader);
+        deferred->wg_rows = p.wg_rows;
+    } else {
+        if (ws_bytes < ggnn_xty_workspace_bytes(m_max, K, N, nbatch)) return fail(GGNN_E_WORKSPACE, "xty workspace too small");
+        a.part = static_cast<float*>(ws);
+    }
     a.Kout = Kout;
-    a.nseg = nseg; a.Dseg = Dseg; a.x_rows = x_rows; a.Y = Y; a.ldy = ldy; a.part = static_cast<float*>(ws);
+    a.nseg = nseg; a.Dseg = Dseg; a.x_rows = x_rows; a.Y = Y; a.ldy = ldy;
     a.K = K; a.N = N; a.nbatch = nbatch; a.kb_tiles = p.kb_tiles; a.n_tiles = p.n_tiles;
     a.pitch_x = p.px; a.pitch_y = p.py;
     for (int b = 0; b <= kXtyMaxBatch; ++b) a.wg_off[b] = p.wg_off[b <= nbatch ? b : nbatch];
@@ -841,6 +913,79 @@
     return fail(GGNN_E_UNSUPPORTED, "xty: no kernel for %d x %d tile groups (K=%d N=%d)", mtm, ntm, K, N);
 }
 
+extern "C" int ggnn_xty_acc_f32(const float* const* x_segs, int nseg, int Dseg, const int32_t* ldx, const int32_t* x_rows,
+                                const float* Y, int ldy, float* C, float* Cb, int accumulate, int K, int N, int ones_row,
+                                const int32_t* row_off, int nbatch, void* ws, size_t ws_bytes, ggnn_stream_t stream) {
+    return xty_product(x_segs, nseg, Dseg, ldx, x_rows, Y, ldy, C, Cb, accumulate, K, N, ones_row, row_off, nbatch, ws, ws_bytes, nullptr, stream);
+}
+
+extern "C" size_t ggnn_xty_slot_bytes(const int32_t* row_off, int nbatch, int K, int N, int ones_row) {
+    if (!row_off || nbatch <= 0 || nbatch > kXtyMaxBatch || K <= 0 || N <= 0) return 0;
+    const int Kout = ones_row ? K + 1 : K;
+    return xty_slot_bytes(xty_plan(row_off, nbatch, Kout, N), Kout, N);
+}
+
+extern "C" size_t ggnn_xty_slot_bytes_max(int64_t M_total, int K, int N, int nbatch) {
+    if (M_total < 0 || K <= 0 || N <= 0 || nbatch <= 0) return 0;
+    const long long by_rows = (M_total + 127) / 128 + nbatch;
+    const long long wg_rows = (by_rows < num_cus() ? by_rows : num_cus()) + nbatch;
+    return ((size_t)kXtySlotHeader + (size_t)wg_rows * (K + 1) * N * sizeof(float) + 255) / 256 * 256;
+}
+
+extern "C" int ggnn_xty_defer_f32(const float* const* x_segs, int nseg, int Dseg, const int32_t* ldx, const int32_t* x_rows,
+                                  const float* Y, int ldy, float* C, float* Cb, int accumulate, int K, int N, int ones_row,
+                                  const int32_t* row_off, int nbatch, void* slot, size_t slot_bytes, ggnn_xty_deferred_t* deferred,
+                                  ggnn_stream_t stream) {
+    GGNN_CHECK_ARG(deferred && slot && aligned16(slot), "null or misaligned slot / descriptor");
+    return xty_product(x_segs, nseg, Dseg, ldx, x_rows, Y, ldy, C, Cb, accumulate, K, N, ones_row, row_off, nbatch, slot, slot_bytes, deferred, stream);
+}
+
+extern "C" int ggnn_xty_reduce_deferred_f32(const ggnn_xty_deferred_t* list, int count, ggnn_stream_t stream) {
+    GGNN_CHECK_ARG(count >= 0 && (list || count == 0), "bad list");
+    hipStream_t st = (hipStream_t)stream;
+    XtyDeferredArgs d{};
+    int n = 0, tail[kXtyDeferMax];
+    struct Range { const char* lo[2]; const char* hi[2]; };
+    Range rng[kXtyDeferMax];
+    auto launch = [&]() -> int {
+        if (n == 0) return GGNN_OK;
+        hipLaunchKernelGGL(xty_reduce_deferred_kernel, dim3((unsigned)d.block_begin[d.nchains]), dim3(256), 0, st, d);
+        GGNN_CHECK_HIP(hipGetLastError());
+        d = XtyDeferredArgs{}; n = 0;
+        return GGNN_OK;
+    };
+    for (int i = 0; i < count; ++i) {
+        const ggnn_xty_deferred_t& e = list[i];
+        if (e.nbatch == 0) continue;
+        GGNN_CHECK_ARG(e.slot && aligned16(e.slot) && e.C && e.K > 0 && e.N > 0 && e.N % 4 == 0 && e.nbatch > 0 && e.nbatch <= kXtyMaxBatch && e.wg_rows >= 0 && (!e.Cb || e.ones_row),
+                       "bad deferred product %d", i);
+        const int KN = (e.ones_row ? e.K + 1 : e.K) * e.N, KwN = e.K * e.N;
+        Range r;
+        r.lo[0] = reinterpret_cast<const char*>(e.C); r.hi[0] = r.lo[0] + (size_t)e.nbatch * (e.Cb ? KwN : KN) * sizeof(float);
+        r.lo[1] = reinterpret_cast<const char*>(e.Cb); r.hi[1] = r.lo[1] + (e.Cb ? (size_t)e.nbatch * (KN - KwN) * sizeof(float) : 0);
+        int chain = -1; bool clash = false;
+        for (int g = 0; g < d.nchains && !clash; ++g) {
+            const int h = d.head[g];
+            if (d.C[h] == e.C && d.Cb[h] == e.Cb && d.KN[h] == KN && d.KwN[h] == KwN && d.nbatch[h] == e.nbatch) { chain = g; break; }
+            for (int x = 0; x < 2; ++x) for (int y = 0; y < 2; ++y)
+                if (r.lo[x] < rng[h].hi[y] && rng[h].lo[y] < r.hi[x]) clash = true;
+        }
+        if (clash || n == kXtyDeferMax) { if (int rc = launch()) return rc; chain = -1; }
+        const int s = n++;
+        d.part[s] = reinterpret_cast<const float*>(static_cast<const char*>(e.slot) + kXtySlotHeader);
+        d.C[s] = e.C; d.Cb[s] = e.Cb; d.KN[s] = KN; d.KwN[s] = KwN; d.nbatch[s] = e.nbatch; d.accumulate[s] = e.accumulate;
+        d.wg_rows[s] = e.wg_rows; d.next[s] = -1; rng[s] = r;
+        if (chain >= 0) { d.next[tail[chain]] = s; tail[chain] = s; }
+        else {
+            const int g = d.nchains++;
+            const long long blocks = ((long long)KN * e.nbatch / 4 + 31) / 32;
+            GGNN_CHECK_ARG(d.block_begin[g] + blocks < (1LL << 31), "deferred reduce: too many blocks");
+            d.head[g] = s; tail[g] = s; d.block_begin[g + 1] = d.block_begin[g] + (int)blocks;
+        }
+    }
+    return launch();
+}
+
 extern "C" size_t ggnn_colsum_workspace_bytes(int N) { return (size_t)kColsumBlocks * (N > 0 ? N : 1) * sizeof(float) + 256; }
 
 extern "C" int ggnn_colsum_f32(const float* Y, int ldy, int M, int N, float* out, void* ws, size_t ws_bytes, ggnn_stream_t stream) {
diff --git a/gated-graph-neural-network-samples_amd/csrc/ggnn_train.hip b/gated-graph-neural-network-samples_amd/csrc/ggnn_train.hip
--- a/gated-graph-neural-network-samples_amd/csrc/ggnn_train.hip
+++ b/gated-graph-neural-network-samples_amd/csrc/ggnn_train.hip
@@ -7,12 +7,15 @@
 
 constexpr int kMaxLayers = 62;
 constexpr int kMaxNx = 3;
+constexpr size_t kXtyArenaBudget = (size_t)1 << 30;
+constexpr int kXtyPendingMax = 64;
 
 inline size_t al256(size_t x) { return (x + 255) / 256 * 256; }
 
 struct TrainLayout {
     size_t Hc, state, r, u, c, inc, counters;
     size_t dpc, rh, dh, dpg, dx, dHc, Z, xty;
+    size_t xty_bytes;
     size_t vd, rd, total;
     int steps;
 };
@@ -32,9 +35,16 @@
     L.dpc = take(L.vd * steps); L.rh = take(L.vd * steps); L.dh = take(L.vd * steps); L.dpg = take(2 * L.vd * steps);
     L.dx = take(L.vd * steps * kMaxNx);
     L.dHc = take(L.rd * steps); L.Z = take(L.rd);
-    L.xty = take(ggnn_xty_workspace_bytes((V > R ? V : (int)R) * (steps > 1 ? steps : 1), 4 * D, 2 * D, T));
+    const size_t wc = ggnn_xty_slot_bytes_max(V, (kMaxNx + 1) * D, D, 1), wg = ggnn_xty_slot_bytes_max(V, (kMaxNx + 1) * D, 2 * D, 1);
+    const size_t we = ggnn_xty_slot_bytes_max(R > 0 ? R : 1, D, D, T);
+    const size_t merged = ggnn_xty_slot_bytes_max((int64_t)V * steps, (kMaxNx + 1) * D, 2 * D, 1);
+    size_t arena = (size_t)steps * (wc + wg + we);
+    if (arena > kXtyArenaBudget) arena = kXtyArenaBudget;
+    if (arena < merged) arena = merged;
+    if (arena < we) arena = we;
+    L.xty_bytes = al256(arena);
+    L.xty = take(L.xty_bytes);
     L.total = p + 256;
-    (void)T;
     return L;
 }
 
@@ -304,8 +314,27 @@
     hipStream_t st = (hipStream_t)stream, side = side_stream ? (hipStream_t)side_stream : (hipStream_t)stream;
     auto buf = [&](size_t off, int step) { return reinterpret_cast<float*>(base + off + (size_t)step * L.vd); };
     float* Z = reinterpret_cast<float*>(base + L.Z);
-    void* xty_ws = base + L.xty;
-    const size_t xty_ws_bytes = L.total - 256 - L.xty;
+    char* const arena = base + L.xty;
+    size_t arena_used = 0;
+    ggnn_xty_deferred_t pending[kXtyPendingMax];
+    int npending = 0;
+    auto flush_products = [&]() -> int {
+        if (npending == 0) return GGNN_OK;
+        const int rc = ggnn_xty_reduce_deferred_f32(pending, npending, side);
+        npending = 0; arena_used = 0;
+        return rc;
+    };
+    auto defer_product = [&](const float* const* X, int nseg, const int32_t* ldx, const int32_t* x_rows, const float* Y, int ldy, float* C,
+                             float* Cb, int K, int N, int ones_row, const int32_t* row_off, int nbatch) -> int {
+        const size_t need = ggnn_xty_slot_bytes(row_off, nbatch, K, N, ones_row);
+        if (need == 0 || need > L.xty_bytes) return fail(GGNN_E_WORKSPACE, "training workspace: a weight-gradient slot of %zu bytes does not fit the arena (%zu)", need, L.xty_bytes);
+        if (npending == kXtyPendingMax || arena_used + need > L.xty_bytes) { if (int rc = flush_products()) return rc; }
+        if (int rc = ggnn_xty_defer_f32(X, nseg, D, ldx, x_rows, Y, ldy, C, Cb, 1, K, N, ones_row, row_off, nbatch, arena + arena_used, need,
+                                        &pending[npending], side)) return rc;
+        ++npending; arena_used += need;
+        return GGNN_OK;
+    };
+    static const bool reduce_per_layer = [] { const char* e = getenv("GGNN_TRAIN_REDUCE_PER_LAYER"); return e && atoi(e) != 0; }();
     const size_t edge_img_bytes = ggnn_msg_transform_compact_workspace_bytes(D, T);
     const long long nvd = (long long)V * D;
     int32_t row_off_v[2] = {0, V};
@@ -371,11 +400,10 @@
                     const int k0 = P.first_step;
                     int32_t row_off_m[2] = {0, V * P.steps};
                     const float* X[2] = {buf(L.inc, k0), buf(L.rh, k0)}; int32_t ldx[2] = {D, D};
-                    if (int rc = ggnn_xty_acc_f32(X, 2, D, ldx, nullptr, buf(L.dpc, k0), D, g_Wc[l], g_bc[l], 1, 2 * D, D, 1, row_off_m, 1,
-                                                  xty_ws, xty_ws_bytes, side)) return rc;
+                    if (int rc = defer_product(X, 2, ldx, nullptr, buf(L.dpc, k0), D, g_Wc[l], g_bc[l], 2 * D, D, 1, row_off_m, 1)) return rc;
                     X[1] = buf(L.state, k0);
-                    if (int rc = ggnn_xty_acc_f32(X, 2, D, ldx, nullptr, reinterpret_cast<float*>(base + L.dpg + (size_t)k0 * 2 * L.vd), 2 * D,
-                                                  g_Wg[l], g_bg[l], 1, 2 * D, 2 * D, 1, row_off_m, 1, xty_ws, xty_ws_bytes, side)) return rc;
+                    if (int rc = defer_product(X, 2, ldx, nullptr, reinterpret_cast<float*>(base + L.dpg + (size_t)k0 * 2 * L.vd), 2 * D,
+                                               g_Wg[l], g_bg[l], 2 * D, 2 * D, 1, row_off_m, 1)) return rc;
                 }
             } else {
                 if (int rc = order_after(side, st)) return rc;
@@ -383,11 +411,9 @@
                 for (int i = 0; i < P.nres; ++i) { X[i] = states[P.res[i]]; ldx[i] = D; }
                 X[nx - 1] = buf(L.inc, k); ldx[nx - 1] = D;
                 X[nx] = rh; ldx[nx] = D;
-                if (int rc = ggnn_xty_acc_f32(X, nx + 1, D, ldx, nullptr, dpc, D, g_Wc[l], g_bc[l], 1, (nx + 1) * D, D, 1, row_off_v, 1,
-                                              xty_ws, xty_ws_bytes, side)) return rc;
+                if (int rc = defer_product(X, nx + 1, ldx, nullptr, dpc, D, g_Wc[l], g_bc[l], (nx + 1) * D, D, 1, row_off_v, 1)) return rc;
                 X[nx] = h_in;
-                if (int rc = ggnn_xty_acc_f32(X, nx + 1, D, ldx, nullptr, dpg, 2 * D, g_Wg[l], g_bg[l], 1, (nx + 1) * D, 2 * D, 1, row_off_v, 1,
-                                              xty_ws, xty_ws_bytes, side)) return rc;
+                if (int rc = defer_product(X, nx + 1, ldx, nullptr, dpg, 2 * D, g_Wg[l], g_bg[l], (nx + 1) * D, 2 * D, 1, row_off_v, 1)) return rc;
             }
 
             float* dHc = reinterpret_cast<float*>(base + L.dHc + (size_t)k * L.rd);
@@ -411,8 +437,7 @@
             if (int rc = order_after(side, st)) return rc;
             {
                 const float* X[1] = {h_in}; int32_t ldx[1] = {D};
-                if (int rc = ggnn_xty_acc_f32(X, 1, D, ldx, pair_node, dHc, D, g_edge[l], nullptr, 1, D, D, 0, row_off_t, T, xty_ws, xty_ws_bytes,
-                                              side)) return rc;
+                if (int rc = defer_product(X, 1, ldx, pair_node, dHc, D, g_edge[l], nullptr, D, D, 0, row_off_t, T)) return rc;
             }
             for (int i = 0; i < P.nres; ++i) {
                 if (!dx_direct[i] && P.res[i] != 0) { if (int rc = add_inplace(dstate[P.res[i]], dxp[i], nvd, st)) return rc; }
@@ -420,7 +445,9 @@
             if (s == 0 && !dh_direct && l != 0) { if (int rc = add_inplace(dstate[l], dh_dst, nvd, st)) return rc; }
             g = dh_dst;
         }
+        if (reduce_per_layer) { if (int rc = flush_products()) return rc; }
     }
     GGNN_CHECK_ARG(!z_pending, "internal: a deferred node sum of the transform backward was never added (fuse_node_sum invariant)");
+    if (int rc = flush_products()) return rc;
     return order_after(st, side);
 }
diff --git a/gated-graph-neural-network-samples_amd/ops.py b/gated-graph-neural-network-samples_amd/ops.py
--- a/gated-graph-neural-network-samples_amd/ops.py
+++ b/gated-graph-neural-network-samples_amd/ops.py
@@ -372,6 +372,58 @@
     _launch("xty[K=%d,N=%d%s]" % (K, N, ",x%d" % B if batched else ""), lambda: lib.ggnn_xty_f32(
         segs, nseg, Dseg, ldx, _ptr(x_rows), _ptr(dy), ldy, _ptr(out), K, N, 1 if ones_row else 0, ro, B, _ptr(ws), ws_bytes, _stream()))
     return out if batched else out[0]
+
+
+class XtyDeferredList:
+
+    def __init__(self, device):
+        self.device = device
+        self._desc = []
+        self._keep = []
+
+    def defer(self, x_segs: Sequence[torch.Tensor], dy: torch.Tensor, add_to: torch.Tensor, add_bias_to: Optional[torch.Tensor] = None,
+              x_rows: Optional[torch.Tensor] = None, row_off: Optional[Sequence[int]] = None, ones_row: bool = False,
+              accumulate: bool = True) -> None:
+        lib = _lib.load()
+        nseg = len(x_segs)
+        if not 1 <= nseg <= 4:
+            raise ValueError("a deferred product takes 1..4 segments")
+        Dseg = x_segs[0].shape[1]
+        for i, x in enumerate(x_segs):
+            if not x.is_cuda or x.dtype != torch.float32 or x.dim() != 2 or x.shape[1] != Dseg or (x.shape[0] > 1 and x.stride(1) != 1):
+                raise TypeError("x_segs[%d] must be a [M, %d] float32 CUDA/HIP tensor with unit column stride" % (i, Dseg))
+        if not dy.is_cuda or dy.dtype != torch.float32 or dy.dim() != 2 or (dy.shape[0] > 1 and dy.stride(1) != 1):
+            raise TypeError("dy must be a 2-D float32 CUDA/HIP tensor with unit column stride")
+        M, N = dy.shape
+        K = nseg * Dseg
+        offs = [0, M] if row_off is None else [int(o) for o in row_off]
+        B = len(offs) - 1
+        if ones_row != (add_bias_to is not None):
+            raise ValueError("ones_row needs add_bias_to (and vice versa)")
+        for t, n in ((add_to, B * K * N), (add_bias_to, B * N)):
+            if t is not None and (not t.is_cuda or t.dtype != torch.float32 or not t.is_contiguous() or t.numel() != n):
+                raise TypeError("destinations must be contiguous float32 CUDA/HIP tensors of %d elements" % n)
+        if x_rows is not None:
+            _req(x_rows, torch.int32, "x_rows")
+        ro = (ctypes.c_int32 * (B + 1))(*offs)
+        slot_bytes = lib.ggnn_xty_slot_bytes(ro, B, K, N, 1 if ones_row else 0)
+        slot = torch.empty(max(slot_bytes, 256), dtype=torch.uint8, device=dy.device)
+        segs = (ctypes.c_void_p * nseg)(*[x.data_ptr() for x in x_segs])
+        ldx = (ctypes.c_int32 * nseg)(*[(x.stride(0) if x.shape[0] > 1 else Dseg) for x in x_segs])
+        ldy = dy.stride(0) if M > 1 else N
+        desc = _lib.XtyDeferred()
+        _launch("xty_defer[K=%d,N=%d%s]" % (K, N, ",x%d" % B if row_off is not None else ""), lambda: lib.ggnn_xty_defer_f32(
+            segs, nseg, Dseg, ldx, _ptr(x_rows), _ptr(dy), ldy, _ptr(add_to), _ptr(add_bias_to), 1 if accumulate else 0, K, N,
+            1 if ones_row else 0, ro, B, _ptr(slot), slot_bytes, ctypes.byref(desc), _stream()))
+        self._desc.append(desc)
+        self._keep.append((slot, list(x_segs), dy, x_rows, add_to, add_bias_to))
+
+    def reduce(self) -> None:
+        lib = _lib.load()
+        n = len(self._desc)
+        arr = (_lib.XtyDeferred * max(n, 1))(*self._desc)
+        _launch("xty_reduce_deferred[%d]" % n, lambda: lib.ggnn_xty_reduce_deferred_f32(arr, n, _stream()))
+        self._desc, self._keep = [], []
 
 
 def colsum(dy: torch.Tensor) -> torch.Tensor:
diff --git a/include/ggnn_hip.h b/include/ggnn_hip.h
--- a/include/ggnn_hip.h
+++ b/include/ggnn_hip.h
@@ -194,6 +194,20 @@
 int ggnn_xty_acc_f32(const float* const* x_segs, int nseg, int Dseg, const int32_t* ldx, const int32_t* x_rows, const float* Y,
                      int ldy, float* C, float* Cb, int accumulate, int K, int N, int ones_row, const int32_t* row_off, int nbatch,
                      void* ws, size_t ws_bytes, ggnn_stream_t stream);
+typedef struct ggnn_xty_deferred {
+    void* slot;
+    float* C; float* Cb;
+    int32_t K, N, ones_row;
+    int32_t nbatch;
+    int32_t accumulate;
+    int32_t wg_rows;
+} ggnn_xty_deferred_t;
+size_t ggnn_xty_slot_bytes(const int32_t* row_off, int nbatch, int K, int N, int ones_row);
+size_t ggnn_xty_slot_bytes_max(int64_t M_total, int K, int N, int nbatch);
+int ggnn_xty_defer_f32(const float* const* x_segs, int nseg, int Dseg, const int32_t* ldx, const int32_t* x_rows, const float* Y,
+                       int ldy, float* C, float* Cb, int accumulate, int K, int N, int ones_row, const int32_t* row_off, int nbatch,
+                       void* slot, size_t slot_bytes, ggnn_xty_deferred_t* deferred, ggnn_stream_t stream);
+int ggnn_xty_reduce_deferred_f32(const ggnn_xty_deferred_t* list, int count, ggnn_stream_t stream);
 size_t ggnn_colsum_workspace_bytes(int N);
 int ggnn_colsum_f32(const float* Y, int ldy, int M, int N, float* out, void* ws, size_t ws_bytes, ggnn_stream_t stream);
 int ggnn_gru_bwd_dx_cand_f32(const float* dpc, const float* WcT, const float* h, const float* r, float* dx, float* dh,
```

After: 1.259 billion, median of 2. Within noise of the previous version (-0.3%).
